# yhwu/rsicnv

Measured on AMD Instinct MI355X. Metric: bases/sec through RSI pipeline (bin+GC+NB+segment), higher is better.
Workload: dtype int32

## Files before the change

### include/rsi_hot.h

```cpp
#ifndef RSI_HOT_H
#define RSI_HOT_H
#include <stddef.h>
#include <stdint.h>
#ifdef __cplusplus
extern "C" {
#endif

typedef enum rsi_status {
  RSI_OK = 0,
  RSI_ERR_NO_DEVICE = -1,
  RSI_ERR_BAD_ARG = -2,
  RSI_ERR_HIP = -3,
  RSI_ERR_TOO_SMALL = -4,
  RSI_ERR_UNSUPPORTED = -5,
  RSI_ERR_INTERNAL = -6
} rsi_status;

typedef struct rsi_params {
  int32_t m;
  int32_t gcadjust;
  int32_t trans;
  int32_t merge;
  int32_t maxchkbp;
  int32_t debug;
// ... 182 lines not shown
int rsi_result_summary(const rsi_result* r, int chrom_id, double* out, int max_calls);
int rsi_summary_format_row(const double* block, int i, const char* chrom, char* buf, int cap);
int rsi_summary_format_rows(const double* block, const char* chrom, char* buf, int cap);
int rsi_result_log_line(const rsi_result* r, int i, char* buf, int cap);
int rsi_bam_references(const char* bam_path, char* names, int names_cap, int64_t* lengths, int max_refs);
int rsi_hot_run_bam(rsi_ctx* ctx, const rsi_params* p, const char* bam_path, const char* chrom, int minq, int min_baseq,
                    const uint8_t* fasta, int64_t n, rsi_result** out, rsi_bam_stats* stats);
int rsi_hot_run_device(rsi_ctx* ctx, const rsi_params* p, const void* d_depth, const void* d_fasta, int64_t n,
                       rsi_result** out);

typedef struct rsi_ref rsi_ref;
typedef struct rsi_ref_seq {
  int64_t length, offset;
  int32_t linebases, linewidth;
  char name[256];
} rsi_ref_seq;
typedef struct rsi_ref_stats {
  int64_t bytes_read;
  int64_t text_bytes;
  int64_t members;
  int32_t format;
  int32_t index_used;
  double t_kernel_ms;
  double t_wall_ms;
} rsi_ref_stats;
int rsi_ref_open(const char* fasta_path, const char* fai_path, const char* gzi_path, rsi_ref** out);
void rsi_ref_close(rsi_ref* ref);
const char* rsi_ref_last_error(const rsi_ref* ref);
int rsi_ref_count(const rsi_ref* ref);
int rsi_ref_sequence(const rsi_ref* ref, int i, rsi_ref_seq* out);
int rsi_ref_find(const rsi_ref* ref, const char* rname);
int rsi_ref_format(const rsi_ref* ref);
const char* rsi_ref_index_path(const rsi_ref* ref);
int rsi_ref_load_device(rsi_ref* ref, int device, int i, void* d_out, int64_t cap, void* stream, rsi_ref_stats* st);
int rsi_ref_load_host(rsi_ref* ref, int device, int i, uint8_t* out, int64_t cap);
int rsi_hot_run_text_dfasta(rsi_ctx* ctx, const rsi_params* p, const char* depth_path, const void* d_fasta, int64_t n,
                            rsi_result** out, rsi_text_stats* stats);
int rsi_hot_run_bam_dfasta(rsi_ctx* ctx, const rsi_params* p, const char* bam_path, const char* chrom, int minq, int min_baseq,
                           const void* d_fasta, int64_t n, rsi_result** out, rsi_bam_stats* stats);
void* rsi_ref_device_alloc(int device, int64_t bytes);
void rsi_ref_device_free(int device, void* p);
int rsi_ref_debug_fai_line(const char* line, rsi_ref_seq* out);
int rsi_ref_debug_set_chunks(rsi_ref* ref, int64_t text_chunk_bases, int64_t bgzf_span_bytes);
int rsi_ref_debug_ranges(const rsi_ref_seq* s, int64_t k0, int64_t k1, int64_t a_in, int64_t b_in, int at_eof, int64_t* out);
int64_t rsi_ref_debug_gzi(const uint8_t* image, int64_t len, int64_t* table, int64_t cap);
int rsi_ref_debug_cover(const int64_t* table, int64_t n, int64_t a, int64_t b, int64_t* out);

int rsi_hot_set_exclude(rsi_ctx* ctx, const int64_t* start, const int64_t* end, int count);
int rsi_exclude_read_bed(const char* path, const char* chrom, int64_t n, int64_t* start, int64_t* end, int cap);

typedef struct rsi_track_stats { int64_t n, lines, bytes, slices; double t_total_ms, t_kernel_ms, t_write_ms; } rsi_track_stats;
int rsi_hot_write_track(rsi_ctx* ctx, int which, const char* chrom, const char* path, int append, rsi_track_stats* stats);
int rsi_hot_write_track_device(rsi_ctx* ctx, const void* d_values, int64_t n, const char* chrom, const char* path, int append,
                               rsi_track_stats* stats);
int64_t rsi_hot_debug_track(rsi_ctx* ctx, const int32_t* values, int64_t n, const char* chrom, int64_t pos0, int64_t slice_bases,
                            char* out, int64_t cap, rsi_track_stats* stats);

int rsi_hot_write_bin_track(rsi_ctx* ctx, int which, const char* chrom, const char* path, int append, rsi_track_stats* stats);
int64_t rsi_hot_debug_bin_track(rsi_ctx* ctx, const int32_t* values, int64_t nb, int m, int64_t n, const int32_t* pairs, int npairs,
                                int64_t median2, int which, const char* chrom, int64_t slice_bins, char* out, int64_t cap,
                                rsi_track_stats* stats);

enum { RSI_TRACK_TEXT = 0, RSI_TRACK_BGZF = 1 };
int rsi_hot_set_track_format(rsi_ctx* ctx, int format);
typedef struct rsi_deflate_stats {
  int64_t members;
  int64_t stored_members;
  int64_t text_bytes;
  int64_t file_bytes;
  double t_kernel_ms;
} rsi_deflate_stats;
int rsi_hot_last_deflate_stats(const rsi_ctx* ctx, rsi_deflate_stats* out);
int rsi_bgzf_write_eof(const char* path);
int64_t rsi_hot_debug_deflate(rsi_ctx* ctx, const uint8_t* text, int64_t len, uint8_t* out, int64_t cap, rsi_deflate_stats* stats);

typedef struct rsi_track_index rsi_track_index;
rsi_track_index* rsi_track_index_create(void);
void rsi_track_index_free(rsi_track_index* ix);
int rsi_hot_set_track_index(rsi_ctx* ctx, rsi_track_index* ix);
int rsi_track_index_append(rsi_track_index* dst, const rsi_track_index* src, int64_t shift);
int rsi_track_index_write_tbi(rsi_track_index* ix, const char* path);
int rsi_track_index_counts(const rsi_track_index* ix, int64_t* nref, int64_t* nchunks, int64_t* nwindows);
int64_t rsi_track_index_debug_tbi(const rsi_track_index* ix, uint8_t* out, int64_t cap);

int rsi_hot_loaded_depth(rsi_ctx* ctx, const void** d_depth, int64_t* n);
typedef struct rsi_depth_summary {
  int64_t n, sum;
  int64_t over;
  int64_t negative;
  int32_t min, max;
} rsi_depth_summary;
int rsi_hot_depth_summary(rsi_ctx* ctx, const void* d_depth, int64_t n, rsi_depth_summary* out, int64_t* dist, int dist_cap);
typedef struct rsi_depth_region { int64_t n, sum; int32_t min, max; } rsi_depth_region;
int rsi_hot_depth_regions(rsi_ctx* ctx, const void* d_depth, int64_t n, int nreg, const int64_t* start, const int64_t* end, rsi_depth_region* out);
int rsi_hot_write_window_track(rsi_ctx* ctx, const void* d_depth, int64_t n, const char* chrom, int64_t W, const char* path, int append,
                               rsi_track_stats* stats);
int rsi_hot_write_region_track(rsi_ctx* ctx, const void* d_depth, int64_t n, const char* chrom, int nreg, const int64_t* start,
                               const int64_t* end, const char* path, int append, rsi_track_stats* stats);
typedef struct rsi_depth_stats {
  int64_t launches;
  int64_t workgroups;
  int64_t bytes;
  double ms;
  double kernel_ms;
} rsi_depth_stats;
int rsi_hot_last_depth_stats(const rsi_ctx* ctx, rsi_depth_stats* out);
int rsi_hot_debug_depth_summary(rsi_ctx* ctx, const int32_t* values, int64_t n, int64_t span, rsi_depth_summary* out, int64_t* dist, int dist_cap);
int rsi_hot_debug_depth_regions(rsi_ctx* ctx, const int32_t* values, int64_t n, int tile, int nreg, const int64_t* start, const int64_t* end,
                                rsi_depth_region* out);
int64_t rsi_hot_debug_region_track(rsi_ctx* ctx, const int32_t* values, int64_t n, const char* chrom, int64_t W, int nreg, const int64_t* start,
                                   const int64_t* end, int span, int tile, int64_t slice_lines, int64_t pos0, char* out, int64_t cap,
                                   rsi_track_stats* stats);

int rsi_result_ncalls(const rsi_result* r, int which);
const rsi_call* rsi_result_calls(const rsi_result* r, int which);
const rsi_chrom_stats* rsi_result_stats(const rsi_result* r);
int rsi_result_noncode(const rsi_result* r, int32_t* pairs, int cap);
int rsi_result_format_row(const rsi_result* r, int i, const char* chrom, char* buf, int cap);
void rsi_result_free(rsi_result* r);

int64_t rsi_hot_fetch_i32(rsi_ctx* ctx, const char* name, int32_t* out, int64_t cap);
int64_t rsi_hot_fetch_f32(rsi_ctx* ctx, const char* name, float* out, int64_t cap);
int64_t rsi_hot_fetch_i64(rsi_ctx* ctx, const char* name, int64_t* out, int64_t cap);

int rsi_hot_debug_level_sums(rsi_ctx* ctx, const float* T, const int32_t* status, int64_t nb, int Lmax, float* sums, int32_t* counts);
int rsi_hot_debug_scan(rsi_ctx* ctx, const float* T, const int32_t* medint, int64_t nb, double RDmedian, double tmedian, double tlamda,
                       int Lmax, int32_t* status, int32_t* info);
int rsi_hot_debug_segments(rsi_ctx* ctx, const float* T, const int32_t* status, int64_t nb, const int32_t* runs, int nruns, double tmedian,
                           double tlamda, int64_t pairs_per_item, int32_t* seg_start, int32_t* seg_end, int32_t* seg_type, double* seg_score,
                           int32_t* info);
int rsi_hot_debug_sharpen(rsi_ctx* ctx, const int32_t* depth, int64_t n, int storage, int32_t* start, int32_t* end, const int32_t* type,
                          int njobs, int32_t* info);
typedef struct rsi_cand_record {
  int32_t capacity, top, margin, cut, nleft, nright;
  int32_t road;
  int32_t flags, nref, nbody, nwin, left_reach, right_reach, body_min, body_max;
  int32_t type, status, geno;
  double body_q[3], body_s1, body_s2, ref_q[3], ref_s1, ref_s2;
  double p1, cnvmed, cnvsd, cnviqr, refmed, refsd, refiqr;
} rsi_cand_record;
int rsi_hot_debug_candidate_tests(rsi_ctx* ctx, const int32_t* depth, int64_t n, int storage, int64_t span_all, double RDmedian, int m,
                                  double minmlen, double chklen, double buffer, int maxchkbp, const int32_t* start, const int32_t* end,
                                  const int32_t* type, const int32_t* status, int ncand, const int32_t* index, int nindex, int form,
                                  rsi_cand_record* out, int32_t* info);
int rsi_hot_debug_range_sums(rsi_ctx* ctx, const int32_t* depth, int64_t n, int storage, const int32_t* lo, const int32_t* hi, int nranges,
                             int64_t* sums, int32_t* info);
int rsi_hot_debug_block_stage(rsi_ctx* ctx, const int32_t* binmedint, const int32_t* status, int64_t nb, int64_t ncompact, double RDmedian,
                              const rsi_params* P, rsi_call* segs, int nsegs, int use_tester, int sparse, int32_t* road, int32_t* info);
int rsi_hot_debug_merge(rsi_ctx* ctx, const int32_t* depth, int64_t n, int storage, double RDmedian, const rsi_params* P, const rsi_call* list,
                        int nlist, int use_tester, rsi_call* out, int32_t* nout, int32_t* info);
int rsi_hot_debug_calls(rsi_ctx* ctx, const int32_t* depth, int64_t n, int storage, double RDmedian, double RDsd, const rsi_params* P,
                        const rsi_call* segs, int nsegs, const int32_t* noncode_start, const int32_t* noncode_end, int nnoncode, int use_tester,
                        rsi_call* blocks, rsi_call* raw, rsi_call* kept, int32_t* counts, int32_t* info);
int rsi_hot_debug_nb_transform(rsi_ctx* ctx, const int64_t* binsum, int64_t nb, int m, int64_t ncompact, double RDmedian, double r,
                               float* raw, float* T, int32_t* info);
int rsi_hot_debug_filterstatus(rsi_ctx* ctx, const float* T, const int32_t* status, int64_t nb, int Lmax, double dev, int32_t* status_out,
                               int32_t* info);
int rsi_hot_debug_grid_median(rsi_ctx* ctx, const float* x, const int32_t* mask, int64_t nb, int mode, double center, double* out,
                              int32_t* info);
int rsi_hot_debug_grid_mad_i32(rsi_ctx* ctx, const int32_t* x, int64_t nb, double center, double* out, int32_t* info);
int rsi_hot_debug_nb_keyed(rsi_ctx* ctx, const int64_t* binsum, const int32_t* mask, int64_t nb, int m, int64_t K, double RDmedian, double r,
                           float* T, double* out, int32_t* info);

int rsi_hot_debug_classify(rsi_ctx* ctx, const uint8_t* fasta, int64_t n, const int64_t* start, const int64_t* end, int count,
                           uint64_t* gcbits, uint64_t* nbits);

int rsi_hot_debug_per_base(rsi_ctx* ctx, const rsi_params* p, const int32_t* depth, const uint8_t* fasta, int64_t n, const int64_t* start,
                           const int64_t* end, int count, rsi_chrom_stats* out);

int rsi_hot_kernel_times(const rsi_ctx* ctx, const char** names, float* ms, int cap);
int rsi_hot_phase_times(const rsi_ctx* ctx, const char** names, double* ms, int cap);
void rsi_hot_set_timing(rsi_ctx* ctx, int on);
void rsi_hot_set_timing_kernel(rsi_ctx* ctx, const char* name);

typedef struct rsi_pool rsi_pool;
#define RSI_MAX_TIMED 64
typedef struct rsi_batch_times {
  int32_t nkernels, nphases;
  const char* kernel_name[RSI_MAX_TIMED];
  double kernel_ms[RSI_MAX_TIMED];
  int64_t kernel_launches[RSI_MAX_TIMED];
  int64_t kernel_bases[RSI_MAX_TIMED];
  const char* phase_name[RSI_MAX_TIMED];
  double phase_ms[RSI_MAX_TIMED];
} rsi_batch_times;

rsi_pool* rsi_pool_create(int device, int nworkers, int* status);
void rsi_pool_destroy(rsi_pool* pool);
int rsi_pool_workers(const rsi_pool* pool);
int rsi_pool_hw_queues(const rsi_pool* pool);
rsi_ctx* rsi_pool_worker(rsi_pool* pool, int w);
void rsi_pool_set_timing(rsi_pool* pool, int on);
void rsi_pool_set_timing_kernel(rsi_pool* pool, const char* name);
void rsi_pool_set_schedule(rsi_pool* pool, int isolate, int streamers);
const char* rsi_pool_last_error(const rsi_pool* pool);
int rsi_pool_run(rsi_pool* pool, const rsi_params* p, int nchrom, const void* const* d_depth,
                 const void* const* d_fasta, const int64_t* n, rsi_result** out, int* status,
                 rsi_batch_times* times);

int rsi_plot_expand(const int32_t* rdc, int64_t ncompact, const int32_t* regions, int npairs, int32_t* out, int64_t n);
int rsi_plot_write_files(const rsi_call* c, const char* title, const int32_t* rd, int64_t n, double chrom_median, int m,
                         double minmlen, double chklen, const char* format, double gnuplot_version, const char* datfile,
                         const char* gpfile, const char* imgfile);

typedef struct rsi_plot_batch rsi_plot_batch;
rsi_plot_batch* rsi_plot_batch_new(int64_t n, int m, double minmlen, double chklen);
void rsi_plot_batch_free(rsi_plot_batch* b);
int rsi_plot_batch_add(rsi_plot_batch* b, const rsi_call* c);
int rsi_plot_batch_add_span(rsi_plot_batch* b, int start, int end, int type);
int rsi_plot_batch_size(const rsi_plot_batch* b);
int rsi_plot_batch_refusal(const rsi_plot_batch* b, int i);
const char* rsi_plot_refusal_text(int refusal);
int64_t rsi_plot_batch_queries(const rsi_plot_batch* b);
int rsi_plot_batch_fill_host(rsi_plot_batch* b, const int32_t* rd, int64_t n);
double rsi_plot_batch_chrom_median(const rsi_plot_batch* b);
int rsi_plot_batch_compare(const rsi_plot_batch* a, const rsi_plot_batch* b);
int rsi_plot_batch_write(const rsi_plot_batch* b, int i, const char* title, const char* format, double gnuplot_version, const char* datfile,
                         const char* gpfile, const char* imgfile);
typedef struct rsi_plot_stats {
  int64_t launches, batches, tiles;
  int64_t calls, queries;
  int64_t bytes_up, bytes_down;
  int64_t bytes;
  double ms, expand_ms;
} rsi_plot_stats;
int rsi_hot_plot_depth(rsi_ctx* ctx, const void* d_depth, int64_t n, rsi_plot_batch* b);
int rsi_hot_plot_run(rsi_ctx* ctx, const rsi_result* res, rsi_plot_batch* b);
int rsi_hot_last_plot_stats(const rsi_ctx* ctx, rsi_plot_stats* out);
int rsi_hot_debug_plot(rsi_ctx* ctx, const int32_t* depth, int64_t n, int tile, int64_t workspace_bytes, rsi_plot_batch* b);
int rsi_hot_debug_plot_expand(rsi_ctx* ctx, const int32_t* rdc, int64_t ncompact, int storage, const int32_t* regions, int npairs, int32_t* out, int64_t n);

int rsi_pool_run_host(rsi_pool* pool, const rsi_params* p, int nchrom, const int32_t* const* depth,
                      const uint8_t* const* fasta, const int64_t* n, rsi_result** out, int* status,
                      rsi_batch_times* times);

uint64_t rsi_pool_submit(rsi_pool* pool, const rsi_params* p, int nchrom, const void* const* d_depth,
                         const void* const* d_fasta, const int64_t* n, rsi_result** out, int* status,
                         rsi_batch_times* times);
int rsi_pool_wait(rsi_pool* pool, uint64_t ticket);

#ifdef __cplusplus
}
#endif
#endif
```

### rsicnv_amd/api.py

```python
import contextlib
import ctypes as C
import os

import numpy as np

POOL_HW_QUEUES, MIN_HW_QUEUES = 32, 4


def _queue_count(s):
    return int(s) if s is not None and 1 <= len(s) <= 9 and all(c in "0123456789" for c in s) else -1


def _process_setup(env=os.environ):
    user = env.get("RSI_HOT_HW_QUEUES")
    if user != "keep":
        want = _queue_count(user)
        if want >= 0:
            env["GPU_MAX_HW_QUEUES"] = str(min(POOL_HW_QUEUES, max(MIN_HW_QUEUES, want)))
        elif _queue_count(env.get("GPU_MAX_HW_QUEUES")) < POOL_HW_QUEUES:
            env["GPU_MAX_HW_QUEUES"] = str(POOL_HW_QUEUES)
    return max(0, _queue_count(env.get("GPU_MAX_HW_QUEUES")))


HW_QUEUES = _process_setup()

_HERE = os.path.dirname(os.path.abspath(__file__))
LIB_PATH = os.environ.get("RSI_HOT_LIB") or os.path.join(_HERE, "librsi_hot.so")

RSI_OK = 0
STATUS_NAMES = {0: "RSI_OK", -1: "RSI_ERR_NO_DEVICE", -2: "RSI_ERR_BAD_ARG", -3: "RSI_ERR_HIP",
                -4: "RSI_ERR_TOO_SMALL", -5: "RSI_ERR_UNSUPPORTED", -6: "RSI_ERR_INTERNAL"}

CAND_RECORD = np.dtype([(k, np.int32) for k in ("capacity", "top", "margin", "cut", "nleft", "nright", "road", "flags", "nref", "nbody", "nwin",
                                                "left_reach", "right_reach", "body_min", "body_max", "type", "status", "geno")] +
                       [("body_q", np.float64, 3), ("body_s1", np.float64), ("body_s2", np.float64), ("ref_q", np.float64, 3),
                        ("ref_s1", np.float64), ("ref_s2", np.float64)] +
                       [(k, np.float64) for k in ("p1", "cnvmed", "cnvsd", "cnviqr", "refmed", "refsd", "refiqr")])
assert CAND_RECORD.itemsize == 18 * 4 + 17 * 8

CALL_RECORD = np.dtype([(k, np.int32) for k in ("start", "end", "type", "geno", "status", "length", "qscore", "pad")] +
                       [(k, np.float64) for k in ("score", "p1", "cnvmed", "cnvsd", "cnviqr", "refmed", "refsd", "refiqr")])
assert CALL_RECORD.itemsize == 8 * 4 + 8 * 8
LIST_INFO = ("spec_hits", "single_tests", "host_fallbacks", "block_batch_hits", "waits", "sum_launches", "sum_reused", "sum_redone", "tests")

GENO_RECORD = np.dtype([(k, np.int32) for k in ("n_body", "n_flank", "body_min", "body_max")] +
                       [("body_sum", np.int64), ("flank_sum", np.int64), ("body_q", np.float64, 3), ("flank_q", np.float64, 3),
                        ("chrom_median", np.float64)])
assert GENO_RECORD.itemsize == 4 * 4 + 2 * 8 + 7 * 8

DEPTH_SUMMARY = np.dtype([(k, np.int64) for k in ("n", "sum", "over", "negative")] + [("min", np.int32), ("max", np.int32)])
DEPTH_REGION = np.dtype([("n", np.int64), ("sum", np.int64), ("min", np.int32), ("max", np.int32)])
assert DEPTH_SUMMARY.itemsize == 40 and DEPTH_REGION.itemsize == 24
DEPTH_BINS = 65536

EXPORTS = ["rsi_default_params", "rsi_hot_create", "rsi_hot_destroy", "rsi_hot_last_error", "rsi_hot_run",
           "rsi_hot_run_device", "rsi_hot_load_depth_text", "rsi_hot_run_text", "rsi_hot_load_depth_bam", "rsi_hot_run_bam", "rsi_bam_references", "rsi_result_annotate_bam", "rsi_result_summary", "rsi_summary_format_row", "rsi_summary_format_rows", "rsi_result_pairs", "rsi_result_ncalls", "rsi_result_calls", "rsi_result_stats", "rsi_result_noncode",
           "rsi_result_format_row", "rsi_result_free", "rsi_hot_fetch_i32", "rsi_hot_fetch_f32", "rsi_hot_fetch_i64",
           "rsi_hot_kernel_times", "rsi_hot_phase_times", "rsi_hot_set_timing", "rsi_hot_process_setup", "rsi_pool_create", "rsi_pool_destroy", "rsi_pool_workers", "rsi_pool_hw_queues", "rsi_pool_worker",
           "rsi_pool_set_timing", "rsi_pool_set_timing_kernel", "rsi_hot_set_timing_kernel", "rsi_pool_set_schedule", "rsi_pool_last_error", "rsi_pool_run", "rsi_pool_run_host", "rsi_pool_submit", "rsi_pool_wait", "rsi_plot_expand", "rsi_plot_write_files", "rsi_result_log_line", "rsi_hot_debug_level_sums", "rsi_hot_debug_scan", "rsi_hot_debug_segments", "rsi_hot_debug_sharpen", "rsi_hot_debug_candidate_tests", "rsi_hot_debug_range_sums", "rsi_hot_debug_block_stage", "rsi_hot_debug_merge", "rsi_hot_debug_calls", "rsi_hot_debug_nb_transform", "rsi_hot_debug_nb_keyed", "rsi_hot_debug_filterstatus", "rsi_hot_debug_grid_median", "rsi_hot_debug_grid_mad_i32", "rsi_synth_generate_host", "rsi_synth_generate_device", "rsi_synth_write_depth_text", "rsi_synth_write_fasta", "rsi_synth_append_genome_text",
           "rsi_genome_text_open", "rsi_genome_text_next", "rsi_genome_text_release", "rsi_genome_text_copy_depth",
           "rsi_genome_text_kernel_ms", "rsi_genome_text_close", "rsi_genome_text_last_error", "rsi_hot_run_depth_device",
           "rsi_hot_last_inflate_stats", "rsi_hot_inflate_bgzf", "rsi_genome_text_inflate_stats",
           "rsi_synth_append_genome_bgzf", "rsi_genome_text_open_samples", "rsi_genome_text_samples", "rsi_genome_text_max_resident",
           "rsi_genome_text_sample_depth", "rsi_genome_text_copy_sample_depth", "rsi_synth_append_genome_samples",
           "rsi_genome_bedgraph_open", "rsi_synth_append_genome_bedgraph", "rsi_genome_bedgraph_open_indexed", "rsi_genome_text_index_range",
           "rsi_hot_set_exclude", "rsi_exclude_read_bed", "rsi_hot_debug_classify", "rsi_hot_debug_per_base",
           "rsi_hot_write_track", "rsi_hot_write_track_device", "rsi_hot_debug_track",
           "rsi_hot_write_bin_track", "rsi_hot_debug_bin_track",
           "rsi_hot_set_track_format", "rsi_hot_last_deflate_stats", "rsi_bgzf_write_eof", "rsi_hot_debug_deflate",
           "rsi_track_index_create", "rsi_track_index_free", "rsi_hot_set_track_index", "rsi_track_index_append",
           "rsi_track_index_write_tbi", "rsi_track_index_counts", "rsi_track_index_debug_tbi",
           "rsi_ref_open", "rsi_ref_close", "rsi_ref_last_error", "rsi_ref_count", "rsi_ref_sequence", "rsi_ref_find", "rsi_ref_format",
           "rsi_ref_index_path", "rsi_ref_load_device", "rsi_ref_load_host", "rsi_ref_device_alloc", "rsi_ref_device_free",
           "rsi_hot_run_text_dfasta", "rsi_hot_run_bam_dfasta",
           "rsi_hot_set_bam_read", "rsi_hot_last_bam_read_stats",
           "rsi_hot_set_bam_pairs", "rsi_result_annotate_device", "rsi_hot_last_pairs_stats", "rsi_hot_debug_pair_sample",
           "rsi_hot_debug_pair_annotate",
           "rsi_hot_set_bam_pin", "rsi_hot_stat_calls", "rsi_hot_pin_sample", "rsi_hot_pin_calls", "rsi_hot_last_pin_stats",
           "rsi_hot_debug_pin_sample", "rsi_hot_debug_pin_calls",
           "rsi_hot_geno_calls", "rsi_hot_last_geno_stats", "rsi_hot_debug_geno",
           "rsi_hot_loaded_depth", "rsi_hot_depth_summary", "rsi_hot_depth_regions", "rsi_hot_write_window_track", "rsi_hot_write_region_track",
           "rsi_hot_last_depth_stats", "rsi_hot_debug_depth_summary", "rsi_hot_debug_depth_regions", "rsi_hot_debug_region_track",
           "rsi_plot_batch_new", "rsi_plot_batch_free", "rsi_plot_batch_add", "rsi_plot_batch_add_span", "rsi_plot_batch_size",
           "rsi_plot_batch_refusal", "rsi_plot_refusal_text", "rsi_plot_batch_queries", "rsi_plot_batch_fill_host",
           "rsi_plot_batch_chrom_median", "rsi_plot_batch_compare", "rsi_plot_batch_write", "rsi_hot_plot_depth", "rsi_hot_plot_run", "rsi_hot_last_plot_stats",
           "rsi_hot_debug_plot", "rsi_hot_debug_plot_expand",
           "rsi_ref_debug_set_chunks", "rsi_ref_debug_fai_line", "rsi_ref_debug_ranges", "rsi_ref_debug_gzi", "rsi_ref_debug_cover"]


class RsiParams(C.Structure):
    _fields_ = [("m", C.c_int32), ("gcadjust", C.c_int32), ("trans", C.c_int32), ("merge", C.c_int32),
                ("maxchkbp", C.c_int32), ("debug", C.c_int32), ("cap", C.c_double), ("epsilon", C.c_double),
                ("threshold", C.c_double), ("chklen", C.c_double), ("minmlen", C.c_double),
                ("buffer", C.c_double), ("p", C.c_double)]


class RsiCall(C.Structure):
    _fields_ = [("start", C.c_int32), ("end", C.c_int32), ("type", C.c_int32), ("geno", C.c_int32),
                ("status", C.c_int32), ("length", C.c_int32), ("qscore", C.c_int32), ("pad", C.c_int32),
                ("score", C.c_double), ("p1", C.c_double), ("cnvmed", C.c_double), ("cnvsd", C.c_double),
                ("cnviqr", C.c_double), ("refmed", C.c_double), ("refsd", C.c_double), ("refiqr", C.c_double)]


class RsiChromStats(C.Structure):
    _fields_ = [("n", C.c_int64), ("n_compact", C.c_int64), ("nbins", C.c_int64), ("n_noncode", C.c_int32),
                ("Lmax", C.c_int32), ("gc_rdmean", C.c_double), ("cap_median", C.c_double), ("RDmedian", C.c_double),
                ("RDsd", C.c_double), ("nb_mad", C.c_double), ("nb_r", C.c_double), ("nb_tmin", C.c_double),
                ("tmedian1", C.c_double), ("tsigma1", C.c_double), ("tlamda1", C.c_double), ("tmedian2", C.c_double),
                ("tsigma2", C.c_double), ("tlamda2", C.c_double), ("trim_escapes", C.c_int32),
                ("inexact_sums", C.c_int32), ("t_device_ms", C.c_double), ("t_kernels_ms", C.c_double),
                ("byte_escapes", C.c_int64), ("scan_tiles", C.c_int32), ("scan_tiles_listed", C.c_int32)]


RSI_MAX_TIMED = 64
SUMMARY_HEAD, SUMMARY_CALL = 8, 8


class RsiTextStats(C.Structure):
    _fields_ = [("bytes", C.c_int64), ("lines", C.c_int64), ("stored", C.c_int64), ("beyond", C.c_int64),
                ("fallback", C.c_int32), ("pad", C.c_int32), ("t_total_ms", C.c_double), ("t_parse_kernel_ms", C.c_double)]


class RsiInflateStats(C.Structure):
    _fields_ = [("format", C.c_int32), ("eof_block", C.c_int32), ("input_error", C.c_int32), ("pad", C.c_int32), ("compressed_bytes", C.c_int64), ("text_bytes", C.c_int64),
                ("blocks", C.c_int64), ("t_inflate_kernel_ms", C.c_double), ("t_host_inflate_ms", C.c_double)]


class RsiTrackStats(C.Structure):
    _fields_ = [("n", C.c_int64), ("lines", C.c_int64), ("bytes", C.c_int64), ("slices", C.c_int64),
                ("t_total_ms", C.c_double), ("t_kernel_ms", C.c_double), ("t_write_ms", C.c_double)]


class RsiDeflateStats(C.Structure):
    _fields_ = [("members", C.c_int64), ("stored_members", C.c_int64), ("text_bytes", C.c_int64), ("file_bytes", C.c_int64),
                ("t_kernel_ms", C.c_double)]


INFLATE_FORMATS = {0: "text", 1: "bgzf", 2: "gzip"}
TRACK_FORMATS = {"text": 0, "bgzf": 1}


class RsiRefSeq(C.Structure):
    _fields_ = [("length", C.c_int64), ("offset", C.c_int64), ("linebases", C.c_int32), ("linewidth", C.c_int32), ("name", C.c_char * 256)]


class RsiRefStats(C.Structure):
    _fields_ = [("bytes_read", C.c_int64), ("text_bytes", C.c_int64), ("members", C.c_int64), ("format", C.c_int32),
                ("index_used", C.c_int32), ("t_kernel_ms", C.c_double), ("t_wall_ms", C.c_double)]


def _inflate_dict(st):
    d = {f[0]: getattr(st, f[0]) for f in RsiInflateStats._fields_ if f[0] != "pad"}
    d["format"] = INFLATE_FORMATS.get(st.format, str(st.format))
    return d


class RsiGenomeChrom(C.Structure):
    _fields_ = [("slot", C.c_int32), ("pad", C.c_int32), ("n", C.c_int64), ("d_depth", C.c_void_p), ("stats", RsiTextStats),
                ("name", C.c_char * 256)]


class RsiBamStats(C.Structure):
    _fields_ = [("n", C.c_int64), ("bytes_compressed", C.c_int64), ("bytes_inflated", C.c_int64), ("records", C.c_int64), ("on_chrom", C.c_int64),
                ("used", C.c_int64), ("runs", C.c_int64), ("tid", C.c_int32), ("indexed", C.c_int32),
                ("t_total_ms", C.c_double), ("t_inflate_ms", C.c_double), ("t_walk_ms", C.c_double), ("t_wait_ms", C.c_double),
                ("malformed", C.c_int64)]


class RsiBamReadStats(C.Structure):
    _fields_ = [("mode", C.c_int32), ("pad", C.c_int32), ("chunks", C.c_int64), ("members", C.c_int64), ("segments", C.c_int64),
                ("guessed", C.c_int64), ("rewalked", C.c_int64), ("passed", C.c_int64),
                ("t_upload_ms", C.c_double), ("t_inflate_ms", C.c_double), ("t_find_ms", C.c_double)]


class RsiPairsStats(C.Structure):
    _fields_ = [("records", C.c_int64), ("table_bytes", C.c_int64), ("maxspan", C.c_int64), ("sample_count", C.c_int64),
                ("sample_abs", C.c_int64), ("sample_sq", C.c_int64), ("sample_stop", C.c_int64), ("isize", C.c_int32),
                ("isize_sd", C.c_int32), ("calls", C.c_int64), ("examined", C.c_int64),
                ("t_table_ms", C.c_double), ("t_sample_ms", C.c_double), ("t_annotate_ms", C.c_double)]


class RsiPinStats(C.Structure):
    _fields_ = [("records", C.c_int64), ("table_bytes", C.c_int64), ("pool_words", C.c_int64), ("sample_reads", C.c_int64),
                ("pos_start", C.c_int32), ("pos_end", C.c_int32), ("l_qseq", C.c_int32), ("r_len", C.c_int32),
                ("rd", C.c_double), ("rd_sd", C.c_double), ("drd", C.c_double), ("drd_sd", C.c_double), ("breakpoints", C.c_int64),
                ("t_table_ms", C.c_double), ("t_sample_ms", C.c_double), ("t_windows_ms", C.c_double)]


class RsiGenoStats(C.Structure):
    _fields_ = [("launches", C.c_int64), ("jobs", C.c_int64), ("tiles", C.c_int64), ("passes", C.c_int64), ("bytes", C.c_int64),
                ("ms", C.c_double)]


class RsiPlotStats(C.Structure):
    _fields_ = [(k, C.c_int64) for k in ("launches", "batches", "tiles", "calls", "queries", "bytes_up", "bytes_down", "bytes")] + \
               [("ms", C.c_double), ("expand_ms", C.c_double)]


class RsiDepthStats(C.Structure):
    _fields_ = [("launches", C.c_int64), ("workgroups", C.c_int64), ("bytes", C.c_int64), ("ms", C.c_double), ("kernel_ms", C.c_double)]


BAM_READ_MODES = {"host": 0, "device": 1}
BAM_SEGMENT = 16384


class RsiBatchTimes(C.Structure):
    _fields_ = [("nkernels", C.c_int32), ("nphases", C.c_int32), ("kernel_name", C.c_char_p * RSI_MAX_TIMED),
                ("kernel_ms", C.c_double * RSI_MAX_TIMED), ("kernel_launches", C.c_int64 * RSI_MAX_TIMED),
                ("kernel_bases", C.c_int64 * RSI_MAX_TIMED), ("phase_name", C.c_char_p * RSI_MAX_TIMED),
                ("phase_ms", C.c_double * RSI_MAX_TIMED)]

# ... 438 lines not shown
        return [r.replace("%CHROM%", chrom) for r in self.rows]


class RsiHot:

    def __init__(self, device=0):
        self.lib = load_library()
        st = C.c_int(0)
        self.ctx = self.lib.rsi_hot_create(device, C.byref(st))
        if not self.ctx:
            raise RsiError(st.value, self.lib.rsi_hot_last_error(None).decode())

    def close(self):
        if getattr(self, "ctx", None):
            self.lib.rsi_hot_destroy(self.ctx)
            self.ctx = None

    def __del__(self):
        try:
            self.close()
        except Exception:
            pass

    def _check(self, rc):
        if rc != RSI_OK:
            raise RsiError(rc, self.lib.rsi_hot_last_error(self.ctx).decode())

    def set_timing(self, on=True):
        self.lib.rsi_hot_set_timing(self.ctx, int(on))

    def debug_level_sums(self, T, status, Lmax):
        t = np.ascontiguousarray(T, dtype=np.float32)
        s = np.ascontiguousarray(status, dtype=np.int32)
        assert t.size == s.size
        sums = np.zeros(2 * Lmax + 1, dtype=np.float32)
        counts = np.zeros(2 * Lmax + 1, dtype=np.int32)
        self.lib.rsi_hot_debug_level_sums.argtypes = [C.c_void_p, C.c_void_p, C.c_void_p, C.c_int64, C.c_int, C.c_void_p, C.c_void_p]
        self._check(self.lib.rsi_hot_debug_level_sums(self.ctx, t.ctypes.data, s.ctypes.data, t.size, int(Lmax), sums.ctypes.data, counts.ctypes.data))
        return sums, counts

    def debug_scan(self, T, medint, RDmedian, tmedian, tlamda, Lmax):
        t = np.ascontiguousarray(T, dtype=np.float32)
        mi = np.ascontiguousarray(medint, dtype=np.int32)
        assert t.size == mi.size
        st = np.zeros(t.size, dtype=np.int32)
        info = np.zeros(4, dtype=np.int32)
        self.lib.rsi_hot_debug_scan.argtypes = [C.c_void_p, C.c_void_p, C.c_void_p, C.c_int64, C.c_double, C.c_double, C.c_double, C.c_int,
                                                C.c_void_p, C.c_void_p]
        self._check(self.lib.rsi_hot_debug_scan(self.ctx, t.ctypes.data, mi.ctypes.data, t.size, float(RDmedian), float(tmedian), float(tlamda),
                                                int(Lmax), st.ctypes.data, info.ctypes.data))
        return st, info

    def debug_segments(self, T, status, runs, tmedian, tlamda=0.0, pairs_per_item=0):
        t = np.ascontiguousarray(T, dtype=np.float32)
        st = np.ascontiguousarray(status, dtype=np.int32)
        assert st.size == t.size
        rl = np.ascontiguousarray(runs, dtype=np.int32).reshape(-1, 2)
        k = rl.shape[0]
        s, e, ty = (np.zeros(max(k, 1), dtype=np.int32) for _ in range(3))
        sc = np.zeros(max(k, 1), dtype=np.float64)
        info = np.zeros(8, dtype=np.int32)
        self.lib.rsi_hot_debug_segments.argtypes = [C.c_void_p, C.c_void_p, C.c_void_p, C.c_int64, C.c_void_p, C.c_int, C.c_double, C.c_double,
                                                    C.c_int64, C.c_void_p, C.c_void_p, C.c_void_p, C.c_void_p, C.c_void_p]
        self._check(self.lib.rsi_hot_debug_segments(self.ctx, t.ctypes.data, st.ctypes.data, t.size, rl.ctypes.data, k, float(tmedian), float(tlamda),
                                                    int(pairs_per_item), s.ctypes.data, e.ctypes.data, ty.ctypes.data, sc.ctypes.data, info.ctypes.data))
        n = int(info[5])
        return s[:n], e[:n], ty[:n], sc[:n], info

    def debug_sharpen(self, depth, storage, start, end, type_):
        d = np.ascontiguousarray(depth, dtype=np.int32)
        s = np.array(start, dtype=np.int32).reshape(-1)
        e = np.array(end, dtype=np.int32).reshape(-1)
        ty = np.ascontiguousarray(type_, dtype=np.int32).reshape(-1)
        assert s.size == e.size == ty.size
        info = np.zeros(4, dtype=np.int32)
        self.lib.rsi_hot_debug_sharpen.argtypes = [C.c_void_p, C.c_void_p, C.c_int64, C.c_int, C.c_void_p, C.c_void_p, C.c_void_p, C.c_int, C.c_void_p]
        self._check(self.lib.rsi_hot_debug_sharpen(self.ctx, d.ctypes.data, d.size, int(storage), s.ctypes.data, e.ctypes.data, ty.ctypes.data, s.size,
                                                   info.ctypes.data))
        return s, e, info

    def debug_candidate_tests(self, depth, storage, span_all, RDmedian, cands, index, form, m=101, minmlen=3.01, chklen=2.5, buffer=0.05,
                              maxchkbp=100000):
        d = np.ascontiguousarray(depth, dtype=np.int32)
        c = np.ascontiguousarray(cands, dtype=np.int32).reshape(-1, 4)
        cols = [np.ascontiguousarray(c[:, j]) for j in range(4)]
        ix = np.ascontiguousarray(index, dtype=np.int32).reshape(-1)
        out = np.zeros(max(ix.size, 1), dtype=CAND_RECORD)
        info = np.zeros(8, dtype=np.int32)
        self.lib.rsi_hot_debug_candidate_tests.argtypes = [C.c_void_p, C.c_void_p, C.c_int64, C.c_int, C.c_int64, C.c_double, C.c_int, C.c_double,
                                                           C.c_double, C.c_double, C.c_int, C.c_void_p, C.c_void_p, C.c_void_p, C.c_void_p, C.c_int,
                                                           C.c_void_p, C.c_int, C.c_int, C.c_void_p, C.c_void_p]
        self._check(self.lib.rsi_hot_debug_candidate_tests(self.ctx, d.ctypes.data, d.size, int(storage), int(span_all), float(RDmedian), int(m),
                                                           float(minmlen), float(chklen), float(buffer), int(maxchkbp), cols[0].ctypes.data,
                                                           cols[1].ctypes.data, cols[2].ctypes.data, cols[3].ctypes.data, c.shape[0],
                                                           ix.ctypes.data, ix.size, int(form), out.ctypes.data, info.ctypes.data))
        return out[:ix.size], info

    def debug_range_sums(self, depth, storage, lo, hi):
        d = np.ascontiguousarray(depth, dtype=np.int32)
        a = np.ascontiguousarray(lo, dtype=np.int32).reshape(-1)
        b = np.ascontiguousarray(hi, dtype=np.int32).reshape(-1)
        assert a.size == b.size
        sums = np.zeros(max(a.size, 1), dtype=np.int64)
        info = np.zeros(2, dtype=np.int32)
        self.lib.rsi_hot_debug_range_sums.argtypes = [C.c_void_p, C.c_void_p, C.c_int64, C.c_int, C.c_void_p, C.c_void_p, C.c_int, C.c_void_p, C.c_void_p]
        self._check(self.lib.rsi_hot_debug_range_sums(self.ctx, d.ctypes.data, d.size, int(storage), a.ctypes.data, b.ctypes.data, a.size,
                                                      sums.ctypes.data, info.ctypes.data))
        return sums[:a.size], info

    def debug_block_stage(self, binmedint, status, segs, ncompact, RDmedian, tester=True, sparse=False, **params):
        b = np.ascontiguousarray(binmedint, dtype=np.int32)
        st = np.ascontiguousarray(status, dtype=np.int32)
        assert b.size == st.size
        L = np.array(segs, dtype=CALL_RECORD).reshape(-1)
        road = np.full(max(L.size, 1), -1, dtype=np.int32)
        info = np.zeros(10, dtype=np.int32)
        P = make_params(**params)
        self.lib.rsi_hot_debug_block_stage.argtypes = [C.c_void_p, C.c_void_p, C.c_void_p, C.c_int64, C.c_int64, C.c_double, C.c_void_p, C.c_void_p,
                                                       C.c_int, C.c_int, C.c_int, C.c_void_p, C.c_void_p]
        self._check(self.lib.rsi_hot_debug_block_stage(self.ctx, b.ctypes.data, st.ctypes.data, b.size, int(ncompact), float(RDmedian), C.addressof(P),
                                                       L.ctypes.data, L.size, int(bool(tester)), int(bool(sparse)), road.ctypes.data, info.ctypes.data))
        return L, road[:L.size], dict(zip(LIST_INFO, (int(v) for v in info)))

    def debug_merge(self, depth, storage, cands, RDmedian, tester=True, **params):
        d = np.ascontiguousarray(depth, dtype=np.int32)
        L = np.ascontiguousarray(np.array(cands, dtype=CALL_RECORD).reshape(-1))
        out = np.zeros(max(L.size, 1), dtype=CALL_RECORD)
        nout = np.zeros(1, dtype=np.int32)
        info = np.zeros(10, dtype=np.int32)
        P = make_params(**params)
        self.lib.rsi_hot_debug_merge.argtypes = [C.c_void_p, C.c_void_p, C.c_int64, C.c_int, C.c_double, C.c_void_p, C.c_void_p, C.c_int, C.c_int,
                                                 C.c_void_p, C.c_void_p, C.c_void_p]
        self._check(self.lib.rsi_hot_debug_merge(self.ctx, d.ctypes.data, d.size, int(storage), float(RDmedian), C.addressof(P), L.ctypes.data, L.size,
                                                 int(bool(tester)), out.ctypes.data, nout.ctypes.data, info.ctypes.data))
        return out[:int(nout[0])], dict(zip(LIST_INFO, (int(v) for v in info)))

    def debug_calls(self, depth, storage, segs, noncode, RDmedian, RDsd, tester=True, **params):
        d = np.ascontiguousarray(depth, dtype=np.int32)
        L = np.ascontiguousarray(np.array(segs, dtype=CALL_RECORD).reshape(-1))
        nc = np.asarray(noncode, dtype=np.int32).reshape(-1, 2)
        a, b = np.ascontiguousarray(nc[:, 0]), np.ascontiguousarray(nc[:, 1])
        outs = [np.zeros(max(L.size, 1), dtype=CALL_RECORD) for _ in range(3)]
        counts = np.zeros(3, dtype=np.int32)
        info = np.zeros(10, dtype=np.int32)
        P = make_params(**params)
        self.lib.rsi_hot_debug_calls.argtypes = [C.c_void_p, C.c_void_p, C.c_int64, C.c_int, C.c_double, C.c_double, C.c_void_p, C.c_void_p, C.c_int,
                                                 C.c_void_p, C.c_void_p, C.c_int, C.c_int, C.c_void_p, C.c_void_p, C.c_void_p, C.c_void_p, C.c_void_p]
        self._check(self.lib.rsi_hot_debug_calls(self.ctx, d.ctypes.data, d.size, int(storage), float(RDmedian), float(RDsd), C.addressof(P),
                                                 L.ctypes.data, L.size, a.ctypes.data if a.size else None, b.ctypes.data if b.size else None, a.size,
                                                 int(bool(tester)), outs[0].ctypes.data, outs[1].ctypes.data, outs[2].ctypes.data, counts.ctypes.data,
                                                 info.ctypes.data))
        return outs[0][:counts[0]], outs[1][:counts[1]], outs[2][:counts[2]], dict(zip(LIST_INFO, (int(v) for v in info)))

    def debug_nb_transform(self, binsum, m, ncompact, RDmedian, r):
        b = np.ascontiguousarray(binsum, dtype=np.int64)
        raw = np.zeros(b.size, dtype=np.float32)
        T = np.zeros(b.size, dtype=np.float32)
        info = np.zeros(8, dtype=np.int32)
        self.lib.rsi_hot_debug_nb_transform.argtypes = [C.c_void_p, C.c_void_p, C.c_int64, C.c_int, C.c_int64, C.c_double, C.c_double, C.c_void_p,
                                                        C.c_void_p, C.c_void_p]
        self._check(self.lib.rsi_hot_debug_nb_transform(self.ctx, b.ctypes.data, b.size, int(m), int(ncompact), float(RDmedian), float(r),
                                                        raw.ctypes.data, T.ctypes.data, info.ctypes.data))
        return raw, T, info

    def debug_nb_keyed(self, binsum, m, K, RDmedian, r, mask=None):
        b = np.ascontiguousarray(binsum, dtype=np.int64)
        mk = None if mask is None else np.ascontiguousarray(mask, dtype=np.int32)
        assert mk is None or mk.size == b.size
        T = np.zeros(b.size, dtype=np.float32)
        out = np.zeros(4, dtype=np.float64)
        info = np.zeros(8, dtype=np.int32)
        self.lib.rsi_hot_debug_nb_keyed.argtypes = [C.c_void_p, C.c_void_p, C.c_void_p, C.c_int64, C.c_int, C.c_int64, C.c_double, C.c_double,
                                                    C.c_void_p, C.c_void_p, C.c_void_p]
        self._check(self.lib.rsi_hot_debug_nb_keyed(self.ctx, b.ctypes.data, None if mk is None else mk.ctypes.data, b.size, int(m), int(K),
                                                    float(RDmedian), float(r), T.ctypes.data, out.ctypes.data, info.ctypes.data))
        return T, out, info

    def debug_filterstatus(self, T, status, Lmax, dev):
        t = np.ascontiguousarray(T, dtype=np.float32)
        st = np.ascontiguousarray(status, dtype=np.int32)
        assert st.size == t.size
        out = np.zeros(t.size, dtype=np.int32)
        info = np.zeros(10, dtype=np.int32)
        self.lib.rsi_hot_debug_filterstatus.argtypes = [C.c_void_p, C.c_void_p, C.c_void_p, C.c_int64, C.c_int, C.c_double, C.c_void_p, C.c_void_p]
        self._check(self.lib.rsi_hot_debug_filterstatus(self.ctx, t.ctypes.data, st.ctypes.data, t.size, int(Lmax), float(dev), out.ctypes.data,
                                                        info.ctypes.data))
        return out, info

    GRID_MODES = {"pair": 0, "mad": 1, "host": 2}

    def debug_grid_median(self, x, mask=None, mode="pair", center=0.0):
        out = np.zeros(4, dtype=np.float64)
        info = np.zeros(8, dtype=np.int32)
        if mode == "med":
            assert mask is None
            xi = np.ascontiguousarray(x, dtype=np.int32)
            self.lib.rsi_hot_debug_grid_mad_i32.argtypes = [C.c_void_p, C.c_void_p, C.c_int64, C.c_double, C.c_void_p, C.c_void_p]
            self._check(self.lib.rsi_hot_debug_grid_mad_i32(self.ctx, xi.ctypes.data, xi.size, float(center), out.ctypes.data, info.ctypes.data))
            return out, info
        xf = np.ascontiguousarray(x, dtype=np.float32)
        mk = None if mask is None else np.ascontiguousarray(mask, dtype=np.int32)
        assert mk is None or mk.size == xf.size
        self.lib.rsi_hot_debug_grid_median.argtypes = [C.c_void_p, C.c_void_p, C.c_void_p, C.c_int64, C.c_int, C.c_double, C.c_void_p, C.c_void_p]
        self._check(self.lib.rsi_hot_debug_grid_median(self.ctx, xf.ctypes.data, None if mk is None else mk.ctypes.data, xf.size,
                                                       self.GRID_MODES[mode], float(center), out.ctypes.data, info.ctypes.data))
        return out, info

    def set_exclude(self, exclude):
        if exclude is None or len(exclude) == 0:
            self._check(self.lib.rsi_hot_set_exclude(self.ctx, None, None, 0))
            return
        s, e = _interval_arrays(exclude)
        self._check(self.lib.rsi_hot_set_exclude(self.ctx, s.ctypes.data, e.ctypes.data, s.size))

    def debug_classify(self, fasta, exclude=None):
        f = np.ascontiguousarray(fasta, dtype=np.uint8)
        gc = np.zeros(f.size // 64 + 1, dtype=np.uint64)
        nb = np.zeros(f.size // 64 + 1, dtype=np.uint64)
        if exclude is None or len(exclude) == 0:
            rc = self.lib.rsi_hot_debug_classify(self.ctx, f.ctypes.data, f.size, None, None, 0, gc.ctypes.data, nb.ctypes.data)
        else:
            s, e = _interval_arrays(exclude)
            rc = self.lib.rsi_hot_debug_classify(self.ctx, f.ctypes.data, f.size, s.ctypes.data, e.ctypes.data, s.size, gc.ctypes.data, nb.ctypes.data)
        self._check(rc)
        return gc, nb

    def debug_per_base(self, params, depth, fasta, exclude=None):
        d = np.ascontiguousarray(depth, dtype=np.int32)
        f = np.ascontiguousarray(fasta, dtype=np.uint8)
        if d.shape != f.shape or d.ndim != 1:
            raise ValueError("depth and fasta must be 1-D arrays of the same length")
        st = RsiChromStats()
        if exclude is None or len(exclude) == 0:
            rc = self.lib.rsi_hot_debug_per_base(self.ctx, C.byref(params), d.ctypes.data, f.ctypes.data, d.size, None, None, 0, C.byref(st))
        else:
            s, e = _interval_arrays(exclude)
            rc = self.lib.rsi_hot_debug_per_base(self.ctx, C.byref(params), d.ctypes.data, f.ctypes.data, d.size, s.ctypes.data, e.ctypes.data,
                                                 s.size, C.byref(st))
        self.last_stats = {k[0]: getattr(st, k[0]) for k in RsiChromStats._fields_}
        self._check(rc)
        return self.last_stats

    def run(self, params, depth, fasta, exclude=None):
        d = np.ascontiguousarray(depth, dtype=np.int32)
        f = np.ascontiguousarray(fasta, dtype=np.uint8)
        if d.shape != f.shape or d.ndim != 1:
            raise ValueError("depth and fasta must be 1-D arrays of the same length")
        out = C.c_void_p()
        if exclude is not None:
            self.set_exclude(exclude)
        self._check(self.lib.rsi_hot_run(self.ctx, C.byref(params), d.ctypes.data, f.ctypes.data, d.size, C.byref(out)))
        return Result(self.lib, out)

    def load_depth_text(self, path, n):
        st = RsiTextStats()
        self._check(self.lib.rsi_hot_load_depth_text(self.ctx, os.fsencode(path), int(n), C.byref(st)))
        return {f[0]: getattr(st, f[0]) for f in RsiTextStats._fields_ if f[0] != "pad"}

    def inflate_bgzf(self, data):
        data = bytes(data)
        st = RsiInflateStats()
        src = np.frombuffer(data, dtype=np.uint8) if data else np.zeros(1, dtype=np.uint8)
        size = self._bgzf_text_size(data)
        out = np.zeros(max(size, 1), dtype=np.uint8)
        k = self.lib.rsi_hot_inflate_bgzf(self.ctx, src.ctypes.data, len(data), out.ctypes.data, size, C.byref(st))
        self._check(int(k) if k < 0 else 0)
        return out[:k].tobytes()

    @staticmethod
    def _bgzf_text_size(data):
        p, total = 0, 0
        while p + 18 <= len(data):
            xlen = data[p + 10] | (data[p + 11] << 8)
            bsize = None
            k = p + 12
            while k + 4 <= p + 12 + xlen and k + 4 <= len(data):
                slen = data[k + 2] | (data[k + 3] << 8)
                if data[k] == 66 and data[k + 1] == 67 and slen == 2 and k + 6 <= len(data):
                    bsize = (data[k + 4] | (data[k + 5] << 8)) + 1
                k += 4 + slen
            if bsize is None or p + bsize > len(data):
                break
            total += int.from_bytes(data[p + bsize - 4:p + bsize], "little")
            p += bsize
        return total

    def inflate_stats(self):
        st = RsiInflateStats()
        self._check(self.lib.rsi_hot_last_inflate_stats(self.ctx, C.byref(st)))
        return _inflate_dict(st)

    def run_text(self, params, path, fasta, exclude=None):
        f = np.ascontiguousarray(fasta, dtype=np.uint8)
        if exclude is not None:
            self.set_exclude(exclude)
        out = C.c_void_p()
        st = RsiTextStats()
        self._check(self.lib.rsi_hot_run_text(self.ctx, C.byref(params), os.fsencode(path), f.ctypes.data, f.size, C.byref(out), C.byref(st)))
        res = Result(self.lib, out)
        res.text_stats = {f_[0]: getattr(st, f_[0]) for f_ in RsiTextStats._fields_ if f_[0] != "pad"}
        return res

    def load_depth_bam(self, bam, chrom, minq=0, min_baseq=13):
        st = RsiBamStats()
        self._check(self.lib.rsi_hot_load_depth_bam(self.ctx, os.fsencode(bam), chrom.encode(), int(minq), int(min_baseq), C.byref(st)))
        return {f[0]: getattr(st, f[0]) for f in RsiBamStats._fields_}
# ... 682 lines not shown
```

### rsicnv_amd/csrc/host_calls.cpp

```cpp
#include "host_calls.h"
#include <immintrin.h>
#include <math.h>
#include <stdio.h>
#include <stdlib.h>
#include <string.h>
#include <algorithm>
#include <chrono>
#include "hostmath.h"

namespace rsih {

static inline double tick_ms() { return std::chrono::duration<double, std::milli>(std::chrono::steady_clock::now().time_since_epoch()).count(); }

namespace {
inline void bucket_indices_body(const float* x, size_t n, double lo, double dy, uint32_t* idx) {
  for (size_t i = 0; i < n; ++i) idx[i] = (uint32_t)(int64_t)(((double)x[i] - lo) / dy + 0.5);
}
__attribute__((target("avx2"))) void bucket_indices_avx2(const float* x, size_t n, double lo, double dy, uint32_t* idx) {
  bucket_indices_body(x, n, lo, dy, idx);
}
void bucket_indices_sse2(const float* x, size_t n, double lo, double dy, uint32_t* idx) { bucket_indices_body(x, n, lo, dy, idx); }
}

void bucket_indices_f32(const float* x, size_t n, double lo, double dy, uint32_t* idx) {
// ... 524 lines not shown
  auto mean_of = [&](int slot, int lo, int hi) -> double {
    if (slot >= 0 && ranges[slot].first == lo && ranges[slot].second == hi) {
      if (in.prof) in.prof->sum_reused++;
      return (double)sums[slot] / double(hi - lo + 1);
    }
    if (in.tester) {
      std::vector<std::pair<int, int>> one(1, {lo, hi});
      std::vector<int64_t> s1;
      if (in.prof) { in.prof->sum_launches++; in.prof->sum_redone++; }
      if (in.tester->range_sums(one, s1)) return (double)s1[0] / double(hi - lo + 1);
    }
    return range_mean(A, lo, hi);
  };
  auto depth_rule = [&](int i, int slot) {
    const int w1 = L[i].end - L[i].start, w2 = L[i + 1].end - L[i + 1].start;
    const double m1 = mean_of(slot, L[i].start, L[i].end), m2 = mean_of(slot < 0 ? -1 : slot + 1, L[i + 1].start, L[i + 1].end);
    const double both = (m1 * w1 + m2 * w2) / (w1 + w2);
    const double across = mean_of(slot < 0 ? -1 : slot + 2, L[i].start, L[i + 1].end);
    if (L[i].type == kDel && across > both + 1.5 * L[i + 1].refsd + 1.5 * L[i].refsd) return false;
    if (L[i].type == kDup && across < both - 1.5 * L[i + 1].refsd - 1.5 * L[i].refsd) return false;
    return true;
  };
  auto joined_list = [&](int i) {
    Candidate joined = L[i];
    joined.end = L[i + 1].end;
    T = L; T[i] = joined; T[i + 1] = joined; T[i + 1].status = -9;
  };
  Speculation spec;
  std::vector<int> spec_slot((size_t)npairs, -1);
  if (in.tester) {
    for (int i = 0; i < npairs; ++i) {
      if (sum_slot[i] < 0 || !depth_rule(i, sum_slot[i])) continue;
      joined_list(i);
      int cut = 0;
      spec_slot[i] = (int)spec.plans.size();
      spec.plans.push_back(plan_test(in, A.size(), T, i, &cut));
    }
    spec.run(in);
  }
  for (int i = 0; i + 1 < (int)L.size(); ++i) {
    if (!near_pair(i)) continue;
    if (!depth_rule(i, in.tester ? sum_slot[i] : -1)) continue;
    joined_list(i);
    test_bases(in, A, T, i, &spec, spec_slot[i]);
    if (T[i].geno == 0) continue;
    L[i] = T[i]; L[i + 1] = T[i]; L[i].status = -9;
  }
  drop_deleted(L);
}

int to_reference(const std::vector<Region>& noncode, int p) {
  int removed = 0;
  for (const Region& r : noncode) {
    const int grown = removed + (r.end - r.start + 1);
    if (p < r.end + 1 - grown) break;
    removed = grown;
  }
  return p + removed;
}

}

void debug_merge_neighbours(const CallerInput& in, DepthPager& depth, std::vector<Candidate>& list) {
  merge_neighbours(in, PagedView{&depth}, list);
}

int debug_neighbour_tests(const CallerInput& in, DepthPager& depth, const std::vector<Candidate>& list, const std::vector<int>& idx,
                          std::vector<DebugTest>& out) {
  const PagedView A{&depth};
  std::vector<TestPlan> plans;
  int cut = 0;
  for (int ci : idx) {
    plans.push_back(plan_test(in, A.size(), list, ci, &cut));
    if (plans.back().capacity <= 0) return 2;
  }
  std::vector<TestStats> stats;
  std::vector<int> reach;
  std::vector<char> ok;
  if (!in.tester || !in.tester->test(plans, stats, reach, ok)) return 1;
  out.clear();
  std::vector<Candidate> L;
  for (size_t k = 0; k < idx.size(); ++k) {
    L = list;
    if (ok[k]) finish_judgement(in, stats[k], L[(size_t)idx[k]]);
    else test_candidate(in, A, L, idx[k]);
    out.push_back(DebugTest{plans[k], L[(size_t)idx[k]], ok[k] ? 0 : 1});
  }
  return 0;
}

void test_block_segments(const CallerInput& in, IntSpan status, std::vector<Candidate>& segs) {
  const VecView bins{in.binmedint};
  std::vector<Candidate> T = segs;
  constexpr int kBlockBatchMin = 24;
  std::vector<TestPlan> plans;
  std::vector<TestStats> stats;
  std::vector<int> reach;
  std::vector<char> ok;
  bool sorted = true;
  for (size_t i = 1; i < T.size(); ++i) sorted = sorted && T[i - 1].end < T[i].start;
  for (const Candidate& c : T) sorted = sorted && c.status != -9;
  if (in.block_tester && sorted && (int)T.size() >= kBlockBatchMin) {
    int cut = 0;
    for (int i = 0; i < (int)T.size(); ++i) plans.push_back(plan_test(in, bins.size(), T, i, &cut));
    if (!in.block_tester->test(plans, stats, reach, ok)) plans.clear();
  }
  int rejected_end = -1;
  if (in.block_roads) in.block_roads->clear();
  for (int i = 0; i < (int)T.size(); ++i) {
    if (!plans.empty() && ok[(size_t)i] && !(plans[(size_t)i].cut & 1) && rejected_end < reach[(size_t)i]) {
      finish_judgement(in, stats[(size_t)i], T[i]);
      if (in.prof) in.prof->block_batch_hits++;
      if (in.block_roads) in.block_roads->push_back(0);
    } else {
      if (in.block_roads) in.block_roads->push_back(plans.empty() ? 1 : !ok[(size_t)i] ? 4 : (plans[(size_t)i].cut & 1) ? 3 : 2);
      test_candidate(in, bins, T, i);
    }
    if (T[i].status == -9 && T[i].end > rejected_end) rejected_end = T[i].end;
  }
  for (int i = 0; i < (int)T.size(); ++i) {
    if (T[i].status != -9) continue;
    if (T[i].type == kDel && T[i].cnvmed < 0.7 * T[i].refmed) { T[i].geno = 1; T[i].p1 = in.P.p; continue; }
    if (T[i].type == kDup && T[i].cnvmed > 1.3 * T[i].refmed) { T[i].geno = 1; T[i].p1 = in.P.p; continue; }
    const Candidate original = T[i];
    Candidate chosen = T[i];
    std::vector<Candidate> levels;
    nested_levels(chosen, status, levels);
    for (int j = (int)levels.size() - 1; j >= 0; --j) {
      levels[j].type = chosen.type;
      T[i] = levels[j];
      test_candidate(in, bins, T, i);
      levels[j] = T[i];
    }
    for (int j = (int)levels.size() - 1; j >= 0; --j) {
      if (levels[j].geno == 0) continue;
      if (chosen.geno == 0) chosen = levels[j];
      if (levels[j].length > chosen.length) chosen = levels[j];
    }
    if (chosen.geno == 0) chosen = original;
    T[i] = chosen;
  }
  segs.swap(T);
}

void call_from_segments(const CallerInput& in, std::vector<Candidate> segs, DepthPager& depth,
                        std::vector<Candidate>& blocks, std::vector<Candidate>& raw, std::vector<Candidate>& kept) {
  const rsi_params& P = in.P;
  const PagedView bases{&depth};
  const int m = P.m, np = (int)in.ncompact;
  order_by_start(segs);
  blocks = segs;
  std::vector<Candidate> L;
  for (Candidate c : segs) {
    if (c.geno == 0 || c.start == c.end) continue;
    c.start = c.start * m + m / 2;
    c.end = c.end * m + m / 2;
    if (c.start < 0) c.start = 0;
    if (c.end > np - 1) c.end = np - 1;
    c.length = c.end - c.start + 1;
    L.push_back(c);
  }
  const double ts0 = tick_ms();
  if (!(in.tester && in.tester->sharpen(L)))
    for (int pass = 0; pass < 2; ++pass) for (Candidate& c : L) sharpen_edges(bases, c);
  order_by_start(L);
  const double ts1 = tick_ms();
  merge_neighbours(in, bases, L);
  const double ts2 = tick_ms();
  order_by_start(L);
  Speculation spec;
  if (in.tester) {
    int cut = 0;
    for (int i = 0; i < (int)L.size(); ++i) spec.plans.push_back(plan_test(in, bases.size(), L, i, &cut));
    spec.run(in);
  }
  raw.clear();
  for (int i = 0; i < (int)L.size(); ++i) {
    const double nbins = double(L[i].end - L[i].start + 1) / double(m);
    test_bases(in, bases, L, i, &spec, i);
    L[i].score = (L[i].cnvmed - in.RDmedian) * sqrt(nbins);
    const int r1 = to_reference(*in.noncode, L[i].start), r2 = to_reference(*in.noncode, L[i].end);
    for (const Region& g : *in.noncode) if (std::max(r1, g.start) <= std::min(r2, g.end)) L[i].status = -9;
    if (L[i].status != -9) raw.push_back(L[i]);
  }
  if (in.prof) { in.prof->sharpen += ts1 - ts0; in.prof->merge += ts2 - ts1; in.prof->final_tests += tick_ms() - ts2; }
  for (Candidate& c : raw) { c.start = to_reference(*in.noncode, c.start); c.end = to_reference(*in.noncode, c.end); }

  kept.clear();
  const int minlen = std::max(m * 2, 500);
  const double sd = in.RDsd / 1.2;
  for (const Candidate& c : raw) {
    const int span = abs(c.end - c.start);
    bool keep = !(span < 1000);
    if (c.type == kDel) {
      if (c.p1 > 0.2 || c.refsd > 0.6 * sd || c.cnvsd > 1.3 * sd) keep = false;
      if (c.cnvsd * in.RDmedian > 2.5 * c.cnvmed * sd) keep = false;
      if (c.cnvmed < 0.66 * std::min(in.RDmedian, c.refmed) && c.cnvsd < sd && span > 800) keep = true;
    }
    if (c.type == kDup) {
      if (c.p1 > 0.05 || c.refsd > 0.6 * sd) keep = false;
      if (c.cnvsd * in.RDmedian > 2.0 * c.cnvmed * sd) keep = false;
    }
    if (span < minlen) keep = false;
    if (keep) kept.push_back(c);
  }
}

}
```

### rsicnv_amd/csrc/host_calls.h

```cpp
#pragma once
#include <hip/hip_runtime.h>
#include <stdint.h>
#include <functional>
#include <memory>
#include <utility>
#include <vector>
#include "../../include/rsi_hot.h"

namespace rsih {

enum { kDel = 0, kDup = 1, kUnknown = 2 };

struct Candidate {
  int type = kUnknown, geno = 0, status = 0, start = 0, end = 0, length = 0;
  double score = 0, p1 = 1.0, cnvmed = 0, cnvsd = 0, cnviqr = 0, refmed = 0, refsd = 0, refiqr = 0;
};

struct Region { int start, end; };

class DepthPager {
 public:
  DepthPager(const int32_t* d_ptr, int64_t n, hipStream_t stream, std::function<int32_t*()> mirror, void* staging = nullptr,
             size_t staging_bytes = 0, hipEvent_t sync_event = nullptr);
  DepthPager(const int32_t* host_ptr, int64_t n);
  DepthPager(const DepthPager&) = delete;
  DepthPager& operator=(const DepthPager&) = delete;
  int64_t size() const { return n_; }
  int operator[](int64_t i) {
    if (!have_[(size_t)(i >> kBits)]) fetch(i >> kBits, i >> kBits);
    return failed_ ? 0 : mirror_[i];
  }
  bool failed() const { return failed_; }
  void prefetch(int64_t lo, int64_t hi);
  const int32_t* raw() const { return mirror_; }
  int64_t bytes_fetched() const { return fetched_; }
  double fetch_ms() const { return fetch_ms_; }
 private:
  static constexpr int kBits = 14;
  void fetch(int64_t p0, int64_t p1);
  const int32_t* d_;
  int64_t n_;
  hipStream_t stream_;
  std::function<int32_t*()> mirror_source_;
  int32_t* mirror_ = nullptr;
  std::vector<unsigned char> have_;
  int32_t* staging_ = nullptr;
  int64_t staging_elems_ = 0;
  hipEvent_t sync_ev_ = nullptr;
  void wait();
  int64_t fetched_ = 0;
  double fetch_ms_ = 0;
  bool failed_ = false;
};

struct CallProfile {
  double fetch = 0, gather = 0, winmean = 0, quantiles = 0, variance = 0, sharpen = 0, merge = 0, final_tests = 0, device_ms = 0;
  int tests = 0, spec_hits = 0, single_tests = 0, host_fallbacks = 0, block_batch_hits = 0;
  int sum_launches = 0, sum_reused = 0, sum_redone = 0;
};

struct TestStats { double cnv_lqt, cnv_med, cnv_uqt, cnv_var, ref_lqt, ref_med, ref_uqt, ref_var; };

struct TestPlan {
  int start, end, kind, margin, capacity, top, budget, cut;
  double right_cap;
  std::vector<std::pair<int, int>> left_chain, right_chain;
};

class NeighbourTester {
 public:
  virtual ~NeighbourTester() {}
  virtual bool sharpen(std::vector<Candidate>& L) = 0;
  virtual bool test(const std::vector<TestPlan>& plans, std::vector<TestStats>& stats, std::vector<int>& left_reach,
                    std::vector<char>& ok) = 0;
  virtual bool range_sums(const std::vector<std::pair<int, int>>& ranges, std::vector<int64_t>& sums) = 0;
};

struct IntSpan {
  const int* p = nullptr;
  int64_t n = 0;
  struct Range { int64_t first, last, at; };
  const std::vector<Range>* ranges = nullptr;
  IntSpan() {}
  IntSpan(const int* p_, int64_t n_) : p(p_), n(n_) {}
  IntSpan(const std::vector<int>& v) : p(v.data()), n((int64_t)v.size()) {}
  IntSpan(const int* values, int64_t n_, const std::vector<Range>* r) : p(values), n(n_), ranges(r) {}
  const int* at(int64_t i) const {
    if (!ranges) return p + i;
    size_t lo = 0, hi = ranges->size();
    while (lo + 1 < hi) { const size_t mid = (lo + hi) / 2; if ((*ranges)[mid].first <= i) lo = mid; else hi = mid; }
    const Range& r = (*ranges)[lo];
    if (i < r.first || i > r.last) { static const int zero = 0; return &zero; }
    return p + r.at + (i - r.first);
  }
  int operator[](int64_t i) const { return ranges ? *at(i) : p[i]; }
  int64_t size() const { return n; }
};

struct CallerInput {
  rsi_params P;
  CallProfile* prof = nullptr;
  NeighbourTester* tester = nullptr;
  NeighbourTester* block_tester = nullptr;
  double RDmedian, RDsd;
  int64_t ncompact;
  const std::vector<Region>* noncode;
  IntSpan binmedint;
  int* short_neighbourhoods = nullptr;
  std::vector<int>* block_roads = nullptr;
};

void test_block_segments(const CallerInput& in, IntSpan status, std::vector<Candidate>& segs);

void call_from_segments(const CallerInput& in, std::vector<Candidate> segs, DepthPager& depth,
                        std::vector<Candidate>& blocks, std::vector<Candidate>& raw, std::vector<Candidate>& kept);

struct DebugTest { TestPlan plan; Candidate judged; int road; };
int debug_neighbour_tests(const CallerInput& in, DepthPager& depth, const std::vector<Candidate>& list, const std::vector<int>& idx,
                          std::vector<DebugTest>& out);

void debug_merge_neighbours(const CallerInput& in, DepthPager& depth, std::vector<Candidate>& list);

int64_t narrow_depth_u8(const int32_t* src, int64_t n, uint8_t* dst, int32_t* esc_pos, int32_t* esc_val, int64_t cap);

}
```

### rsicnv_amd/csrc/hostmath.h

```cpp
#pragma once
#include <math.h>
#include <stddef.h>
#include <stdint.h>
#include <algorithm>
#include <vector>

namespace rsih {

struct Quantiles { double lqt, med, uqt; };

template <class T>
inline double grid_step(const T*) { return 0.01; }
template <>
inline double grid_step<int>(const int*) { return 1.0; }

void bucket_indices_f32(const float* x, size_t n, double lo, double dy, uint32_t* idx);

template <class T>
Quantiles grid_quantiles(const T* x, size_t n) {
  const double dy = grid_step(x);
  double lo = x[0], hi = x[0], acc = 0;
  for (size_t i = 0; i < n; ++i) {
    acc += x[i];
    if (x[i] < lo) lo = x[i];
    if (x[i] > hi) hi = x[i];
  }
  Quantiles q{lo, acc / (double)n, hi};
  if ((hi - lo) < dy) return q;
  const size_t buckets = (size_t)((hi - lo) / dy + 2);
  std::vector<uint32_t> cnt(buckets + 1, 0);
  for (size_t i = 0; i < n; ++i) cnt[(size_t)((x[i] - lo) / dy + 0.5)]++;
  const size_t r1 = n / 4, r2 = n / 2, r3 = n * 3 / 4;
  size_t seen = 0;
  for (size_t b = 0; b < buckets; ++b) {
    const size_t upto = seen + cnt[b];
    if (seen < r1 && upto >= r1) q.lqt = lo + b * dy;
    if (seen < r2 && upto >= r2) q.med = lo + b * dy;
    if (seen < r3 && upto >= r3) q.uqt = lo + b * dy;
    seen = upto;
  }
  return q;
}

template <>
inline Quantiles grid_quantiles<int>(const int* x, size_t n) {
  int lo = x[0], hi = x[0];
  double acc = 0;
  long long isum = 0;
  for (size_t i = 0; i < n; ++i) { isum += x[i]; lo = x[i] < lo ? x[i] : lo; hi = x[i] > hi ? x[i] : hi; }
  acc = (double)isum;
  Quantiles q{(double)lo, acc / (double)n, (double)hi};
  if (((double)hi - (double)lo) < 1.0) return q;
  const size_t buckets = (size_t)(((double)hi - (double)lo) / 1.0 + 2);
  std::vector<uint32_t> cnt(buckets + 1, 0);
  for (size_t i = 0; i < n; ++i) cnt[(size_t)((long long)x[i] - lo)]++;
  const size_t r1 = n / 4, r2 = n / 2, r3 = n * 3 / 4;
  size_t seen = 0;
  for (size_t b = 0; b < buckets; ++b) {
    const size_t upto = seen + cnt[b];
    if (seen < r1 && upto >= r1) q.lqt = (double)lo + b * 1.0;
    if (seen < r2 && upto >= r2) q.med = (double)lo + b * 1.0;
    if (seen < r3 && upto >= r3) q.uqt = (double)lo + b * 1.0;
    seen = upto;
  }
  return q;
}
inline Quantiles grid_quantiles_f32_known(const float* x, size_t n, float flo, float fhi, double sum) {
  const double dy = 0.01;
  const double lo = flo, hi = fhi;
  Quantiles q{lo, sum / (double)n, hi};
  if (n == 0 || (hi - lo) < dy) return q;
  const size_t buckets = (size_t)((hi - lo) / dy + 2);
  std::vector<uint32_t> cnt(buckets + 1, 0), idx(n);
  bucket_indices_f32(x, n, lo, dy, idx.data());
  for (size_t i = 0; i < n; ++i) cnt[idx[i]]++;
  const size_t r1 = n / 4, r2 = n / 2, r3 = n * 3 / 4;
  size_t seen = 0;
  for (size_t b = 0; b < buckets; ++b) {
    const size_t upto = seen + cnt[b];
    if (seen < r1 && upto >= r1) q.lqt = lo + b * dy;
    if (seen < r2 && upto >= r2) q.med = lo + b * dy;
    if (seen < r3 && upto >= r3) q.uqt = lo + b * dy;
    seen = upto;
  }
  return q;
}
template <>
inline Quantiles grid_quantiles<float>(const float* x, size_t n) {
  float flo = x[0], fhi = x[0];
  double acc = 0;
  for (size_t i = 0; i < n; ++i) { acc += x[i]; flo = x[i] < flo ? x[i] : flo; fhi = x[i] > fhi ? x[i] : fhi; }
  return grid_quantiles_f32_known(x, n, flo, fhi, acc);
}

inline bool hist_quantiles_int(const uint64_t* hist, size_t nvals, uint64_t total, Quantiles& q) {
  if (total == 0) return false;
  size_t lo = 0, hi = nvals - 1;
  while (lo < nvals && hist[lo] == 0) ++lo;
  while (hi > lo && hist[hi] == 0) --hi;
  if (lo >= nvals) return false;
  q = Quantiles{(double)lo, (double)lo, (double)hi};
  if ((double)hi - (double)lo < 1.0) return true;
  const uint64_t r1 = total / 4, r2 = total / 2, r3 = total * 3 / 4;
  uint64_t seen = 0;
  for (size_t v = lo; v <= hi; ++v) {
    const uint64_t upto = seen + hist[v];
    if (seen < r1 && upto >= r1) q.lqt = (double)lo + (double)(v - lo) * 1.0;
    if (seen < r2 && upto >= r2) q.med = (double)lo + (double)(v - lo) * 1.0;
    if (seen < r3 && upto >= r3) q.uqt = (double)lo + (double)(v - lo) * 1.0;
    seen = upto;
  }
  return true;
}

inline double hist_median_grid(const uint32_t* hist, size_t np, uint64_t total, double ymin) {
  const uint64_t r2 = total / 2;
  uint64_t seen = 0;
  double med = ymin;
  for (size_t b = 0; b < np; ++b) {
    const uint64_t upto = seen + hist[b];
    if (seen < r2 && upto >= r2) med = ymin + b * 0.01;
    seen = upto;
  }
  return med;
}

template <class T>
double variance_pop(const T* y, size_t n) {
  double s1 = 0.0, s2 = 0.0;
  for (size_t i = 0; i < n; ++i) { s1 += (double)y[i]; s2 += (double)y[i] * (double)y[i]; }
  const double mu = s1 / double(n);
  return s2 / double(n) - mu * mu;
}

double normal_cdf(double x);

template <class Pred>
double last_true(Pred pred) {
  if (!pred(0.0)) return -1.0;
  union { double d; uint64_t u; } lo, hi, mid;
  lo.d = 0.0; hi.d = INFINITY;
  if (pred(hi.d)) return INFINITY;
  while (hi.u - lo.u > 1) {
    mid.u = lo.u + (hi.u - lo.u) / 2;
    if (pred(mid.d)) lo = mid; else hi = mid;
  }
  return lo.d;
}
template <class Pred>
double first_true(Pred pred) {
  if (pred(0.0)) return 0.0;
  union { double d; uint64_t u; } lo, hi, mid;
  lo.d = 0.0; hi.d = INFINITY;
  if (!pred(hi.d)) return INFINITY;
  while (hi.u - lo.u > 1) {
    mid.u = lo.u + (hi.u - lo.u) / 2;
    if (pred(mid.d)) hi = mid; else lo = mid;
  }
  return hi.d;
}

}
```

### rsicnv_amd/csrc/pipeline.hip

```cpp
#include <new>
#include "pipeline_internal.h"
#include "geno_host.h"
#include "pipeline_steps.h"

using namespace rsik;
using namespace rsip;
using rsih::Candidate;
using rsih::Region;

namespace {

struct ScanOut {
  double tmedian1 = 0, tsigma1 = 0, tlamda1 = 0, tmedian2 = 0, tsigma2 = 0, tlamda2 = 0;
  int Lmax = 0;
  rsih::IntSpan status2;
  std::vector<int> run_status;
  std::vector<rsih::IntSpan::Range> run_ranges;
  std::vector<Candidate> segs;
  uint32_t escapes = 0, inexact = 0;
  uint32_t tiles_listed = 0;
  std::vector<uint32_t> level_log[4];
  uint32_t stop_levels[4] = {0, 0, 0, 0};
  std::vector<std::string> fs_lines;
};

int selection_mean(rsi_ctx* ctx, const float* d_x, const int32_t* d_mask, int64_t nb, int use_abs, double center, double* mean,
                   uint64_t* count) {
  HIPCHK(ctx->h_T.ensure((size_t)nb * 4));
  HIPCHK(hipMemcpyAsync(ctx->h_T.p, d_x, (size_t)nb * 4, hipMemcpyDeviceToHost, ctx->stream));
  if (d_mask) {
    HIPCHK(ctx->h_status.ensure((size_t)nb * 4));
    HIPCHK(hipMemcpyAsync(ctx->h_status.p, d_mask, (size_t)nb * 4, hipMemcpyDeviceToHost, ctx->stream));
  }
  HIPCHK(CTX_SYNC());
  const float* x = ctx->h_T.as<float>();
  const int* mk = d_mask ? ctx->h_status.as<int>() : nullptr;
  double acc = 0.0;
  uint64_t k = 0;
  for (int64_t i = 0; i < nb; ++i) {
    if (mk && mk[i] != 0) continue;
    const float v = use_abs ? (float)fabs((double)x[i] - center) : x[i];
    acc += v;
    ++k;
  }
  *count = k;
  *mean = k ? acc / (double)k : 0.0;
  return RSI_OK;
}

int grid_median(rsi_ctx* ctx, const float* d_x, const int32_t* d_mask, int64_t nb, int use_abs, double center,
                double* med, uint64_t* count) {
  uint8_t* small = ctx->small.as<uint8_t>();
  { Timer t(ctx, "minmax_f32"); launch_minmax_f32(d_x, d_mask, nb, use_abs, center, reinterpret_cast<MinMaxF*>(small + kOffMinMax), ctx->stream); }
  MinMaxF mm;
  HIPCHK(copy_d2h(ctx, &mm, small + kOffMinMax, sizeof(mm)));
  HIPCHK(hipMemsetAsync(small + kOffMinMax, 0, sizeof(MinMaxF), ctx->stream));
  HIPCHK(CTX_SYNC());
  if (mm.min_inv == 0u) { *count = 0; *med = 0; return RSI_OK; }
  if (mm.nonfinite) return fail(ctx, RSI_ERR_UNSUPPORTED, "non-finite value in the transformed bins");
  const double ymin = rsih::unkey_f32(~mm.min_inv), ymax = rsih::unkey_f32(mm.max_bits);
  if ((ymax - ymin) < 0.01) return selection_mean(ctx, d_x, d_mask, nb, use_abs, center, med, count);
  const size_t np = (size_t)((ymax - ymin) / 0.01 + 2);
  if (np > (64u << 20)) return fail(ctx, RSI_ERR_UNSUPPORTED, "transformed bin range too wide for the 0.01 grid");
  HIPCHK(ctx->hist_f.ensure(np * 4));
  HIPCHK(hipMemsetAsync(ctx->hist_f.p, 0, np * 4, ctx->stream));
  { Timer t(ctx, "hist_f32"); launch_hist_f32(d_x, d_mask, nb, use_abs, center, ymin, ctx->hist_f.as<uint32_t>(), (uint32_t)np, ctx->stream); }
  std::vector<uint32_t> h(np);
  HIPCHK(copy_d2h(ctx, h.data(), ctx->hist_f.p, np * 4));
  HIPCHK(CTX_SYNC());
  uint64_t total = 0;
  for (uint32_t c : h) total += c;
  *count = total;
  *med = rsih::hist_median_grid(h.data(), np, total, ymin);
  return RSI_OK;
}

constexpr uint32_t kGridCap = 1u << 20;
constexpr int32_t kFsListCap = 1 << 20;
struct ChainOut { GridMedian g[2]; uint32_t rawmin_inv; uint32_t pad[15]; };
GridChain grid_chain(rsi_ctx* ctx) {
  uint8_t* small = ctx->small.as<uint8_t>();
  return GridChain{reinterpret_cast<MinMaxF*>(small + kOffMinMax), ctx->hist_f.as<uint32_t>(), kGridCap,
                   reinterpret_cast<unsigned int*>(small + kOffDone) + kDoneBinSlot};
}
int nb_transform(rsi_ctx* ctx, const int64_t* d_binsum, int64_t nb, int m, int64_t ncompact, double RDmedian, double r, rsih::NbLevels& lev,
                 float* raw_out) {
  uint8_t* small = ctx->small.as<uint8_t>();
  hipStream_t st = ctx->stream;
  HIPCHK(ctx->tnb.ensure((size_t)nb * 4));
  HIPCHK(ctx->hist_f.ensure((size_t)kGridCap * 4));
  uint32_t* d_rawmin = reinterpret_cast<uint32_t*>(small + kOffRawMin);
  GridMedian* d_g = reinterpret_cast<GridMedian*>(small + kOffGrid);
  { Timer t(ctx, "nb_raw"); launch_nb_raw(d_binsum, nb, m, ncompact, r, ctx->tnb.as<float>(), d_rawmin, st); }
  if (raw_out) HIPCHK(hipMemcpyAsync(raw_out, ctx->tnb.p, (size_t)nb * 4, hipMemcpyDeviceToHost, st));
  lev = rsih::nb_reference_levels(RDmedian, m, r);
  { Timer t(ctx, "nb_scale"); launch_nb_scale_minmax(ctx->tnb.as<float>(), nb, d_rawmin, lev.med_raw, lev.del_raw, lev.dup_raw, RDmedian, grid_chain(ctx), d_g, st); }
  return RSI_OK;
}
void scan_fill_list(rsi_ctx* ctx, int pass, int64_t nb, FillList& fl) {
  uint8_t* small = ctx->small.as<uint8_t>();
  uint32_t* d_first_del = ctx->first_del.as<uint32_t>();
  const int64_t nbpad = (nb + 3) & ~int64_t(3);
  fill_add(fl, d_first_del, (size_t)(nbpad + nb) * 4, 0xffffffffu);
  fill_add(fl, small + kOffScanPass + (size_t)pass * kScanPassBytes, kScanPassBytes, 0u);
  fill_add(fl, small + kOffCounters, 32, 0u);
  if (pass == 0 && ctx->fs_ws.p) fill_add(fl, ctx->fs_ws.p, level_sums_head_bytes(kMaxL), 0u);
}
int grid_pair_issue(rsi_ctx* ctx, const float* d_x, const int32_t* d_mask, int64_t nb, bool with_median, double center, bool planned,
                    int fill_pass, ChainOut** out) {
  uint8_t* small = ctx->small.as<uint8_t>();
  GridMedian* d_g = reinterpret_cast<GridMedian*>(small + kOffGrid);
  const GridChain gc = grid_chain(ctx);
  ChainOut* slot = static_cast<ChainOut*>(mb_alloc(ctx, sizeof(ChainOut)));
  if (!slot) return fail(ctx, RSI_ERR_INTERNAL, "out of pinned mailbox memory");
  memset(slot, 0, sizeof(*slot));
  GateShared gs(ctx);
  if (with_median) {
    if (!planned) { Timer t(ctx, "minmax_plan"); launch_minmax_plan(d_x, d_mask, nb, 0, 0.0, nullptr, gc, d_g, ctx->stream); }
    { Timer t(ctx, "hist_walk"); launch_hist_walk(d_x, d_mask, nb, 0, 0.0, nullptr, gc, d_g, nullptr, nullptr, ctx->stream); }
    planned = false;
  }
  const double* d_center = with_median ? &d_g->med : nullptr;
  if (!planned) { Timer t(ctx, "minmax_plan"); launch_minmax_plan(d_x, d_mask, nb, 1, center, d_center, gc, d_g + 1, ctx->stream); }
  GridExport ex{};
  ex.src[0] = d_g; ex.dst[0] = slot->g; ex.bytes[0] = 2 * sizeof(GridMedian);
  ex.src[1] = small + kOffRawMin; ex.dst[1] = &slot->rawmin_inv; ex.bytes[1] = 4;
  FillList fl{};
  if (fill_pass >= 0) scan_fill_list(ctx, fill_pass, nb, fl);
  { Timer t(ctx, "hist_walk"); launch_hist_walk(d_x, d_mask, nb, 1, center, d_center, gc, d_g + 1, &ex, &fl, ctx->stream); }
  *out = slot;
  return RSI_OK;
}
static_assert(rsih::kNbKeyLimit == kNbKeyMax, "the route's limit is the kernels' table size");
struct NbKeyed { int64_t K = 0; const int64_t* d_binsum = nullptr; int m = 0; int64_t ncompact = 0; double r = 0, RDmedian = 0; rsih::NbLevels lev{0, 0, 0}; };
int nb_keyed_issue(rsi_ctx* ctx, const NbKeyed& kd, const int32_t* d_mask, int64_t nb, int fill_pass, ChainOut** out) {
  uint8_t* small = ctx->small.as<uint8_t>();
  GridMedian* d_g = reinterpret_cast<GridMedian*>(small + kOffGrid);
  hipStream_t st = ctx->stream;
  HIPCHK(ctx->tnb.ensure((size_t)nb * 4));
  HIPCHK(ctx->hist_f.ensure((size_t)kGridCap * 4));
  const bool fresh = ctx->nb_keys.p == nullptr;
  HIPCHK(ctx->nb_keys.ensure(nb_keys_workspace_bytes()));
  if (fresh) HIPCHK(hipMemsetAsync(ctx->nb_keys.p, 0, nb_keys_workspace_bytes(), st));
  ChainOut* slot = static_cast<ChainOut*>(mb_alloc(ctx, sizeof(ChainOut)));
  if (!slot) return fail(ctx, RSI_ERR_INTERNAL, "out of pinned mailbox memory");
  memset(slot, 0, sizeof(*slot));
  GridExport ex{};
  ex.src[0] = d_g; ex.dst[0] = slot->g; ex.bytes[0] = 2 * sizeof(GridMedian);
  ex.src[1] = small + kOffRawMin; ex.dst[1] = &slot->rawmin_inv; ex.bytes[1] = 4;
  FillList fl{};
  if (fill_pass >= 0) scan_fill_list(ctx, fill_pass, nb, fl);
  uint32_t* d_rawmin = reinterpret_cast<uint32_t*>(small + kOffRawMin);
  GateShared gs(ctx);
  if (!d_mask) {
    { Timer t(ctx, "nb_keys"); launch_nb_keys(kd.d_binsum, nullptr, nb, kd.m, kd.K, kd.r, kd.lev.med_raw, kd.lev.del_raw, kd.lev.dup_raw, kd.RDmedian, ctx->nb_keys.p, d_rawmin, grid_chain(ctx), d_g, &ex, nullptr, st); }
    { Timer t(ctx, "nb_apply"); launch_nb_apply(kd.d_binsum, nb, kd.K, ctx->nb_keys.p, ctx->tnb.as<float>(), &fl, st); }
  } else {
    Timer t(ctx, "nb_keys_masked");
    launch_nb_keys(kd.d_binsum, d_mask, nb, kd.m, kd.K, kd.r, kd.lev.med_raw, kd.lev.del_raw, kd.lev.dup_raw, kd.RDmedian, ctx->nb_keys.p, d_rawmin, grid_chain(ctx), d_g, &ex, &fl, st);
  }
  *out = slot;
  return RSI_OK;
}

struct Selection { const float* d_x; const int32_t* d_mask; int64_t nb; int use_abs; double center; };
int grid_result(rsi_ctx* ctx, const GridMedian& g, const Selection& sel, double* med, uint64_t* count) {
  if (g.flags & kGridEmpty) { *count = 0; *med = 0; return RSI_OK; }
  if (g.flags & kGridNonFinite) return fail(ctx, RSI_ERR_UNSUPPORTED, "non-finite value in the transformed bins");
  if (g.flags & kGridDegenerate) return selection_mean(ctx, sel.d_x, sel.d_mask, sel.nb, sel.use_abs, sel.center, med, count);
  *med = g.med; *count = g.count;
  return RSI_OK;
}

void scan_thresholds(double tmedian, double tlamda, int Lmax, std::vector<double>& del, std::vector<double>& dup) {
  del.assign((size_t)Lmax + 1 + kScanPad, -INFINITY);
  dup.assign((size_t)Lmax + 1 + kScanPad, INFINITY);
  del[0] = -1.0;
  for (int L = 1; L <= Lmax; ++L) {
    const double dL = (double)L, sq = sqrt(dL);
    auto score = [&](double sum) { const float meanf = (float)(sum / dL); return ((double)meanf - tmedian) * sq; };
    del[L] = rsih::last_true([&](double s) { return !(score(s) > -tlamda); });
    dup[L] = rsih::first_true([&](double s) { return !(score(s) < tlamda); });
  }
}

constexpr uint32_t kEagerBounds = 1024;
int runs_from_export(rsi_ctx* ctx, const uint32_t* slot, const uint64_t* d_list, std::vector<Region>& runs) {
  const uint32_t cnt = slot[0];
  runs.clear();
  if (cnt == 0) return RSI_OK;
  if (cnt > kMaxRunEntries) return fail(ctx, RSI_ERR_UNSUPPORTED, "boundary list overflow");
  std::vector<uint64_t> raw(cnt);
  memcpy(raw.data(), slot + 2, (size_t)std::min(cnt, kEagerBounds) * 8);
  if (cnt > kEagerBounds) {
    HIPCHK(copy_d2h(ctx, raw.data() + kEagerBounds, d_list + kEagerBounds, (size_t)(cnt - kEagerBounds) * 8));
    HIPCHK(CTX_SYNC());
  }
  if (!rsih::boundary_pairs(raw.data(), raw.size(), false, runs)) return fail(ctx, RSI_ERR_INTERNAL, "unbalanced run boundaries");
  runs.pop_back();
  return RSI_OK;
}

struct RunArgs { RunsInline inl; bool use_inl = false; int32_t* d_start = nullptr; int32_t* d_end = nullptr; };
int prepare_runs(rsi_ctx* ctx, const std::vector<Region>& runs, RunArgs& ra) {
  const size_t k = runs.size();
  if (k <= (size_t)kRunsInline) {
    memset(&ra.inl, 0, sizeof(ra.inl));
    for (size_t i = 0; i < k; ++i) { ra.inl.se[2 * i] = runs[i].start; ra.inl.se[2 * i + 1] = runs[i].end; }
    ra.use_inl = true;
    return RSI_OK;
  }
  HIPCHK(ctx->run_se.ensure(k * 8 + 64));
  std::vector<int32_t> se(2 * k);
  for (size_t i = 0; i < k; ++i) { se[i] = runs[i].start; se[k + i] = runs[i].end; }
  HIPCHK(copy_h2d(ctx, ctx->run_se.p, se.data(), k * 8));
  ra.use_inl = false;
  ra.d_start = ctx->run_se.as<int32_t>();
  ra.d_end = ctx->run_se.as<int32_t>() + k;
  return RSI_OK;
}

constexpr size_t kCandScratchBytes = size_t(512) << 20;
class DeviceTester : public rsih::NeighbourTester {
 public:
  DeviceTester(rsi_ctx* c, DepthRef rdc, int64_t n, double RDmedian) : ctx(c), d_rdc(rdc), N(n), median(RDmedian) {}
  double kernel_wait_ms = 0;
  int launches = 0;
  int force_split = -1, force_bytes = -1;
  std::vector<CandOut>* sink = nullptr;
  int mailbox_lists = 0, copied_lists = 0;

  bool sharpen(std::vector<Candidate>& L) override {
    if (L.empty()) return true;
    const int nj = (int)L.size();
    EdgeJob* slot = static_cast<EdgeJob*>(mb_alloc(ctx, (size_t)nj * sizeof(EdgeJob)));
    std::vector<EdgeJob> spill;
    EdgeJob* jobs = slot;
    if (!slot) { spill.resize((size_t)nj); jobs = spill.data(); }
    for (int i = 0; i < nj; ++i) jobs[i] = {L[(size_t)i].start, L[(size_t)i].end, L[(size_t)i].type, 0};
    {
      Phase ph(ctx, "cand.ensure");
      if (nj > ctx->sharpen_ws_jobs) {
        const int cap = std::max(256, 2 * nj);
        if (!ok(ctx->sharpen_ws.ensure(sharpen_workspace_bytes(cap)))) return false;
        if (!ok(hipMemsetAsync(ctx->sharpen_ws.p, 0, sharpen_workspace_zero_bytes(cap), ctx->stream))) return false;
        ctx->sharpen_ws_jobs = cap;
      }
      if (!slot && !ok(ctx->cand_jobs.ensure((size_t)nj * sizeof(EdgeJob)))) return false;
    }
    GateShared gs(ctx);
    Phase ph(ctx, "cand.sharpen");
    EdgeJob* d_jobs = slot ? slot : ctx->cand_jobs.as<EdgeJob>();
    if (!slot && !ok(copy_h2d(ctx, ctx->cand_jobs.p, jobs, (size_t)nj * sizeof(EdgeJob)))) return false;
    for (int pass = 0; pass < 2; ++pass) {
      Timer t(ctx, "sharpen_edges");
      launch_sharpen_edges(d_rdc, N, d_jobs, nj, ctx->sharpen_ws.p, ctx->sharpen_ws_jobs, ctx->stream);
    }
    if (!slot && !ok(copy_d2h(ctx, jobs, ctx->cand_jobs.p, (size_t)nj * sizeof(EdgeJob)))) return false;
    if (!wait()) return false;
    gs.release();
    for (int i = 0; i < nj; ++i) { L[(size_t)i].start = jobs[i].start; L[(size_t)i].end = jobs[i].end; }
    return true;
  }

  bool test(const std::vector<rsih::TestPlan>& plans, std::vector<rsih::TestStats>& stats, std::vector<int>& left_reach,
            std::vector<char>& okv) override {
    const size_t n = plans.size();
    stats.assign(n, rsih::TestStats{});
    left_reach.assign(n, 0);
    okv.assign(n, 0);
    const bool split = force_split >= 0 ? force_split != 0 : env_int("RSI_HOT_CAND_SPLIT", 1) != 0;
    if (sink) { CandOut none{}; none.flags = -1; sink->assign(n, none); }
    const int value_bytes = d_rdc.bytes == 1 && (force_bytes >= 0 ? force_bytes != 0 : env_int("RSI_HOT_CAND_BYTES", 1) != 0) ? 1 : 4;
    size_t first = 0;
    while (first < n) {
      std::vector<CandJob> jobs;
      std::vector<int32_t> chains;
      size_t ibytes = 0, lwords = 0, last = first;
      for (; last < n; ++last) {
        const rsih::TestPlan& T = plans[last];
        if (T.capacity <= 0 || T.end < T.start || T.start < 0 || T.end >= N) break;
        auto up4 = [](size_t x) { return (x + 3) & ~(size_t)3; };
        const size_t ib = cand_scratch_bytes(T.top, T.capacity, T.budget, value_bytes, split);
        const size_t lw = split ? 0 : up4((size_t)T.capacity + 1);
        if (!jobs.empty() && ibytes + ib + (lwords + lw) * 8 > kCandScratchBytes) break;
        CandJob J{};
        J.start = T.start; J.end = T.end; J.kind = T.kind; J.margin = T.margin; J.capacity = T.capacity; J.top = T.top;
        J.nleft = (int)T.left_chain.size(); J.nright = (int)T.right_chain.size();
        J.left_off = (int)(chains.size() / 2);
        for (const auto& iv : T.left_chain) { chains.push_back(iv.first); chains.push_back(iv.second); }
        J.right_off = (int)(chains.size() / 2);
        for (const auto& iv : T.right_chain) { chains.push_back(iv.first); chains.push_back(iv.second); }
        J.budget = T.budget; J.cut = T.cut; J.right_cap = T.right_cap;
        J.iscratch_off = (int64_t)(ibytes / 4); J.lscratch_off = (int64_t)lwords;
        ibytes += ib; lwords += lw;
        jobs.push_back(J);
      }
      if (jobs.empty()) { ++first; continue; }
      chains.push_back(0); chains.push_back(0);
      std::vector<CandOut> outs(jobs.size());
      {
        Phase ph(ctx, "cand.ensure");
        if (!ok(ctx->cand_jobs.ensure(jobs.size() * sizeof(CandJob))) || !ok(ctx->cand_chains.ensure(chains.size() * 4)) ||
            !ok(ctx->cand_outs.ensure(outs.size() * sizeof(CandOut))) || !ok(ctx->cand_i32.ensure(ibytes)) ||
            (!split && !ok(ctx->cand_i64.ensure(lwords * 8))))
          return false;
        if (split) {
          const size_t m0 = ctx->cand_mid.cap, h0 = ctx->cand_hist.cap;
          if (!ok(ctx->cand_mid.ensure(jobs.size() * sizeof(CandMid))) || !ok(ctx->cand_hist.ensure(jobs.size() * (size_t)kCandHistBins * 4))) return false;
          if (ctx->cand_mid.cap != m0 && !ok(hipMemsetAsync(ctx->cand_mid.p, 0, ctx->cand_mid.cap, ctx->stream))) return false;
          if (ctx->cand_hist.cap != h0 && !ok(hipMemsetAsync(ctx->cand_hist.p, 0, ctx->cand_hist.cap, ctx->stream))) return false;
        }
      }
      GateShared gs(ctx);
      Phase ph(ctx, "cand.test");
      const size_t jb = (jobs.size() * sizeof(CandJob) + 63) & ~size_t(63), cb = (chains.size() * 4 + 63) & ~size_t(63);
      const size_t ob = outs.size() * sizeof(CandOut);
      unsigned char* slot = jb + cb + ob <= kMailboxMaxCopy ? static_cast<unsigned char*>(mb_alloc(ctx, jb + cb + ob)) : nullptr;
      const CandJob* d_jobs = ctx->cand_jobs.as<CandJob>();
      const void* d_chains = ctx->cand_chains.p;
      CandOut* d_outs = ctx->cand_outs.as<CandOut>();
      ++(slot ? mailbox_lists : copied_lists);
      if (slot) {
        memcpy(slot, jobs.data(), jobs.size() * sizeof(CandJob));
        memcpy(slot + jb, chains.data(), chains.size() * 4);
        d_jobs = reinterpret_cast<const CandJob*>(slot); d_chains = slot + jb; d_outs = reinterpret_cast<CandOut*>(slot + jb + cb);
      } else {
        if (!ok(copy_h2d(ctx, ctx->cand_jobs.p, jobs.data(), jobs.size() * sizeof(CandJob)))) return false;
        if (!ok(copy_h2d(ctx, ctx->cand_chains.p, chains.data(), chains.size() * 4))) return false;
      }
      {
        const bool wide = d_rdc.bytes == 1 && value_bytes == 4;
        Timer t(ctx, split ? (wide ? "candidate_test_i32" : "candidate_test") : (wide ? "candidate_test_one_wg_i32" : "candidate_test_one_wg"));
        if (split)
          launch_candidate_test_split(d_rdc, N, d_jobs, (int)jobs.size(), d_chains, ctx->cand_i32.as<int32_t>(),
                                      median, ctx->cand_mid.as<CandMid>(), ctx->cand_hist.as<uint32_t>(),
                                      d_outs, value_bytes, ctx->stream);
        else
          launch_candidate_test(d_rdc, N, d_jobs, (int)jobs.size(), d_chains, ctx->cand_i32.as<int32_t>(),
                                ctx->cand_i64.as<long long>(), median, d_outs, value_bytes, ctx->stream);
      }
      if (!slot && !ok(copy_d2h(ctx, outs.data(), ctx->cand_outs.p, outs.size() * sizeof(CandOut)))) return false;
      if (!wait()) return false;
      if (slot) memcpy(outs.data(), d_outs, ob);
      gs.release();
      ph.stop();
      static const bool cand_dbg = env_int("RSI_HOT_CAND_DBG", 0) != 0;
      for (size_t k = 0; k < jobs.size(); ++k) {
        const CandOut& O = outs[k];
        if (cand_dbg)
          fprintf(stderr, "[cand] [%d,%d] kind %d margin %d cap %d top %d chains %d/%d cut %d -> flags %d nref %d nbody %d nwin %d reach %d/%d ref q %.6f %.6f %.6f s1 %.6f s2 %.6f\n",
                  jobs[k].start, jobs[k].end, jobs[k].kind, jobs[k].margin, jobs[k].capacity, jobs[k].top, jobs[k].nleft, jobs[k].nright, jobs[k].cut,
                  O.flags, O.nref, O.nbody, O.nwin, O.left_reach, O.right_reach, O.ref_q[0], O.ref_q[1], O.ref_q[2], O.ref_s1, O.ref_s2);
        if (sink) (*sink)[first + k] = O;
        if (O.flags != 0) continue;
        rsih::TestStats& S = stats[first + k];
        const double nb = (double)O.nbody, nw = (double)O.nwin;
        S.cnv_lqt = O.body_q[0]; S.cnv_med = O.body_q[1]; S.cnv_uqt = O.body_q[2];
        { const double mu = O.body_s1 / nb; S.cnv_var = O.body_s2 / nb - mu * mu; }
        S.ref_lqt = O.ref_q[0]; S.ref_med = O.ref_q[1]; S.ref_uqt = O.ref_q[2];
        { const double mu = O.ref_s1 / nw; S.ref_var = O.ref_s2 / nw - mu * mu; }
        left_reach[first + k] = O.left_reach;
        okv[first + k] = 1;
      }
      first += jobs.size();
    }
    return true;
  }

  bool range_sums(const std::vector<std::pair<int, int>>& ranges, std::vector<int64_t>& sums) override {
    sums.assign(ranges.size(), 0);
    if (ranges.empty()) return true;
    std::vector<int32_t> flat;
    for (const auto& r : ranges) {
      if (r.first < 0 || r.second >= N || r.second < r.first) return false;
      flat.push_back(r.first); flat.push_back(r.second);
    }
    static_assert(sizeof(long long) == sizeof(int64_t), "int64");
    const size_t fb = (flat.size() * 4 + 63) & ~size_t(63);
    unsigned char* slot = static_cast<unsigned char*>(mb_alloc(ctx, fb + ranges.size() * 8));
    GateShared gs(ctx);
    if (slot) {
      memcpy(slot, flat.data(), flat.size() * 4);
      long long* d_sums = reinterpret_cast<long long*>(slot + fb);
      { Timer t(ctx, "range_sums"); launch_range_sums(d_rdc, slot, (int)ranges.size(), d_sums, ctx->stream); }
      if (!wait()) return false;
      memcpy(sums.data(), d_sums, ranges.size() * 8);
      return true;
    }
    if (!ok(ctx->cand_chains.ensure(flat.size() * 4)) || !ok(ctx->cand_outs.ensure(ranges.size() * 8))) return false;
    if (!ok(copy_h2d(ctx, ctx->cand_chains.p, flat.data(), flat.size() * 4))) return false;
    { Timer t(ctx, "range_sums"); launch_range_sums(d_rdc, ctx->cand_chains.p, (int)ranges.size(), ctx->cand_outs.as<long long>(), ctx->stream); }
    if (!ok(copy_d2h(ctx, sums.data(), ctx->cand_outs.p, ranges.size() * 8))) return false;
    return wait();
  }

 private:
  rsi_ctx* ctx;
  DepthRef d_rdc;
  int64_t N;
  double median;
  bool ok(hipError_t e) {
    if (e == hipSuccess) return true;
    ctx->err = std::string("candidate stage: ") + hipGetErrorString(e);
    set_global_error(ctx->err);
    failed = true;
    return false;
  }
  bool wait() {
    const double t0 = now_ms();
    const bool r = ok(ctx_sync(ctx));
    kernel_wait_ms += now_ms() - t0;
    ++launches;
    return r;
  }
 public:
  bool failed = false;
};

int scan_pass(rsi_ctx* ctx, int pass, const float* d_T, const int32_t* d_medint, int64_t nb, double RDmedian, double tmedian,
              double tlamda, int Lmax, int32_t* d_status, int32_t* d_copy, const uint32_t** work_slot, const uint32_t** runs_slot,
              std::vector<uint32_t>* spill) {
  uint8_t* small = ctx->small.as<uint8_t>();
  std::vector<double> del, dup;
  scan_thresholds(tmedian, tlamda, Lmax, del, dup);
  const size_t nthr = (size_t)Lmax + 1 + kScanPad;
  ScanThr inl;
  const bool use_inl = nthr <= (size_t)kThrInline;
  double* d_del = nullptr;
  double* d_dup = nullptr;
  if (use_inl) {
    for (size_t k = 0; k < (size_t)kThrInline; ++k) { inl.del[k] = k < nthr ? del[k] : -INFINITY; inl.dup[k] = k < nthr ? dup[k] : INFINITY; }
  } else {
    HIPCHK(ctx->thr.ensure(nthr * 16));
    d_del = ctx->thr.as<double>();
    d_dup = d_del + nthr;
    del.insert(del.end(), dup.begin(), dup.end());
    HIPCHK(copy_h2d(ctx, d_del, del.data(), 2 * nthr * 8));
  }
  uint32_t* work = reinterpret_cast<uint32_t*>(small + kOffScanPass + (size_t)pass * kScanPassBytes);
  if (Lmax > kMaxL) {
    const size_t dev_bytes = (64 + 2 * (size_t)scan_level_stride(Lmax) * 4 + 255) & ~size_t(255);
    HIPCHK(ctx->scan_work_big.ensure(2 * dev_bytes));
    work = reinterpret_cast<uint32_t*>(ctx->scan_work_big.as<uint8_t>() + (size_t)pass * dev_bytes);
    HIPCHK(hipMemsetAsync(work, 0, dev_bytes, ctx->stream));
    if (pass == 0) ctx->phases.push_back({"scan.long (Lmax > 10400)", 1.0});
  }
  uint32_t* d_first_del = ctx->first_del.as<uint32_t>();
  uint32_t* d_first_dup = d_first_del + ((nb + 3) & ~int64_t(3));
  unsigned int* d_done = reinterpret_cast<unsigned int*>(small + kOffDone) + kDoneBinSlot;
  uint32_t* d_count = reinterpret_cast<uint32_t*>(small + kOffCounters) + 4;
  const size_t work_bytes = 64 + ((size_t)scan_level_stride(Lmax) + (size_t)Lmax + 1) * 4;
  if (scan_tile_workspace_bytes(Lmax)) HIPCHK(ctx->scan_ws.ensure(scan_tile_workspace_bytes(Lmax)));
  uint32_t* rslot = static_cast<uint32_t*>(mb_alloc(ctx, 8 + (size_t)kEagerBounds * 8));
  uint32_t* wslot = static_cast<uint32_t*>(work_bytes <= kMailboxBytes / 8 ? mb_alloc(ctx, work_bytes) : nullptr);
  const bool spilled = !wslot && Lmax > kMaxL && spill;
  if (spilled) spill->assign((work_bytes + 3) / 4, 0u);
  if ((!wslot && !spilled) || !rslot) return fail(ctx, RSI_ERR_INTERNAL, "out of pinned mailbox memory");
  ScanParams sp;
  sp.nb = nb; sp.Lmax = Lmax; sp.pad = 0; sp.tmedian = tmedian;
  sp.lim_del = RDmedian * 0.75; sp.lim_dup = RDmedian * 1.25;
  { Timer t(ctx, "rsi_scan"); launch_rsi_scan(d_T, d_medint, sp, d_del, d_dup, use_inl ? &inl : nullptr, d_first_del, d_first_dup, work, ctx->scan_tiles.as<uint32_t>(), ctx->scan_ws.p, ctx->stream); }
  { Timer t(ctx, "level_stop"); launch_level_stop(d_first_del, d_first_dup, nb, Lmax, work, ctx->runs.p, d_done + 2, wslot, wslot ? work_bytes : 0, ctx->stream); }
  if (spilled) { HIPCHK(hipMemcpyAsync(spill->data(), work, work_bytes, hipMemcpyDeviceToHost, ctx->stream)); wslot = spill->data(); }
  { Timer t(ctx, "resolve_runs"); launch_resolve_runs(d_first_del, d_first_dup, work + 2, nb, d_status, d_copy, ctx->runs.as<uint64_t>(), d_count, kMaxRunEntries, d_done + 3, rslot, kEagerBounds, ctx->stream); }
  *work_slot = wslot; *runs_slot = rslot;
  return RSI_OK;
}

struct SegForm { int runs = 0, items = 0, inl = 0, mailbox_status = 0, unstaged = 0; int64_t pairs_per_item = 0; };
int rsi_segments(rsi_ctx* ctx, const float* d_T, const int32_t* d_st2, int64_t nb, const std::vector<Region>& runs, double tmedian,
                 double tlamda, int64_t pairs_per_item, ScanOut& out, SegForm* form) {
  int rc;
  out.status2 = rsih::IntSpan();
  out.segs.clear();
  if (runs.empty()) return RSI_OK;
  std::vector<int64_t> poff;
  std::vector<SegItem> items;
  if (pairs_per_item <= 0) pairs_per_item = rsih::segment_pairs_per_item(runs, !ctx->gate || ctx->gate->lonely());
  rsih::segment_items(runs, pairs_per_item, poff, items);
  HIPCHK(ctx->scratch.ensure((size_t)poff.back() * 8 + (runs.size() + 1) * 8));
  double* d_scratch = ctx->scratch.as<double>();
  const bool inl = runs.size() <= (size_t)kRunsInline && items.size() <= (size_t)kItemsInline && poff.back() < (int64_t)1 << 31;
  std::vector<BestSeg> best(items.size());
  if (inl) {
    RunArgs ra;
    if ((rc = prepare_runs(ctx, runs, ra)) != RSI_OK) return rc;
    ItemsInline ii;
    memset(&ii, 0, sizeof(ii));
    for (size_t r = 0; r < runs.size(); ++r) { ra.inl.off[r] = (int32_t)poff[r]; ii.off[r] = (int32_t)poff[r]; }
    for (size_t i = 0; i < items.size(); ++i) ii.it[i] = items[i];
    BestSeg* slot = static_cast<BestSeg*>(mb_alloc(ctx, items.size() * sizeof(BestSeg)));
    if (!slot) return fail(ctx, RSI_ERR_INTERNAL, "out of pinned mailbox memory");
    const size_t run_bins = (size_t)(poff.back() - (int64_t)runs.size());
    int32_t* sslot = run_bins * 4 <= kMailboxMaxCopy ? static_cast<int32_t*>(mb_alloc(ctx, std::max<size_t>(run_bins, 1) * 4)) : nullptr;
    if (!sslot) {
      HIPCHK(ctx->h_status2.ensure((size_t)nb * 4));
      HIPCHK(hipMemcpyAsync(ctx->h_status2.p, d_st2, (size_t)nb * 4, hipMemcpyDeviceToHost, ctx->stream));
    }
    { Timer t(ctx, "run_prefix"); launch_run_prefix(d_T, nullptr, nullptr, &ra.inl, (int)runs.size(), nullptr, d_scratch, d_st2, sslot, ctx->stream); }
    { Timer t(ctx, "best_subsegment"); launch_best_items(nullptr, &ii, (int)items.size(), nullptr, d_scratch, tmedian, slot, ctx->stream); }
    HIPCHK(CTX_SYNC());
    memcpy(best.data(), slot, items.size() * sizeof(BestSeg));
    if (sslot) {
      out.run_status.assign(sslot, sslot + run_bins);
      out.run_ranges.clear();
      for (size_t r = 0; r < runs.size(); ++r) out.run_ranges.push_back({runs[r].start, runs[r].end, poff[r] - (int64_t)r});
      out.status2 = rsih::IntSpan(out.run_status.data(), nb, &out.run_ranges);
    } else {
      out.status2 = rsih::IntSpan(ctx->h_status2.as<int>(), nb);
    }
  } else {
    RunArgs ra;
    const size_t kr = runs.size();
    HIPCHK(ctx->run_se.ensure(kr * 8 + 64));
    std::vector<int32_t> se(2 * kr);
    for (size_t i = 0; i < kr; ++i) { se[i] = runs[i].start; se[kr + i] = runs[i].end; }
    HIPCHK(copy_h2d(ctx, ctx->run_se.p, se.data(), kr * 8));
    int64_t* d_poff = reinterpret_cast<int64_t*>(d_scratch + poff.back());
    HIPCHK(ctx->items.ensure(items.size() * sizeof(SegItem)));
    HIPCHK(ctx->best.ensure(items.size() * sizeof(BestSeg)));
    HIPCHK(copy_h2d(ctx, d_poff, poff.data(), poff.size() * 8));
    HIPCHK(copy_h2d(ctx, ctx->items.p, items.data(), items.size() * sizeof(SegItem)));
    HIPCHK(ctx->h_status2.ensure((size_t)nb * 4));
    HIPCHK(hipMemcpyAsync(ctx->h_status2.p, d_st2, (size_t)nb * 4, hipMemcpyDeviceToHost, ctx->stream));
    out.status2 = rsih::IntSpan(ctx->h_status2.as<int>(), nb);
    { Timer t(ctx, "run_prefix"); launch_run_prefix(d_T, ctx->run_se.as<int32_t>(), ctx->run_se.as<int32_t>() + kr, nullptr, (int)kr, d_poff, d_scratch, nullptr, nullptr, ctx->stream); }
    { Timer t(ctx, "best_subsegment"); launch_best_items(ctx->items.p, nullptr, (int)items.size(), d_poff, d_scratch, tmedian, ctx->best.as<BestSeg>(), ctx->stream); }
    HIPCHK(copy_d2h(ctx, best.data(), ctx->best.p, items.size() * sizeof(BestSeg)));
    HIPCHK(CTX_SYNC());
  }
  if (form) {
    form->runs = (int)runs.size(); form->items = (int)items.size(); form->inl = inl ? 1 : 0;
    form->mailbox_status = out.status2.ranges ? 1 : 0;
    form->pairs_per_item = pairs_per_item;
    for (const Region& r : runs) if (r.end - r.start + 2 > kBestLds) ++form->unstaged;
  }
  rsih::segments_from_best(runs, items, best.data(), out.status2, tlamda, out.segs);
  return RSI_OK;
}

struct FsForm { int runs = -1, inl = -1, copied = -1, route = 0, has_level0 = 0, trim = 0, leveldel = 0, leveladd = 0; float m0 = 0.0f; };
template <class Synced>
int rsi_filterstatus(rsi_ctx* ctx, const float* d_T, const int32_t* d_st1, int32_t* d_st1f, int64_t nb, int Lmax, double dev,
                     const uint32_t* rslot, Synced&& synced, std::vector<std::string>* fs_lines, FsForm* form) {
  int rc;
  const bool long_scan = Lmax > kMaxL;
  const int nlev = 2 * Lmax + 1;
  uint32_t* fs_slot = long_scan ? nullptr : static_cast<uint32_t*>(mb_alloc(ctx, (size_t)nlev * 8));
  if (!fs_slot && !long_scan) return fail(ctx, RSI_ERR_INTERNAL, "out of pinned mailbox memory");
  if (!long_scan) {
    GateShared gs(ctx);
    Timer t(ctx, "level_sums");
    launch_level_sums(d_T, d_st1, nb, Lmax, ctx->fs_ws.p, kMaxL, kFsListCap, ctx->fs_out.as<float>(),
                      reinterpret_cast<unsigned int*>(ctx->small.as<uint8_t>() + kOffDone) + kDoneBinSlot + 4, fs_slot, ctx->stream);
  }
  { Phase phc(ctx, "fs.wait"); HIPCHK(CTX_SYNC()); }
  if ((rc = synced()) != RSI_OK) return rc;
  {
    Phase phs(ctx, "fs.sums");
    std::vector<float> wsum((size_t)nlev, 0.0f);
    std::vector<int> wcnt((size_t)nlev, 0);
    if (fs_slot) {
      memcpy(wsum.data(), fs_slot, (size_t)nlev * 4);
      memcpy(wcnt.data(), fs_slot + nlev, (size_t)nlev * 4);
    }
    if (form) form->route = long_scan ? 2 : (wcnt[(size_t)Lmax] < 0 ? 1 : 0);
    if (long_scan || wcnt[(size_t)Lmax] < 0) {
      Phase phc(ctx, "fs.copy");
      HIPCHK(ctx->h_T.ensure((size_t)nb * 4));
      HIPCHK(ctx->h_status.ensure((size_t)nb * 4));
      HIPCHK(hipMemcpyAsync(ctx->h_T.p, d_T, (size_t)nb * 4, hipMemcpyDeviceToHost, ctx->stream));
      HIPCHK(hipMemcpyAsync(ctx->h_status.p, d_st1, (size_t)nb * 4, hipMemcpyDeviceToHost, ctx->stream));
      HIPCHK(CTX_SYNC());
      rsih::level_sums_host(ctx->h_T.as<float>(), ctx->h_status.as<int>(), nb, Lmax, wsum, wcnt);
    }
    rsih::LevelChoice lc = rsih::choose_levels(wsum, wcnt, Lmax, dev);
    phs.stop();
// ... 473 lines not shown
  K4Regions inl;
  memset(&inl, 0, sizeof(inl));
  if ((int)noncode.size() <= kRegInline) {
    for (size_t k = 0; k < ct.cbreak.size(); ++k) inl.brk[k] = ct.cbreak[k];
    for (size_t k = 0; k < ct.cum.size(); ++k) inl.cum[k] = ct.cum[k];
  } else {
    std::vector<int64_t> both((size_t)4100 + ct.cum.size(), 0);
    std::copy(ct.cbreak.begin(), ct.cbreak.end(), both.begin());
    std::copy(ct.cum.begin(), ct.cum.end(), both.begin() + 4100);
    HIPCHK(copy_h2d(ctx, d_cbreak, both.data(), both.size() * 8));
  }
  HIPCHK(ctx->rdc.ensure((size_t)(ncompact + 4) * 4));
  HIPCHK(ctx->binmed.ensure((size_t)nb * 4));
  HIPCHK(ctx->binsum.ensure((size_t)nb * 8));
  const size_t res_vals = want_cap && capval < kHistValues - 1 ? (size_t)std::max(capval, 0) + 1 : (size_t)kHistValues;
  size_t exp_bytes = kResHead + res_vals * kResClasses * 4;
  const K4Plan plan = k4_plan(P.gcadjust, want_cap, capval, P.m, ncompact, (int)noncode.size(), deep, joint_ok, sw);
  PhaseParams hpp;
  memcpy(&hpp, head + kOffPhase, sizeof(hpp));
  bool spec_done = false;
  if (spec_slot) {
    const bool ran = spec_slot[3] != kSpecMagic;
    spec_done = ran && (!P.gcadjust || (joint_ok && !deep && !jinfo.esc_pending)) && hpp.regions_ok == 1 && hpp.capval == capval &&
                hpp.nreg == (int32_t)noncode.size() && hpp.ncompact == ncompact && plan.bytes_fit && plan.shape == spec_plan.shape &&
                (int)noncode.size() <= kMaxRegions;
    if (ran && !spec_done) HIPCHK(hipMemsetAsync(ctx->hist_res.p, 0, kResHead + (size_t)256 * kResClasses * 4, st));
    ctx->phases.push_back({spec_done ? "spec.k4j accepted" : "spec.k4j rejected", 1.0});
  }
  uint32_t* exp_slot = spec_done ? spec_slot : (exp_bytes <= kMailboxMaxCopy ? static_cast<uint32_t*>(mb_alloc(ctx, exp_bytes)) : nullptr);
  if (spec_done) {
    ctx->rdc_is_bytes = true;
    for (const char* mark : spec_plan.marks)
      if (mark) ctx->phases.push_back({mark, 1.0});
  } else {
    int vbase = 0;
    if (plan.route == K4Route::wide16 || plan.route == K4Route::int32) {
      if (P.gcadjust) {
        const int rcm = materialize_rd_gc(ctx);
        if (rcm != RSI_OK) return rcm;
        d_src = ctx->rd_gc.as<int32_t>();
      }
      vbase = want_cap ? hist_window_base(S.cap_median, kK4Window) : (P.gcadjust ? hist_window_base(S.gc_rdmean, kK4Window) : 0);
      if (plan.route == K4Route::wide16 || !cap_compact_overwrites(P.m, capval, ncompact, vbase)) HIPCHK(hipMemsetAsync(d_res, 0, res_vals * kResClasses * 4, st));
      HIPCHK(ctx->slabs.ensure(plan.route == K4Route::wide16 ? cap_compact16_slab_bytes(P.m, ncompact) : cap_compact_slab_bytes(P.m, capval, ncompact, vbase)));
    } else {
      HIPCHK(ctx->slabs.ensure(cap_compact8_slab_bytes(P.m, capval, ncompact)));
      HIPCHK(ctx->rdc8.ensure((size_t)ncompact + 64));
      if (plan.route == K4Route::stream) {
        HIPCHK(ctx->slabs.ensure(rescale_compact_split_slab_bytes(capval, ncompact)));
        HIPCHK(ctx->rdc8.ensure(rescale_compact_split_rdc_bytes(ncompact)));
      }
      ctx->rdc_is_bytes = true;
    }
    for (const char* mark : plan.marks)
      if (mark) ctx->phases.push_back({mark, 1.0});
    K4Args a = k4_args(inl, (int)noncode.size(), ncompact, capval, exp_slot, exp_slot ? exp_bytes : 0);
    a.vbase = vbase;
    issue_k4(ctx, plan, a);
  }
  BinAccum bacc;
  std::vector<uint32_t> hres_all(kResHead / 4 + res_vals * kResClasses);
  if (!exp_slot) HIPCHK(copy_d2h(ctx, hres_all.data(), ctx->hist_res.p, hres_all.size() * 4));
  if (!spec_done) HIPCHK(CTX_SYNC());
  if ((joint_ok || nogc_bytes) && plan.bytes_fit) { ctx->spec_capval = capval; ctx->spec_m = P.m; ctx->spec_cap = (double)P.cap; ctx->spec_gc = P.gcadjust != 0; }
  if (exp_slot) memcpy(hres_all.data(), exp_slot, exp_bytes);
  memcpy(&bacc, hres_all.data(), sizeof(bacc));
  const uint32_t* hres = hres_all.data() + kResHead / 4;
  if (bacc.big) {
    Phase ph_h(ctx, "a6.statistics on the host (depth > 65535)");
    if (ctx->rdc_is_bytes) return fail(ctx, RSI_ERR_INTERNAL, "values beyond the histogram on the byte path");
    std::vector<int32_t> rd;
    const int rcf = fetch_i32(ctx, ctx->rdc.as<int32_t>(), ncompact, rd);
    if (rcf != RSI_OK) return rcf;
    rsih::ChromStats cs;
    rsih::array_chrom_stats(rd, cs, pb.mads);
    const double RDmed = cs.median;
    S.RDsd = cs.sd;
    S.RDmedian = RDmed;
    pb.host_stats = true;
    pb.capval = capval; pb.capped = want_cap;
    pb.ncompact = ncompact; pb.nb = nb; pb.res_vals = 0; pb.RDmedian = RDmed;
    return RSI_OK;
  }
  rsih::ChromStats cs;
  if (!rsih::hist_chrom_stats(hres, res_vals, ncompact, cs)) return fail(ctx, RSI_ERR_INTERNAL, "empty depth histogram");
  const double RDmedian = cs.median;
  S.RDsd = cs.sd;
  S.RDmedian = RDmedian;
  pb.capval = capval; pb.capped = want_cap;
  pb.ncompact = ncompact; pb.nb = nb; pb.res_vals = res_vals; pb.RDmedian = RDmedian;
  pb.hres_all = std::move(hres_all);
  return RSI_OK;
}

int bin_level_stages(rsi_ctx* ctx, const rsi_params& P, int64_t n, rsi_result* res, const PerBase& pb,
                     std::vector<Candidate>& blocks, std::vector<Candidate>& raw, std::vector<Candidate>& kept,
                     std::vector<Candidate>& segs_all) {
  rsi_chrom_stats& S = res->stats;
  uint8_t* small = ctx->small.as<uint8_t>();
  hipStream_t st = ctx->stream;
  const std::vector<Region>& noncode = pb.noncode;
  const int64_t ncompact = pb.ncompact, nb = pb.nb;
  const size_t res_vals = pb.res_vals;
  const uint32_t* hres = pb.hres_all.data() + kResHead / 4;
  const double RDmedian = pb.RDmedian;
  int rc = RSI_OK;

  if (!(RDmedian < 5)) {
    Phase ph_nb(ctx, "a9-10.mad+nb");
    GateShared gs_nb(ctx);
    double mads[31];
    const uint64_t sublen = (uint64_t)(ncompact / 31);
    if (sublen == 0) return fail(ctx, RSI_ERR_TOO_SMALL, "fewer than 31 bases");
    if (pb.host_stats) std::copy(pb.mads, pb.mads + 31, mads);
    else if (!rsih::hist_subsample_mads(hres, res_vals, RDmedian, sublen, mads)) return fail(ctx, RSI_ERR_INTERNAL, "empty MAD histogram");
    const double mad = rsih::grid_quantiles(mads, (size_t)31).med;
    const double r = RDmedian / mad;
    S.nb_mad = mad; S.nb_r = r;
    const double factor = sqrt(2.0 * (1.0 + P.epsilon) * log(3.1E9));
    const int LmaxBase = std::max(20, 10000 / P.m);

    HIPCHK(ctx->first_del.ensure((size_t)(2 * nb + 8) * 4));
    HIPCHK(ctx->status1.ensure((size_t)nb * 4));
    HIPCHK(ctx->status1f.ensure((size_t)nb * 4));
    HIPCHK(ctx->status2.ensure((size_t)nb * 4));
    HIPCHK(ctx->runs.ensure((size_t)kMaxRunEntries * 8));
    HIPCHK(ctx->scan_tiles.ensure((size_t)(nb / 256 + 2) * 4));
    HIPCHK(ctx->fs_ws.ensure(level_sums_workspace_bytes(nb, kFsListCap, kMaxL)));
    HIPCHK(ctx->fs_out.ensure((size_t)(2 * kMaxL + 1) * 8 + 64));

    GridMedian* d_g = reinterpret_cast<GridMedian*>(small + kOffGrid);
    rsih::NbLevels lev;
    NbKeyed keyed;
    const int64_t nkeys = pb.capped ? rsih::nb_key_count(P.m, pb.capval) : 0;
    if (!env_off("RSI_HOT_NB_KEYED") && rsih::nb_keyed_applies(P.trans == 0, pb.capped && pb.capval >= 0, nkeys, nb, LmaxBase > kMaxL)) {
      keyed.K = nkeys; keyed.d_binsum = ctx->binsum.as<int64_t>(); keyed.m = P.m; keyed.ncompact = ncompact; keyed.r = r; keyed.RDmedian = RDmedian;
      keyed.lev = lev = rsih::nb_reference_levels(RDmedian, P.m, r);
      ctx->phases.push_back({"nb.keyed", 1.0});
    } else {
      if ((rc = nb_transform(ctx, ctx->binsum.as<int64_t>(), nb, P.m, ncompact, RDmedian, r, lev, nullptr)) != RSI_OK) return rc;
      ctx->have_nb = true;
    }
    const double med_raw = lev.med_raw, del_raw = lev.del_raw, dup_raw = lev.dup_raw;
    bool nb_planned = true;

    ph_nb.stop();
    gs_nb.release();
    rsih::CallerInput in;
    int short_neighbourhoods = 0;
    in.short_neighbourhoods = &short_neighbourhoods;
    in.P = P; in.RDmedian = RDmedian; in.RDsd = S.RDsd; in.ncompact = ncompact; in.noncode = &noncode;
    HIPCHK(ctx->h_medint.ensure((size_t)nb * 4));
    struct CopyJoin { rsi_ctx* c; ~CopyJoin() { (void)join_copy(c); } } copy_join{ctx};
    HIPCHK(hipMemcpyAsync(ctx->h_medint.p, ctx->binmed.p, (size_t)nb * 4, hipMemcpyDeviceToHost, ctx->copy_stream));
    ctx->copy_pending = true;
    HIPCHK(hipEventRecord(ctx->copy_ev, ctx->copy_stream));
    ctx->copy_recorded = true;
    in.binmedint = rsih::IntSpan(ctx->h_medint.as<int>(), nb);

    auto do_scan = [&](bool use_med, std::vector<Candidate>& segs) -> int {
      ScanOut so;
      const float* d_T;
      ChainOut* first = nullptr;
      int rc2;
      if (use_med) {
        HIPCHK(ctx->tmed.ensure((size_t)nb * 4));
        { Timer t(ctx, "i32_to_f32"); launch_i32_to_f32_minmax(ctx->binmed.as<int32_t>(), ctx->tmed.as<float>(), nb, RDmedian, grid_chain(ctx), d_g + 1, st); }
        d_T = ctx->tmed.as<float>();
        ctx->have_med = true;
        nb_planned = false;
        if ((rc2 = grid_pair_issue(ctx, d_T, nullptr, nb, false, RDmedian, true, 0, &first)) != RSI_OK) return rc2;
      } else {
        if (keyed.K) {
          if ((rc2 = nb_keyed_issue(ctx, keyed, nullptr, nb, 0, &first)) != RSI_OK) return rc2;
          ctx->have_nb = true;
        }
        d_T = ctx->tnb.as<float>();
        if (!keyed.K && (rc2 = grid_pair_issue(ctx, d_T, nullptr, nb, true, 0.0, nb_planned, 0, &first)) != RSI_OK) return rc2;
        nb_planned = false;
      }
      rc2 = run_scan(ctx, P, use_med, d_T, nb, RDmedian, factor, LmaxBase, first, med_raw, del_raw, dup_raw, use_med ? nullptr : &keyed, so);
      if (rc2 != RSI_OK) return rc2;
      S.nb_tmin = rsih::unkey_f32(~first->rawmin_inv);
      ctx->last_scan_med = use_med;
      S.tmedian1 = so.tmedian1; S.tsigma1 = so.tsigma1; S.tlamda1 = so.tlamda1;
      S.tmedian2 = so.tmedian2; S.tsigma2 = so.tsigma2; S.tlamda2 = so.tlamda2;
      S.Lmax = so.Lmax; S.trim_escapes += (int)so.escapes; S.inexact_sums = (int)so.inexact;
      S.scan_tiles = (int32_t)((nb + 255) / 256); S.scan_tiles_listed = (int32_t)so.tiles_listed;
      for (int w = 0; w < 4; ++w) { res->level_log[w] = so.level_log[w]; res->stop_levels[w] = so.stop_levels[w]; }
      res->fs_lines = so.fs_lines;
      res->log_nb = !use_med;
      for (const Candidate& c : so.segs) segs_all.push_back(c);
      segs = so.segs;
      {
        Phase ph(ctx, "a15.blocks");
        HIPCHK(join_copy(ctx));
        DeviceTester block_tester(ctx, DepthRef{ctx->binmed.p, 4}, nb, RDmedian);
        rsih::CallProfile bprof;
        in.block_tester = env_off("RSI_HOT_BLOCK_BATCH") ? nullptr : &block_tester;
        in.prof = &bprof;
        rsih::test_block_segments(in, so.status2, segs);
        in.block_tester = nullptr;
        in.prof = nullptr;
        if (block_tester.failed) return RSI_ERR_HIP;
        if (bprof.block_batch_hits) ctx->phases.push_back({"a15.block batch hits", (double)bprof.block_batch_hits});
      }
      return RSI_OK;
    };
    std::vector<Candidate> tested;
    if (P.trans != 0) { if ((rc = do_scan(true, tested)) != RSI_OK) return rc; }
    if (P.trans == 0) { if ((rc = do_scan(false, tested)) != RSI_OK) return rc; }
    if (P.trans == 2) {
      std::vector<Candidate> more;
      if ((rc = do_scan(false, more)) != RSI_OK) return rc;
      tested.insert(tested.end(), more.begin(), more.end());
    }
    auto mirror_source = [ctx, ncompact]() -> int32_t* {
      if (materialize_rdc(ctx) != RSI_OK) return nullptr;
      if (ctx->mirror_cap < (size_t)ncompact) {
        if (ctx->mirror) (void)hipHostFree(ctx->mirror);
        ctx->mirror = nullptr;
        ctx->mirror_cap = (size_t)ncompact + (size_t)ncompact / 8 + 1024;
        if (hipHostMalloc(reinterpret_cast<void**>(&ctx->mirror), ctx->mirror_cap * sizeof(int32_t), hipHostMallocDefault) != hipSuccess) {
          ctx->mirror = nullptr; ctx->mirror_cap = 0;
        }
      }
      return ctx->mirror;
    };
    rsih::DepthPager pager(ctx->rdc.as<int32_t>(), ncompact, st, mirror_source, nullptr, 0, ctx->sync_ev);
    rsih::CallProfile prof;
    in.prof = &prof;
    const DepthRef depth_ref = ctx->rdc_is_bytes ? DepthRef{ctx->rdc8.p, 1} : DepthRef{ctx->rdc.p, 4};
    DeviceTester tester(ctx, depth_ref, ncompact, RDmedian);
    const bool host_tests = env_int("RSI_HOT_HOST_CANDIDATES", 0) != 0;
    in.tester = host_tests ? nullptr : &tester;
    { Phase ph(ctx, "a16-19.calls"); rsih::call_from_segments(in, tested, pager, blocks, raw, kept); }
    if (tester.failed) return RSI_ERR_HIP;
    if (short_neighbourhoods) return fail(ctx, RSI_ERR_UNSUPPORTED, "a candidate longer than the neighbourhood left around it (the reference aborts in isitcnv, rsi.cpp:107)");
    if (pager.failed()) return fail(ctx, RSI_ERR_INTERNAL, "no pinned host memory for the candidate stages' depth mirror");
    ctx->phases.push_back({"calls.device(wait)", tester.kernel_wait_ms});
    ctx->phases.push_back({"calls.device_ms", prof.device_ms});
    ctx->phases.push_back({"calls.final", prof.final_tests});
    ctx->phases.push_back({"calls.launches", (double)tester.launches});
    ctx->phases.push_back({"calls.spec_hits", (double)prof.spec_hits});
    ctx->phases.push_back({"calls.single_tests", (double)prof.single_tests});
    ctx->phases.push_back({"calls.host_fallbacks", (double)prof.host_fallbacks});
    ctx->phases.push_back({"calls.fetch", pager.fetch_ms()});
    ctx->phases.push_back({"calls.gather(incl fetch)", prof.gather});
    ctx->phases.push_back({"calls.winmean", prof.winmean});
    ctx->phases.push_back({"calls.quantiles", prof.quantiles});
    ctx->phases.push_back({"calls.variance", prof.variance});
    ctx->phases.push_back({"calls.sharpen", prof.sharpen});
    ctx->phases.push_back({"calls.merge(incl tests)", prof.merge});
    ctx->phases.push_back({"calls.ntests", (double)prof.tests});
  }
  return RSI_OK;
}

int run_enter(rsi_ctx* ctx, const rsi_params& P, const int32_t* d_depth, const uint8_t* d_fasta, int64_t n) {
  ctx->run_m = 0; ctx->run_rdmedian = 0.0;
  if (n <= 0 || n >= (1ll << 31) - 4096) return fail(ctx, RSI_ERR_BAD_ARG, "chromosome length must be in (0, 2^31)");
  if (P.m < 1 || (P.m % 2) != 1) return fail(ctx, RSI_ERR_BAD_ARG, "m must be odd (the reference forces it, rsi.cpp:2061-2064)");
  if (P.m > 3000) return fail(ctx, RSI_ERR_UNSUPPORTED, "bin size above 3000 is not supported by the bin kernel");
  if (((uintptr_t)d_depth & 15) || ((uintptr_t)d_fasta & 15)) return fail(ctx, RSI_ERR_BAD_ARG, "device inputs must be 16-byte aligned");
  if (P.gcadjust && n / 20 <= 201)
    return fail(ctx, RSI_ERR_TOO_SMALL, "size of RDA should be much larger than bin size (gccontent.cpp:66-71)");
  HIPCHK(hipSetDevice(ctx->device));
  ctx->ktimes.clear();
  ctx->event_next = 0;
  ctx->phases.clear();
  { const int64_t reserve = ctx->reserve_n.load(); tl_grow = reserve > n ? (double)reserve / (double)n : 1.0; }
  tl_grow_ms = 0.0;
  if (!ctx_enter(ctx)) return RSI_ERR_HIP;
  mailbox_reset(ctx);
  return RSI_OK;
}

int run_device_impl(rsi_ctx* ctx, const rsi_params* Pp, const int32_t* d_depth, const uint8_t* d_fasta, int64_t n,
                    rsi_result* res) {
  const rsi_params& P = *Pp;
  const double t_begin = now_ms();
  int rc = run_enter(ctx, P, d_depth, d_fasta, n);
  if (rc != RSI_OK) return rc;
  PerBase pb;
  rc = per_base_phase(ctx, P, d_depth, d_fasta, n, res, pb);
  if (rc != RSI_OK) return rc;
  rsi_chrom_stats& S = res->stats;
  std::vector<Candidate> blocks, raw, kept, segs_all;
  if ((rc = bin_level_stages(ctx, P, n, res, pb, blocks, raw, kept, segs_all)) != RSI_OK) return rc;
  Phase ph_fin(ctx, "z.finish");
  const std::vector<Candidate>* lists[4] = {&kept, &raw, &segs_all, &blocks};
  for (int w = 0; w < 4; ++w) {
    res->lists[w].resize(lists[w]->size());
    for (size_t i = 0; i < lists[w]->size(); ++i) to_call((*lists[w])[i], &res->lists[w][i]);
  }
  HIPCHK(CTX_SYNC());
  ph_fin.stop();
  ctx->phases.push_back({"mem.grow", tl_grow_ms});
  S.t_device_ms = now_ms() - t_begin;
  ctx->phases.push_back({"z.total", S.t_device_ms});
  if (ctx->timing) {
    double tot = 0;
    for (const KernelTime& k : ctx->ktimes) tot += elapsed_ms(k.a, k.b);
    S.t_kernels_ms = tot;
  }
  ctx->run_m = P.m; ctx->run_rdmedian = S.RDmedian;
  return RSI_OK;
}

int grid_debug_enter(rsi_ctx* ctx, int64_t nb, double* out, int32_t* info) {
  if (!ctx || !out || !info || nb <= 0 || nb >= (1ll << 31) - 4096) return fail(ctx, RSI_ERR_BAD_ARG, "bad argument");
  HIPCHK(hipSetDevice(ctx->device));
  if (!ctx_enter(ctx)) return RSI_ERR_HIP;
  mailbox_reset(ctx);
  const bool fresh = ctx->small.p == nullptr;
  HIPCHK(ctx->small.ensure(kSmallBytes));
  if (fresh) HIPCHK(hipMemsetAsync(ctx->small.p, 0, kHeaderBytes, ctx->stream));
  HIPCHK(ctx->hist_f.ensure((size_t)kGridCap * 4));
  for (int k = 0; k < 4; ++k) out[k] = 0.0;
  for (int k = 0; k < 8; ++k) info[k] = 0;
  info[0] = info[2] = info[4] = -1;
  return RSI_OK;
}
void grid_debug_record(const GridMedian& g, int32_t* info) { info[0] = (int32_t)g.flags; info[1] = (int32_t)g.np; }
int grid_debug_mad(rsi_ctx* ctx, const float* d_x, const int32_t* d_mask, int64_t nb, double center, bool planned, double* out,
                   int32_t* info) {
  ChainOut* co = nullptr;
  int rc;
  if ((rc = grid_pair_issue(ctx, d_x, d_mask, nb, false, center, planned, -1, &co)) != RSI_OK) return rc;
  HIPCHK(CTX_SYNC());
  const GridMedian g = co->g[1];
  grid_debug_record(g, info + 2);
  info[4] = hist_walk_pack16(nb) ? 1 : 0;
  double mad = 0;
  uint64_t cnt = 0;
  if (g.flags & kGridTooWide) { ++info[5]; rc = grid_median(ctx, d_x, d_mask, nb, 1, center, &mad, &cnt); }
  else rc = grid_result(ctx, g, Selection{d_x, d_mask, nb, 1, center}, &mad, &cnt);
  if (rc != RSI_OK) return rc;
  out[0] = center; out[1] = 0; out[2] = mad; out[3] = (double)cnt;
  return RSI_OK;
}
}

namespace rsip { int ensure_rd_gc(rsi_ctx* ctx) { return materialize_rd_gc(ctx); } }

extern "C" {

void rsi_default_params(rsi_params* p) {
  p->m = 101; p->gcadjust = 1; p->trans = 0; p->merge = 1; p->maxchkbp = 100000; p->debug = 0;
  p->cap = 4.0; p->epsilon = 1.5; p->threshold = -1.0; p->chklen = 2.5; p->minmlen = 3.01; p->buffer = 0.05; p->p = 0.05;
}

static hipStream_t shared_copy_stream(int device) {
  static std::mutex mu;
  static hipStream_t streams[64] = {};
  if (device < 0 || device >= 64) return nullptr;
  std::lock_guard<std::mutex> lk(mu);
  if (!streams[device] && hipStreamCreateWithFlags(&streams[device], hipStreamNonBlocking) != hipSuccess) streams[device] = nullptr;
  return streams[device];
}

rsi_ctx* rsi_hot_create(int device, int* status) {
  int count = 0;
  hipError_t e = hipGetDeviceCount(&count);
  if (e != hipSuccess || count <= 0 || device < 0 || device >= count) {
    set_global_error("no usable HIP device (librsi_hot has no CPU fallback)");
    if (status) *status = RSI_ERR_NO_DEVICE;
    return nullptr;
  }
  rsi_ctx* ctx = new rsi_ctx();
  ctx->device = device;
  if (hipSetDevice(device) != hipSuccess || hipStreamCreateWithFlags(&ctx->stream, hipStreamNonBlocking) != hipSuccess ||
      hipEventCreateWithFlags(&ctx->sync_ev, hipEventDisableTiming) != hipSuccess ||
      (ctx->copy_stream = shared_copy_stream(device)) == nullptr ||
      hipEventCreateWithFlags(&ctx->copy_ev, hipEventDisableTiming) != hipSuccess) {
    set_global_error("hipSetDevice / hipStreamCreate failed");
    if (status) *status = RSI_ERR_HIP;
    delete ctx;
    return nullptr;
  }
  if (status) *status = RSI_OK;
  return ctx;
}

void rsi_hot_destroy(rsi_ctx* ctx) {
  if (!ctx) return;
  (void)hipSetDevice(ctx->device);
  for (hipEvent_t e : ctx->event_pool) (void)hipEventDestroy(e);
  if (ctx->mirror) (void)hipHostFree(ctx->mirror);
  if (ctx->mailbox) (void)hipHostFree(ctx->mailbox);
  for (int b = 0; b < 2; ++b) if (ctx->text_pin[b]) (void)hipHostFree(ctx->text_pin[b]);
  track_free(ctx);
  depth_free(ctx);
  plot_free(ctx);
  for (int b = 0; b < 2; ++b) {
    for (hipEvent_t e : ctx->bamdev.ev[b]) if (e) (void)hipEventDestroy(e);
    if (ctx->bamdev.find[b]) (void)hipEventDestroy(ctx->bamdev.find[b]);
// ... 536 lines not shown
    rsi_cand_record& R = out[k];
    memset(&R, 0, sizeof(R));
    R.capacity = T.plan.capacity; R.top = T.plan.top; R.margin = T.plan.margin; R.cut = T.plan.cut;
    R.nleft = (int32_t)T.plan.left_chain.size(); R.nright = (int32_t)T.plan.right_chain.size();
    R.road = T.road;
    R.flags = O.flags; R.nref = O.nref; R.nbody = O.nbody; R.nwin = O.nwin; R.left_reach = O.left_reach; R.right_reach = O.right_reach;
    R.body_min = O.body_min; R.body_max = O.body_max;
    for (int q = 0; q < 3; ++q) { R.body_q[q] = O.body_q[q]; R.ref_q[q] = O.ref_q[q]; }
    R.body_s1 = O.body_s1; R.body_s2 = O.body_s2; R.ref_s1 = O.ref_s1; R.ref_s2 = O.ref_s2;
    const Candidate& c = T.judged;
    R.type = c.type; R.status = c.status; R.geno = c.geno;
    R.p1 = c.p1; R.cnvmed = c.cnvmed; R.cnvsd = c.cnvsd; R.cnviqr = c.cnviqr; R.refmed = c.refmed; R.refsd = c.refsd; R.refiqr = c.refiqr;
  }
  if (info) {
    info[0] = tester.launches; info[1] = tester.mailbox_lists; info[2] = tester.copied_lists;
    info[3] = (int32_t)mid0; info[4] = (int32_t)ctx->cand_mid.cap; info[5] = (int32_t)hist0; info[6] = (int32_t)ctx->cand_hist.cap; info[7] = 0;
  }
  return RSI_OK;
}

int rsi_hot_debug_range_sums(rsi_ctx* ctx, const int32_t* depth, int64_t n, int storage, const int32_t* lo, const int32_t* hi, int nranges,
                             int64_t* sums, int32_t* info) {
  if (!lo || !hi || !sums || nranges < 1) return fail(ctx, RSI_ERR_BAD_ARG, "bad argument");
  DepthRef ref;
  int rc;
  if ((rc = debug_depth_upload(ctx, depth, n, storage, &ref)) != RSI_OK) return rc;
  std::vector<std::pair<int, int>> ranges((size_t)nranges);
  for (int k = 0; k < nranges; ++k) ranges[(size_t)k] = {lo[k], hi[k]};
  const size_t mb_before = ctx->mb_used;
  DeviceTester tester(ctx, ref, n, 0.0);
  std::vector<int64_t> got;
  if (!tester.range_sums(ranges, got)) return tester.failed ? RSI_ERR_HIP : fail(ctx, RSI_ERR_BAD_ARG, "a range outside the array, or hi < lo");
  memcpy(sums, got.data(), (size_t)nranges * 8);
  if (info) { info[0] = tester.launches; info[1] = ctx->mb_used > mb_before ? 1 : 0; }
  return RSI_OK;
}

static Candidate list_in(const rsi_call& c) {
  Candidate k;
  k.type = c.type; k.geno = c.geno; k.status = c.status; k.start = c.start; k.end = c.end; k.length = c.length;
  k.score = c.score; k.p1 = c.p1; k.cnvmed = c.cnvmed; k.cnvsd = c.cnvsd; k.cnviqr = c.cnviqr; k.refmed = c.refmed; k.refsd = c.refsd;
  k.refiqr = c.refiqr;
  return k;
}
static void list_out(const std::vector<Candidate>& L, rsi_call* out, int32_t* count) {
  for (size_t i = 0; i < L.size(); ++i) {
    const Candidate& k = L[i];
    rsi_call& c = out[i];
    memset(&c, 0, sizeof(c));
    c.type = k.type; c.geno = k.geno; c.status = k.status; c.start = k.start; c.end = k.end; c.length = k.length;
    c.score = k.score; c.p1 = k.p1; c.cnvmed = k.cnvmed; c.cnvsd = k.cnvsd; c.cnviqr = k.cnviqr; c.refmed = k.refmed; c.refsd = k.refsd;
    c.refiqr = k.refiqr;
  }
  *count = (int32_t)L.size();
}
static bool list_params_ok(const rsi_params* P, double RDmedian, int64_t longest) {
  if (!P || P->m < 1 || P->maxchkbp < 1 || P->maxchkbp > ((1 << 30) / 10) || !(P->minmlen > 0 && P->minmlen < 1e6) ||
      !(P->chklen > 0 && P->chklen < 1e6) || !(P->buffer >= 0 && P->buffer < 1e6) || !(P->p == P->p) || !(RDmedian == RDmedian))
    return false;
  const double d = std::max({(double)longest, (double)P->m * P->minmlen, P->minmlen + 1});
  return P->chklen * d * 2 < 1073741824.0;
}
static void list_info(const rsih::CallProfile& prof, int launches, int32_t* info) {
  if (!info) return;
  info[0] = prof.spec_hits; info[1] = prof.single_tests; info[2] = prof.host_fallbacks; info[3] = prof.block_batch_hits;
  info[4] = launches; info[5] = prof.sum_launches; info[6] = prof.sum_reused; info[7] = prof.sum_redone; info[8] = prof.tests; info[9] = 0;
}
int rsi_hot_debug_block_stage(rsi_ctx* ctx, const int32_t* binmedint, const int32_t* status, int64_t nb, int64_t ncompact, double RDmedian,
                              const rsi_params* P, rsi_call* segs, int nsegs, int use_tester, int sparse, int32_t* road, int32_t* info) {
  if (!ctx || !binmedint || !status || !segs || nsegs < 1 || nb < 1 || ncompact < 1 || ncompact >= (1ll << 31) || !list_params_ok(P, RDmedian, nb))
    return fail(ctx, RSI_ERR_BAD_ARG, "bad argument");
  for (int64_t i = 0; i < nb; ++i) if (binmedint[i] < 0) return fail(ctx, RSI_ERR_BAD_ARG, "a negative bin median");
  std::vector<Candidate> L((size_t)nsegs);
  for (int i = 0; i < nsegs; ++i) {
    if (segs[i].start < 0 || segs[i].end < segs[i].start || segs[i].end >= nb) return fail(ctx, RSI_ERR_BAD_ARG, "a segment must lie inside the bins, start <= end");
    if (segs[i].type != rsih::kDel && segs[i].type != rsih::kDup) return fail(ctx, RSI_ERR_BAD_ARG, "a segment's type must be DEL or DUP");
    L[(size_t)i] = list_in(segs[i]);
  }
  std::vector<int> run_status;
  std::vector<rsih::IntSpan::Range> run_ranges;
  if (sparse) {
    for (int64_t i = 0; i < nb;) {
      if (status[i] == 0) { ++i; continue; }
      int64_t j = i;
      while (j + 1 < nb && status[j + 1] != 0) ++j;
      run_ranges.push_back({i, j, (int64_t)run_status.size()});
      run_status.insert(run_status.end(), status + i, status + j + 1);
      i = j + 1;
    }
    if (run_ranges.empty()) return fail(ctx, RSI_ERR_BAD_ARG, "the sparse form needs a marked run");
  }
  DepthRef ref;
  int rc;
  if ((rc = debug_depth_upload(ctx, binmedint, nb, 4, &ref)) != RSI_OK) return rc;
  rsih::CallerInput in{};
  in.P = *P;
  in.RDmedian = RDmedian; in.RDsd = 0; in.ncompact = ncompact; in.noncode = nullptr;
  in.binmedint = rsih::IntSpan(binmedint, nb);
  rsih::CallProfile prof;
  int short_neighbourhoods = 0;
  std::vector<int> roads;
  in.prof = &prof; in.short_neighbourhoods = &short_neighbourhoods; in.block_roads = &roads;
  DeviceTester tester(ctx, ref, nb, RDmedian);
  tester.force_split = 1; tester.force_bytes = 1;
  in.block_tester = use_tester ? &tester : nullptr;
  const rsih::IntSpan st = sparse ? rsih::IntSpan(run_status.data(), nb, &run_ranges) : rsih::IntSpan(status, nb);
  rsih::test_block_segments(in, st, L);
  if (tester.failed) return RSI_ERR_HIP;
  if (short_neighbourhoods) return fail(ctx, RSI_ERR_UNSUPPORTED, "a segment longer than the neighbourhood left around it");
  int32_t count = 0;
  list_out(L, segs, &count);
  if (road) for (int i = 0; i < nsegs; ++i) road[i] = roads[(size_t)i];
  list_info(prof, tester.launches, info);
  return RSI_OK;
}

static int base_list(rsi_ctx* ctx, const rsi_call* list, int nlist, int64_t n, std::vector<Candidate>& L) {
  L.resize((size_t)nlist);
  for (int i = 0; i < nlist; ++i) {
    if (list[i].start < 0 || list[i].end < list[i].start || list[i].end >= n) return fail(ctx, RSI_ERR_BAD_ARG, "a candidate must lie inside the array, start <= end");
    if (list[i].type != rsih::kDel && list[i].type != rsih::kDup) return fail(ctx, RSI_ERR_BAD_ARG, "a candidate's type must be DEL or DUP");
    L[(size_t)i] = list_in(list[i]);
  }
  return RSI_OK;
}

int rsi_hot_debug_merge(rsi_ctx* ctx, const int32_t* depth, int64_t n, int storage, double RDmedian, const rsi_params* P, const rsi_call* list,
                        int nlist, int use_tester, rsi_call* out, int32_t* nout, int32_t* info) {
  if (!ctx || !depth || !list || !out || !nout || nlist < 1 || n < 1 || !list_params_ok(P, RDmedian, n)) return fail(ctx, RSI_ERR_BAD_ARG, "bad argument");
  for (int64_t i = 0; i < n; ++i) if (depth[i] < 0) return fail(ctx, RSI_ERR_BAD_ARG, "a negative depth");
  std::vector<Candidate> L;
  int rc;
  if ((rc = base_list(ctx, list, nlist, n, L)) != RSI_OK) return rc;
  DepthRef ref;
  if ((rc = debug_depth_upload(ctx, depth, n, storage, &ref)) != RSI_OK) return rc;
  rsih::CallerInput in{};
  in.P = *P;
  in.RDmedian = RDmedian; in.RDsd = 0; in.ncompact = n; in.noncode = nullptr;
  rsih::CallProfile prof;
  int short_neighbourhoods = 0;
  in.prof = &prof; in.short_neighbourhoods = &short_neighbourhoods;
  DeviceTester tester(ctx, ref, n, RDmedian);
  tester.force_split = 1; tester.force_bytes = 1;
  in.tester = use_tester ? &tester : nullptr;
  rsih::DepthPager pager(depth, n);
  rsih::debug_merge_neighbours(in, pager, L);
  if (tester.failed) return RSI_ERR_HIP;
  if (short_neighbourhoods) return fail(ctx, RSI_ERR_UNSUPPORTED, "a candidate longer than the neighbourhood left around it");
  list_out(L, out, nout);
  list_info(prof, tester.launches, info);
  return RSI_OK;
}

int rsi_hot_debug_calls(rsi_ctx* ctx, const int32_t* depth, int64_t n, int storage, double RDmedian, double RDsd, const rsi_params* P,
                        const rsi_call* segs, int nsegs, const int32_t* noncode_start, const int32_t* noncode_end, int nnoncode, int use_tester,
                        rsi_call* blocks, rsi_call* raw, rsi_call* kept, int32_t* counts, int32_t* info) {
  if (!ctx || !depth || !segs || !blocks || !raw || !kept || !counts || nsegs < 1 || n < 1 || nnoncode < 0 || (nnoncode > 0 && (!noncode_start || !noncode_end)) ||
      !(RDsd == RDsd) || !list_params_ok(P, RDmedian, n))
    return fail(ctx, RSI_ERR_BAD_ARG, "bad argument");
  for (int64_t i = 0; i < n; ++i) if (depth[i] < 0) return fail(ctx, RSI_ERR_BAD_ARG, "a negative depth");
  std::vector<Candidate> S((size_t)nsegs);
  for (int i = 0; i < nsegs; ++i) {
    if (segs[i].start < 0 || segs[i].end < segs[i].start || (int64_t)segs[i].start * P->m + P->m / 2 > n - 1 || (int64_t)segs[i].end * P->m + P->m / 2 >= (1ll << 31))
      return fail(ctx, RSI_ERR_BAD_ARG, "a segment must start inside the array, start <= end");
    if (segs[i].type != rsih::kDel && segs[i].type != rsih::kDup) return fail(ctx, RSI_ERR_BAD_ARG, "a segment's type must be DEL or DUP");
    S[(size_t)i] = list_in(segs[i]);
  }
  std::vector<Region> noncode((size_t)nnoncode);
  for (int i = 0; i < nnoncode; ++i) {
    if (noncode_start[i] < 0 || noncode_end[i] <= noncode_start[i] || (i > 0 && noncode_start[i] <= noncode_end[i - 1]))
      return fail(ctx, RSI_ERR_BAD_ARG, "the regions must be sorted, disjoint and longer than one base");
    noncode[(size_t)i] = Region{noncode_start[i], noncode_end[i]};
  }
  DepthRef ref;
  int rc;
  if ((rc = debug_depth_upload(ctx, depth, n, storage, &ref)) != RSI_OK) return rc;
  rsih::CallerInput in{};
  in.P = *P;
  in.RDmedian = RDmedian; in.RDsd = RDsd; in.ncompact = n; in.noncode = &noncode;
  rsih::CallProfile prof;
  int short_neighbourhoods = 0;
  in.prof = &prof; in.short_neighbourhoods = &short_neighbourhoods;
  DeviceTester tester(ctx, ref, n, RDmedian);
  tester.force_split = 1; tester.force_bytes = 1;
  in.tester = use_tester ? &tester : nullptr;
  rsih::DepthPager pager(depth, n);
  std::vector<Candidate> B, R, K;
  rsih::call_from_segments(in, S, pager, B, R, K);
  if (tester.failed) return RSI_ERR_HIP;
  if (short_neighbourhoods) return fail(ctx, RSI_ERR_UNSUPPORTED, "a candidate longer than the neighbourhood left around it");
  list_out(B, blocks, &counts[0]);
  list_out(R, raw, &counts[1]);
  list_out(K, kept, &counts[2]);
  list_info(prof, tester.launches, info);
  return RSI_OK;
}

}
int rsip::geno_run(rsi_ctx* ctx, const void* d_depth, int storage, int64_t ncompact, const std::vector<rsigeno::Ranges>& lines, int tile,
                    double chrom_median, rsi_geno_record* out) {
  rsi_ctx::Geno& G = ctx->geno;
  const int64_t bytes_held = G.stats.bytes;
  G.stats = rsi_geno_stats{};
  G.stats.bytes = bytes_held;
  if (lines.empty()) return RSI_OK;
  if (lines.size() > (size_t)(1 << 29)) return fail(ctx, RSI_ERR_UNSUPPORTED, "geno: more than 2^29 lines in one batch");
  const double t0 = now_ms();
  std::vector<rsigeno::Tile> tiles;
  if (!rsigeno::build_tiles(lines, ncompact, tile > 0 ? tile : rsigeno::kDefaultTile, tiles)) return fail(ctx, RSI_ERR_BAD_ARG, "geno: a range outside the array, or hi < lo");
  if (tiles.size() >= (size_t)0x7fffffff) return fail(ctx, RSI_ERR_UNSUPPORTED, "geno: more than 2^31 tiles in one batch");
  static_assert(sizeof(rsigeno::Tile) == sizeof(GenoTile), "one tile layout for the host table and the kernels");
  const int njobs = (int)(2 * lines.size()), ntiles = (int)tiles.size();
  const size_t hist_bytes = geno_hist_bytes(storage, njobs);
  HIPCHK(G.tiles.ensure(std::max<size_t>(tiles.size(), 1) * sizeof(GenoTile)));
  HIPCHK(G.hist.ensure(hist_bytes));
  HIPCHK(G.out.ensure((size_t)njobs * sizeof(GenoOut)));
  if (storage != 1) HIPCHK(G.state.ensure((size_t)njobs * sizeof(GenoState) + 256));
  G.stats.bytes = (int64_t)(G.tiles.cap + G.hist.cap + G.out.cap + G.state.cap);
  hipStream_t st = ctx->stream;
  if (ntiles) HIPCHK(copy_h2d(ctx, G.tiles.p, tiles.data(), tiles.size() * sizeof(GenoTile)));
  HIPCHK(hipMemsetAsync(G.hist.p, 0, hist_bytes, st));
  const GenoTile* d_tiles = G.tiles.as<GenoTile>();
  unsigned int* d_hist = G.hist.as<unsigned int>();
  GenoOut* d_out = G.out.as<GenoOut>();
  int launches = 0, passes = 0;
  if (storage == 1) {
    { Timer t(ctx, "geno_hist"); launch_geno_hist8(static_cast<const uint8_t*>(d_depth), d_tiles, ntiles, d_hist, st); }
    { Timer t(ctx, "geno_scan"); launch_geno_scan8(d_hist, njobs, d_out, st); }
    launches = (ntiles ? 1 : 0) + 1; passes = 1;
  } else {
    GenoState* d_st = G.state.as<GenoState>();
    unsigned int* d_bits = reinterpret_cast<unsigned int*>(G.state.as<uint8_t>() + (size_t)njobs * sizeof(GenoState));
    const int32_t* d32 = static_cast<const int32_t*>(d_depth);
    { Timer t(ctx, "geno_minmax"); launch_geno_init32(d_st, njobs, d_bits, st); launch_geno_minmax32(d32, d_tiles, ntiles, d_st, st); launch_geno_plan32(d_st, njobs, d_out, d_bits, st); }
    launches = 2 + (ntiles ? 1 : 0);
    unsigned int maxbits = 0;
    HIPCHK(copy_d2h(ctx, &maxbits, d_bits, 4));
    HIPCHK(CTX_SYNC());
    passes = (int)((maxbits + kGenoBits - 1) / kGenoBits);
    for (int p = 0; p < passes; ++p) {
      { Timer t(ctx, "geno_hist"); launch_geno_hist32(d32, d_tiles, ntiles, d_st, d_hist, st); }
      { Timer t(ctx, "geno_scan"); launch_geno_scan32(d_st, njobs, d_hist, d_out, st); }
      launches += 2;
    }
  }
  std::vector<GenoOut> got((size_t)njobs);
  HIPCHK(copy_d2h(ctx, got.data(), d_out, (size_t)njobs * sizeof(GenoOut)));
  HIPCHK(CTX_SYNC());
  for (size_t i = 0; i < lines.size(); ++i) {
    const GenoOut& b = got[2 * i], & f = got[2 * i + 1];
    rsi_geno_record& r = out[i];
    memset(&r, 0, sizeof(r));
    r.n_body = b.n; r.n_flank = f.n; r.body_min = b.vmin; r.body_max = b.vmax; r.body_sum = b.sum; r.flank_sum = f.sum;
    for (int q = 0; q < 3; ++q) { r.body_q[q] = b.q[q]; r.flank_q[q] = f.q[q]; }
    r.chrom_median = chrom_median;
  }
  G.stats.launches = launches; G.stats.jobs = njobs; G.stats.tiles = ntiles; G.stats.passes = passes;
  G.stats.ms = now_ms() - t0;
  return RSI_OK;
}
extern "C" {

int rsi_hot_geno_calls(rsi_ctx* ctx, int m, int ncalls, const int32_t* start, const int32_t* end, rsi_geno_record* out) {
  if (!ctx || ncalls < 0 || m < 1 || (ncalls > 0 && (!start || !end || !out))) return fail(ctx, RSI_ERR_BAD_ARG, "bad argument");
  if (!ctx->run_m || ctx->ncompact <= 0 || !(ctx->rdc_is_bytes ? ctx->rdc8.p : ctx->rdc.p))
    return fail(ctx, RSI_ERR_BAD_ARG, "geno: the context holds no successful run's compacted depth (none yet, the last one failed, or a debug hook has overwritten it)");
  HIPCHK(hipSetDevice(ctx->device));
  if (!ctx_enter(ctx)) return RSI_ERR_HIP;
  mailbox_reset(ctx);
  const int npairs = (int)(ctx->noncode_pairs.size() / 2);
  std::vector<rsigeno::Ranges> lines((size_t)ncalls);
  for (int i = 0; i < ncalls; ++i)
    lines[(size_t)i] = rsigeno::line_ranges(rsigeno::map_line(start[i], end[i], ctx->n, ctx->noncode_pairs.data(), npairs), m, ctx->ncompact);
  return geno_run(ctx, ctx->rdc_is_bytes ? ctx->rdc8.p : ctx->rdc.p, ctx->rdc_is_bytes ? 1 : 4, ctx->ncompact, lines, 0, ctx->run_rdmedian, out);
}

int rsi_hot_last_geno_stats(const rsi_ctx* ctx, rsi_geno_stats* out) {
  if (!ctx || !out) return RSI_ERR_BAD_ARG;
  *out = ctx->geno.stats;
  return RSI_OK;
}

int rsi_hot_debug_geno(rsi_ctx* ctx, const int32_t* depth, int64_t n, int storage, const int32_t* lo, const int32_t* hi, const int32_t* flo0,
                       const int32_t* fhi0, const int32_t* flo1, const int32_t* fhi1, int njobs, int tile, rsi_geno_record* out) {
  if (njobs < 0 || tile < 0 || (njobs > 0 && (!lo || !hi || !flo0 || !fhi0 || !flo1 || !fhi1 || !out))) return fail(ctx, RSI_ERR_BAD_ARG, "bad argument");
  DepthRef ref;
  int rc;
  if ((rc = debug_depth_upload(ctx, depth, n, storage, &ref)) != RSI_OK) return rc;
  std::vector<rsigeno::Ranges> lines((size_t)njobs);
  for (int i = 0; i < njobs; ++i) {
    rsigeno::Ranges& r = lines[(size_t)i];
    r.body.a = lo[i]; r.body.b = hi[i]; r.left.a = flo0[i]; r.left.b = fhi0[i]; r.right.a = flo1[i]; r.right.b = fhi1[i];
  }
  return geno_run(ctx, ref.p, storage, n, lines, tile, 0.0, out);
}

int rsi_hot_debug_grid_median(rsi_ctx* ctx, const float* x, const int32_t* mask, int64_t nb, int mode, double center, double* out,
                              int32_t* info) {
  int rc;
  if (!x || mode < 0 || mode > 2) return fail(ctx, RSI_ERR_BAD_ARG, "bad argument");
  if ((rc = grid_debug_enter(ctx, nb, out, info)) != RSI_OK) return rc;
  HIPCHK(ctx->tnb.ensure((size_t)nb * 4));
  HIPCHK(hipMemcpyAsync(ctx->tnb.p, x, (size_t)nb * 4, hipMemcpyHostToDevice, ctx->stream));
  ctx->have_nb = false;
  const int32_t* d_mask = nullptr;
  if (mask) {
    HIPCHK(ctx->status1f.ensure((size_t)nb * 4));
    HIPCHK(hipMemcpyAsync(ctx->status1f.p, mask, (size_t)nb * 4, hipMemcpyHostToDevice, ctx->stream));
    d_mask = ctx->status1f.as<int32_t>();
  }
  const float* d_x = ctx->tnb.as<float>();
  if (mode == 1) return grid_debug_mad(ctx, d_x, d_mask, nb, center, false, out, info);
  double med = 0, mad = 0;
  uint64_t c0 = 0, c1 = 0;
  if (mode == 2) {
    info[5] = 2;
    if ((rc = grid_median(ctx, d_x, d_mask, nb, 0, 0.0, &med, &c0)) != RSI_OK) return rc;
    if ((rc = grid_median(ctx, d_x, d_mask, nb, 1, med, &mad, &c1)) != RSI_OK) return rc;
  } else {
    ChainOut* co = nullptr;
    if ((rc = grid_pair_issue(ctx, d_x, d_mask, nb, true, 0.0, false, -1, &co)) != RSI_OK) return rc;
    HIPCHK(CTX_SYNC());
    const GridMedian g0 = co->g[0], g1 = co->g[1];
    grid_debug_record(g0, info);
    grid_debug_record(g1, info + 2);
    info[4] = hist_walk_pack16(nb) ? 1 : 0;
    if ((g0.flags | g1.flags) & kGridTooWide) {
      info[5] = 2;
      if ((rc = grid_median(ctx, d_x, d_mask, nb, 0, 0.0, &med, &c0)) != RSI_OK) return rc;
      if ((rc = grid_median(ctx, d_x, d_mask, nb, 1, med, &mad, &c1)) != RSI_OK) return rc;
    } else {
      if ((rc = grid_result(ctx, g0, Selection{d_x, d_mask, nb, 0, 0.0}, &med, &c0)) != RSI_OK) return rc;
      if (g0.flags & kGridDegenerate) { info[5] = 1; rc = grid_median(ctx, d_x, d_mask, nb, 1, med, &mad, &c1); }
      else rc = grid_result(ctx, g1, Selection{d_x, d_mask, nb, 1, med}, &mad, &c1);
      if (rc != RSI_OK) return rc;
    }
  }
  out[0] = med; out[1] = (double)c0; out[2] = mad; out[3] = (double)c1;
  return RSI_OK;
}

int rsi_hot_debug_nb_keyed(rsi_ctx* ctx, const int64_t* binsum, const int32_t* mask, int64_t nb, int m, int64_t K, double RDmedian, double r,
                           float* T, double* out, int32_t* info) {
  int rc;
  if (!ctx || !binsum || !T || m < 1 || !(r > 0.0) || nb < 3) return fail(ctx, RSI_ERR_BAD_ARG, "bad argument");
  if ((rc = grid_debug_enter(ctx, nb, out, info)) != RSI_OK) return rc;
  info[0] = info[2] = -1; info[4] = 0;
  ctx->ktimes.clear(); ctx->event_next = 0; ctx->phases.clear();
// ... 193 lines not shown
```

### rsicnv_amd/csrc/pipeline_steps.h

```cpp
#pragma once
#include <math.h>
#include <stdio.h>
#include <string.h>
#include <algorithm>
#include <string>
#include <vector>
#include "host_calls.h"
#include "hostmath.h"
#include "kernels.h"

namespace rsih {

inline bool boundary_pairs(const uint64_t* raw, size_t cnt, bool end_exclusive, std::vector<Region>& out) {
  out.clear();
  std::vector<int64_t> s, e;
  for (size_t i = 0; i < cnt; ++i) { const uint64_t v = raw[i]; ((v & 1) ? e : s).push_back((int64_t)(v >> 1)); }
  if (s.size() != e.size()) return false;
  std::sort(s.begin(), s.end());
  std::sort(e.begin(), e.end());
  for (size_t i = 0; i < s.size(); ++i) out.push_back({(int)s[i], (int)(e[i] - (end_exclusive ? 1 : 0))});
  return true;
}

inline float unkey_f32(uint32_t k) {
  const uint32_t b = (k & 0x80000000u) ? (k & 0x7fffffffu) : ~k;
  float f;
  memcpy(&f, &b, 4);
  return f;
}

inline std::vector<Region> noncode_regions(const std::vector<Region>& nruns, int64_t n, int dx) {
  std::vector<Region> noncode;
  for (const Region& r : nruns) {
    Region g{std::max(0, r.start - dx), (int)std::min<int64_t>(n - 1, (int64_t)r.end + dx)};
    if (!noncode.empty() && g.start <= noncode.back().end + 1) noncode.back().end = std::max(noncode.back().end, g.end);
    else noncode.push_back(g);
  }
  return noncode;
}
struct CompactTable { std::vector<int64_t> cbreak, cum; int64_t ncompact = 0; };
inline CompactTable compact_table(const std::vector<Region>& noncode, int64_t n) {
  CompactTable t;
  t.cbreak.resize(noncode.size());
  t.cum.assign(noncode.size() + 1, 0);
  for (size_t k = 0; k < noncode.size(); ++k) {
    t.cbreak[k] = (int64_t)noncode[k].start - t.cum[k];
    t.cum[k + 1] = t.cum[k] + (noncode[k].end - noncode[k].start + 1);
  }
  t.ncompact = n - t.cum.back();
  return t;
}

struct CapMedian { double med; bool beyond; };
inline CapMedian cap_median(const rsik::ValueMedian& vm, int64_t n) {
  CapMedian c;
  c.med = (double)vm.lo;
  if (vm.lo <= vm.hi && (double)vm.hi - (double)vm.lo >= 1.0 && vm.med >= 0) c.med = (double)vm.med;
  c.beyond = (uint64_t)n / 2 > vm.inrange;
  return c;
}
inline int32_t cap_value(double med, double cap) { return (int32_t)(med * cap); }

struct ChromStats { double median = 0, sd = 0; };
inline bool hist_chrom_stats(const uint32_t* hres, size_t res_vals, int64_t ncompact, ChromStats& out) {
  std::vector<uint64_t> hall(res_vals, 0);
  for (size_t v = 0; v < res_vals; ++v) for (int c = 0; c < rsik::kResClasses; ++c) hall[v] += hres[v * rsik::kResClasses + c];
  Quantiles qall;
  if (!hist_quantiles_int(hall.data(), hall.size(), (uint64_t)ncompact, qall)) return false;
  out.median = qall.med;
  {
    unsigned __int128 s1 = 0, s2 = 0;
    for (size_t v = 0; v < res_vals; ++v) { s1 += (unsigned __int128)v * hall[v]; s2 += (unsigned __int128)v * v * hall[v]; }
    const double d1 = (double)s1, d2 = (double)s2;
    const double mean = d1 / double((int)ncompact);
    out.sd = sqrt(d2 / double((int)ncompact) - mean * mean);
  }
  return true;
}
inline bool hist_subsample_mads(const uint32_t* hres, size_t res_vals, double RDmedian, uint64_t sublen, double mads[31]) {
  for (int j = 0; j < 31; ++j) {
    std::vector<uint64_t> hd(res_vals + 1, 0);
    for (size_t v = 0; v < res_vals; ++v) {
      const uint32_t c = hres[v * rsik::kResClasses + j];
      if (!c) continue;
      const int a = (int)fabs((float)(int)v - RDmedian);
      hd[(size_t)a] += c;
    }
    Quantiles qd;
    if (!hist_quantiles_int(hd.data(), hd.size(), sublen, qd)) return false;
    mads[j] = qd.med;
  }
  return true;
}
inline double rank_value_i32(std::vector<int32_t>& v, uint64_t rank) {
  if (v.empty()) return 0.0;
  const auto mm = std::minmax_element(v.begin(), v.end());
  const int32_t lo = *mm.first, hi = *mm.second;
  if ((double)hi - (double)lo < 1.0 || rank == 0) return (double)lo;
  const size_t k = (size_t)std::min<uint64_t>(rank, v.size()) - 1;
  std::nth_element(v.begin(), v.begin() + k, v.end());
  return (double)v[k];
}
inline void array_chrom_stats(const std::vector<int32_t>& rd, ChromStats& out, double mads[31]) {
  const int64_t ncompact = (int64_t)rd.size();
  out.sd = sqrt(variance_pop(rd.data(), (size_t)ncompact));
  const uint64_t sublen = (uint64_t)(ncompact / 31);
  std::vector<int32_t> sub((size_t)sublen);
  std::vector<int32_t> sorted = rd;
  const double RDmed = rank_value_i32(sorted, (uint64_t)ncompact / 2);
  for (int j = 0; j < 31 && sublen > 0; ++j) {
    for (uint64_t k = 0; k < sublen; ++k) sub[(size_t)k] = (int)fabs((float)rd[(size_t)(j + 31 * k)] - RDmed);
    mads[j] = rank_value_i32(sub, sublen / 2);
  }
  out.median = RDmed;
}

struct NbLevels { double med_raw, del_raw, dup_raw; };
inline NbLevels nb_reference_levels(double RDmedian, int m, double r) {
  auto nbf = [&](double sum) {
    const double mm = (double)m;
    return 2.0 * sqrt(r) * log(sqrt((sum + 0.25) / (mm * r - 0.5)) + sqrt(1.0 + (sum + 0.25) / (mm * r - 0.5)));
  };
  return NbLevels{nbf(RDmedian * m), nbf(RDmedian / 2.0 * (double)m), nbf(RDmedian * 1.5 * (double)m)};
}
struct NbScaled { float t0, t2; };
inline NbScaled nb_scaled_levels(double tmin, double nb_med_raw, double nb_del_raw, double RDmedian) {
  const double med_nbt = nb_med_raw - tmin;
  return NbScaled{(float)((nb_del_raw - tmin) / med_nbt * RDmedian), (float)(med_nbt / med_nbt * RDmedian)};
}

constexpr int64_t kNbKeyLimit = 1 << 15;
inline int64_t nb_key_count(int m, int32_t capval) { return (int64_t)m * (int64_t)capval + 1; }
inline bool nb_keyed_applies(bool nb_route, bool capped, int64_t K, int64_t nb, bool long_scan) {
  return nb_route && capped && K >= 1 && K <= kNbKeyLimit && nb >= 8 && !long_scan;
}

struct Lamda { double tsigma, tlamda; };
inline Lamda lamda_from_mad(double absmed, double factor, double target) {
  Lamda l;
  l.tsigma = absmed / 0.6745;
  l.tlamda = factor * l.tsigma;
  l.tlamda = std::max(l.tlamda, target);
  return l;
}
struct ScanSetup { double tsigma, tlamda, target, dev; int cal_max, Lmax_ref, Lmax; bool clipped; };
inline ScanSetup scan_first_pass(bool use_med, double tmedian, double absmed, double factor, int LmaxBase, float t0, float t2,
                                 double threshold, int64_t nb) {
  ScanSetup s;
  if (!use_med) {
    s.target = (t2 - t0) * sqrt(2.5);
    const Lamda l = lamda_from_mad(absmed, factor, s.target);
    s.tsigma = l.tsigma; s.tlamda = l.tlamda;
    const double dnb = fabsf(t2 - t0) + 0.0001;
    const double q = s.tlamda * 2 / dnb;
    s.cal_max = (int)(q * q);
    s.dev = s.tsigma * 3.0;
  } else {
    s.target = tmedian * sqrt(2.0);
    const Lamda l = lamda_from_mad(absmed, factor, s.target);
    s.tsigma = l.tsigma; s.tlamda = l.tlamda;
    if (threshold > 0) s.tlamda = tmedian * threshold;
    const double q = s.tlamda * 4 / (tmedian + 0.001);
    s.cal_max = (int)(q * q);
    s.dev = tmedian * 0.6;
  }
  s.Lmax = LmaxBase;
  if (s.Lmax < s.cal_max) s.Lmax = s.cal_max;
  s.Lmax_ref = s.Lmax;
  s.clipped = s.Lmax > nb;
  if (s.clipped) s.Lmax = (int)nb;
  return s;
}

struct ScanRecord {
  const uint32_t* w;
  int Lmax;
  uint32_t escapes() const { return w[rsik::kScanRecEscapes]; }
  uint32_t inexact() const { return w[rsik::kScanRecInexact]; }
  uint32_t stop_level(int sweep) const { return w[rsik::kScanRecStop + sweep]; }
  uint32_t tiles_listed() const { return w[rsik::kScanRecTiles]; }
  const uint32_t* level_counts(int sweep) const { return w + rsik::kScanRecLevels + (size_t)sweep * rsik::scan_level_stride(Lmax); }
  bool sweeps_stopped(int64_t nb) const {
    for (int k = 0; k < 2; ++k) {
      const uint32_t* cnt = level_counts(k);
      uint64_t cum = 0;
      for (uint32_t L = 0; L <= stop_level(k) && L <= (uint32_t)Lmax; ++L) cum += cnt[L];
      if (!((double)(int)cum / (double)(int)nb > 0.2)) return false;
    }
    return true;
  }
};

inline void level_sums_host(const float* tv, const int* st, int64_t nb, int Lmax, std::vector<float>& wsum, std::vector<int>& wcnt) {
  std::fill(wsum.begin(), wsum.end(), 0.0f);
  std::fill(wcnt.begin(), wcnt.end(), 0);
  float s0 = 0.0f;
  int n0 = 0;
  for (int64_t i = 0; i < nb; ++i) {
    const int sv = st[i];
    if (sv == 0) { s0 += tv[i]; ++n0; }
    else { wsum[(size_t)(sv + Lmax)] += tv[i]; ++wcnt[(size_t)(sv + Lmax)]; }
  }
  wsum[(size_t)Lmax] = s0; wcnt[(size_t)Lmax] = n0;
}
struct LevelChoice {
  bool has_level0 = false, trim = false;
  int lo = 0, hi = 0, leveldel = 0, leveladd = 0;
  float m0 = 0.0f;
  std::vector<std::string> lines;
};
inline LevelChoice choose_levels(const std::vector<float>& wsum, const std::vector<int>& wcnt, int Lmax, double dev) {
  LevelChoice c;
  int lo = 0, hi = 0;
  { int a = 0, b = 2 * Lmax; while (a < b && wcnt[a] == 0) ++a; while (b > a && wcnt[b] == 0) --b; lo = a - Lmax; hi = b - Lmax; }
  const int nl = hi - lo + 1;
  std::vector<float> lsum(wsum.begin() + (lo + Lmax), wsum.begin() + (hi + Lmax + 1));
  std::vector<int> lcnt(wcnt.begin() + (lo + Lmax), wcnt.begin() + (hi + Lmax + 1));
  for (int l = 0; l < nl; ++l) if (lcnt[l] != 0) lsum[l] /= (double)lcnt[l];
  c.lo = lo; c.hi = hi;
  if (!(lo <= 0 && -lo < nl)) return c;
  c.has_level0 = true;
  const float m0 = lsum[-lo];
  int leveldel = lo, leveladd = hi;
  for (int l = 0; l < nl; ++l) if (lsum[l] < m0 - dev) { leveldel = l + lo; break; }
  for (int l = nl - 1; l >= 0; --l) if (lsum[l] > m0 + dev) { leveladd = l + lo; break; }
  char line[128];
  for (int l = 0; l < nl; ++l) if (lcnt[l] != 0) { snprintf(line, sizeof(line), "%d\t%d\t%g", l + lo, lcnt[l], (double)lsum[l]); c.lines.push_back(line); }
  snprintf(line, sizeof(line), "%d\t%g", leveldel, (double)lsum[leveldel - lo]); c.lines.push_back(line);
  snprintf(line, sizeof(line), "%d\t%g", leveladd, (double)lsum[leveladd - lo]); c.lines.push_back(line);
  c.trim = !(leveldel > 0 || leveladd < 0 || leveldel > leveladd);
  if (!c.trim) c.lines.push_back("warning level error, status not filtered");
  c.m0 = m0; c.leveldel = leveldel; c.leveladd = leveladd;
  return c;
}

inline int64_t segment_pairs_per_item(const std::vector<Region>& runs, bool lonely) {
  int64_t pairs_per_item = 1 << 16;
  if (lonely) {
    int64_t total = 0;
    for (const Region& r : runs) { const int64_t len = r.end - r.start + 1; total += len * (len + 1) / 2; }
    const int64_t room = std::max<int64_t>(8, (int64_t)rsik::kItemsInline - 2 * (int64_t)runs.size());
    pairs_per_item = std::min<int64_t>(pairs_per_item, std::max<int64_t>(1 << 13, total / room + 1));
  }
  return pairs_per_item;
}
inline void segment_items(const std::vector<Region>& runs, int64_t pairs_per_item, std::vector<int64_t>& poff, std::vector<rsik::SegItem>& items) {
  poff.assign(runs.size() + 1, 0);
  items.clear();
  for (size_t r = 0; r < runs.size(); ++r) {
    const int len = runs[r].end - runs[r].start + 1;
    poff[r + 1] = poff[r] + len + 1;
    int L = 1;
    while (L <= len) {
      int64_t pairs = 0; int Le = L;
      while (Le <= len && pairs < pairs_per_item) { pairs += len - Le + 1; ++Le; }
      items.push_back({(int32_t)r, (int32_t)len, (int32_t)L, (int32_t)Le});
      L = Le;
    }
  }
}
inline void segments_from_best(const std::vector<Region>& runs, const std::vector<rsik::SegItem>& items, const rsik::BestSeg* best,
                               const IntSpan& status2, double tlamda, std::vector<Candidate>& segs) {
  std::vector<rsik::BestSeg> per_run(runs.size(), rsik::BestSeg{-1.0, 0, 0});
  for (size_t i = 0; i < items.size(); ++i) {
    rsik::BestSeg& b = per_run[(size_t)items[i].run];
    if (best[i].score > b.score) b = best[i];
  }
  for (size_t r = 0; r < runs.size(); ++r) {
    Candidate c;
    const int len = runs[r].end - runs[r].start + 1;
    double sc = per_run[r].score;
    if (sc > 0) { c.start = runs[r].start + per_run[r].start; c.end = c.start + per_run[r].len - 1; }
    else { c.start = runs[r].start; c.end = runs[r].start + len - 1; sc = 0; }
    const Quantiles q = grid_quantiles(status2.at(c.start), (size_t)(c.end - c.start + 1));
    if (q.med > 0) { c.type = kDup; c.score = sc; } else { c.type = kDel; c.score = -sc; }
    if (fabs(c.score) < tlamda * 0.5) continue;
    segs.push_back(c);
  }
}

}
```

Baseline: 281.3 billion.

## Issue speculative edge sharpening early and speed host scan threshold search

```diff
diff --git a/include/rsi_hot.h b/include/rsi_hot.h
--- a/include/rsi_hot.h
+++ b/include/rsi_hot.h
@@ -358,6 +358,9 @@
 int rsi_hot_debug_calls(rsi_ctx* ctx, const int32_t* depth, int64_t n, int storage, double RDmedian, double RDsd, const rsi_params* P,
                         const rsi_call* segs, int nsegs, const int32_t* noncode_start, const int32_t* noncode_end, int nnoncode, int use_tester,
                         rsi_call* blocks, rsi_call* raw, rsi_call* kept, int32_t* counts, int32_t* info);
+int rsi_hot_debug_calls_spec(rsi_ctx* ctx, const int32_t* depth, int64_t n, int storage, double RDmedian, double RDsd, const rsi_params* P,
+                             const rsi_call* segs, int nsegs, const int32_t* noncode_start, const int32_t* noncode_end, int nnoncode, int alter,
+                             rsi_call* blocks, rsi_call* raw, rsi_call* kept, int32_t* counts, int32_t* info, int32_t* spec_info);
 int rsi_hot_debug_nb_transform(rsi_ctx* ctx, const int64_t* binsum, int64_t nb, int m, int64_t ncompact, double RDmedian, double r,
                                float* raw, float* T, int32_t* info);
 int rsi_hot_debug_filterstatus(rsi_ctx* ctx, const float* T, const int32_t* status, int64_t nb, int Lmax, double dev, int32_t* status_out,
diff --git a/rsicnv_amd/api.py b/rsicnv_amd/api.py
--- a/rsicnv_amd/api.py
+++ b/rsicnv_amd/api.py
@@ -57,7 +57,7 @@
            "rsi_hot_run_device", "rsi_hot_load_depth_text", "rsi_hot_run_text", "rsi_hot_load_depth_bam", "rsi_hot_run_bam", "rsi_bam_references", "rsi_result_annotate_bam", "rsi_result_summary", "rsi_summary_format_row", "rsi_summary_format_rows", "rsi_result_pairs", "rsi_result_ncalls", "rsi_result_calls", "rsi_result_stats", "rsi_result_noncode",
            "rsi_result_format_row", "rsi_result_free", "rsi_hot_fetch_i32", "rsi_hot_fetch_f32", "rsi_hot_fetch_i64",
            "rsi_hot_kernel_times", "rsi_hot_phase_times", "rsi_hot_set_timing", "rsi_hot_process_setup", "rsi_pool_create", "rsi_pool_destroy", "rsi_pool_workers", "rsi_pool_hw_queues", "rsi_pool_worker",
-           "rsi_pool_set_timing", "rsi_pool_set_timing_kernel", "rsi_hot_set_timing_kernel", "rsi_pool_set_schedule", "rsi_pool_last_error", "rsi_pool_run", "rsi_pool_run_host", "rsi_pool_submit", "rsi_pool_wait", "rsi_plot_expand", "rsi_plot_write_files", "rsi_result_log_line", "rsi_hot_debug_level_sums", "rsi_hot_debug_scan", "rsi_hot_debug_segments", "rsi_hot_debug_sharpen", "rsi_hot_debug_candidate_tests", "rsi_hot_debug_range_sums", "rsi_hot_debug_block_stage", "rsi_hot_debug_merge", "rsi_hot_debug_calls", "rsi_hot_debug_nb_transform", "rsi_hot_debug_nb_keyed", "rsi_hot_debug_filterstatus", "rsi_hot_debug_grid_median", "rsi_hot_debug_grid_mad_i32", "rsi_synth_generate_host", "rsi_synth_generate_device", "rsi_synth_write_depth_text", "rsi_synth_write_fasta", "rsi_synth_append_genome_text",
+           "rsi_pool_set_timing", "rsi_pool_set_timing_kernel", "rsi_hot_set_timing_kernel", "rsi_pool_set_schedule", "rsi_pool_last_error", "rsi_pool_run", "rsi_pool_run_host", "rsi_pool_submit", "rsi_pool_wait", "rsi_plot_expand", "rsi_plot_write_files", "rsi_result_log_line", "rsi_hot_debug_level_sums", "rsi_hot_debug_scan", "rsi_hot_debug_segments", "rsi_hot_debug_sharpen", "rsi_hot_debug_candidate_tests", "rsi_hot_debug_range_sums", "rsi_hot_debug_block_stage", "rsi_hot_debug_merge", "rsi_hot_debug_calls", "rsi_hot_debug_calls_spec", "rsi_hot_debug_nb_transform", "rsi_hot_debug_nb_keyed", "rsi_hot_debug_filterstatus", "rsi_hot_debug_grid_median", "rsi_hot_debug_grid_mad_i32", "rsi_synth_generate_host", "rsi_synth_generate_device", "rsi_synth_write_depth_text", "rsi_synth_write_fasta", "rsi_synth_append_genome_text",
            "rsi_genome_text_open", "rsi_genome_text_next", "rsi_genome_text_release", "rsi_genome_text_copy_depth",
            "rsi_genome_text_kernel_ms", "rsi_genome_text_close", "rsi_genome_text_last_error", "rsi_hot_run_depth_device",
            "rsi_hot_last_inflate_stats", "rsi_hot_inflate_bgzf", "rsi_genome_text_inflate_stats",
@@ -802,6 +802,26 @@
                                                  info.ctypes.data))
         return outs[0][:counts[0]], outs[1][:counts[1]], outs[2][:counts[2]], dict(zip(LIST_INFO, (int(v) for v in info)))
 
+    def debug_calls_spec(self, depth, storage, segs, noncode, RDmedian, RDsd, alter=-1, **params):
+        d = np.ascontiguousarray(depth, dtype=np.int32)
+        L = np.ascontiguousarray(np.array(segs, dtype=CALL_RECORD).reshape(-1))
+        nc = np.asarray(noncode, dtype=np.int32).reshape(-1, 2)
+        a, b = np.ascontiguousarray(nc[:, 0]), np.ascontiguousarray(nc[:, 1])
+        outs = [np.zeros(max(L.size, 1), dtype=CALL_RECORD) for _ in range(3)]
+        counts = np.zeros(3, dtype=np.int32)
+        info = np.zeros(10, dtype=np.int32)
+        spec = np.zeros(3, dtype=np.int32)
+        P = make_params(**params)
+        self.lib.rsi_hot_debug_calls_spec.argtypes = [C.c_void_p, C.c_void_p, C.c_int64, C.c_int, C.c_double, C.c_double, C.c_void_p, C.c_void_p, C.c_int,
+                                                      C.c_void_p, C.c_void_p, C.c_int, C.c_int, C.c_void_p, C.c_void_p, C.c_void_p, C.c_void_p, C.c_void_p,
+                                                      C.c_void_p]
+        self._check(self.lib.rsi_hot_debug_calls_spec(self.ctx, d.ctypes.data, d.size, int(storage), float(RDmedian), float(RDsd), C.addressof(P),
+                                                      L.ctypes.data, L.size, a.ctypes.data if a.size else None, b.ctypes.data if b.size else None, a.size,
+                                                      int(alter), outs[0].ctypes.data, outs[1].ctypes.data, outs[2].ctypes.data, counts.ctypes.data,
+                                                      info.ctypes.data, spec.ctypes.data))
+        return (outs[0][:counts[0]], outs[1][:counts[1]], outs[2][:counts[2]], dict(zip(LIST_INFO, (int(v) for v in info))),
+                tuple(int(v) for v in spec))
+
     def debug_nb_transform(self, binsum, m, ncompact, RDmedian, r):
         b = np.ascontiguousarray(binsum, dtype=np.int64)
         raw = np.zeros(b.size, dtype=np.float32)
diff --git a/rsicnv_amd/csrc/host_calls.cpp b/rsicnv_amd/csrc/host_calls.cpp
--- a/rsicnv_amd/csrc/host_calls.cpp
+++ b/rsicnv_amd/csrc/host_calls.cpp
@@ -700,16 +700,32 @@
   blocks = segs;
   std::vector<Candidate> L;
   for (Candidate c : segs) {
-    if (c.geno == 0 || c.start == c.end) continue;
-    c.start = c.start * m + m / 2;
-    c.end = c.end * m + m / 2;
-    if (c.start < 0) c.start = 0;
-    if (c.end > np - 1) c.end = np - 1;
-    c.length = c.end - c.start + 1;
+    if (c.geno == 0 || !bins_to_bases(c, m, np)) continue;
     L.push_back(c);
   }
   const double ts0 = tick_ms();
-  if (!(in.tester && in.tester->sharpen(L)))
+  if (in.tester && in.sharpen_spec && !in.sharpen_spec->empty()) {
+    auto key_less = [](const SharpenRecord& a, const SharpenRecord& b) {
+      return a.start != b.start ? a.start < b.start : a.end != b.end ? a.end < b.end : a.type < b.type;
+    };
+    std::vector<SharpenRecord> rec = *in.sharpen_spec;
+    std::sort(rec.begin(), rec.end(), key_less);
+    std::vector<size_t> miss;
+    for (size_t i = 0; i < L.size(); ++i) {
+      const SharpenRecord k{L[i].start, L[i].end, L[i].type, 0, 0};
+      const auto it = std::lower_bound(rec.begin(), rec.end(), k, key_less);
+      if (it != rec.end() && !key_less(k, *it)) { L[i].start = it->new_start; L[i].end = it->new_end; }
+      else miss.push_back(i);
+    }
+    if (in.prof) { in.prof->sharpen_spec_hits += (int)(L.size() - miss.size()); in.prof->sharpen_spec_misses += (int)miss.size(); }
+    if (!miss.empty()) {
+      std::vector<Candidate> M;
+      for (size_t i : miss) M.push_back(L[i]);
+      if (!in.tester->sharpen(M))
+        for (int pass = 0; pass < 2; ++pass) for (Candidate& c : M) sharpen_edges(bases, c);
+      for (size_t k = 0; k < miss.size(); ++k) L[miss[k]] = M[k];
+    }
+  } else if (!(in.tester && in.tester->sharpen(L)))
     for (int pass = 0; pass < 2; ++pass) for (Candidate& c : L) sharpen_edges(bases, c);
   order_by_start(L);
   const double ts1 = tick_ms();
diff --git a/rsicnv_amd/csrc/host_calls.h b/rsicnv_amd/csrc/host_calls.h
--- a/rsicnv_amd/csrc/host_calls.h
+++ b/rsicnv_amd/csrc/host_calls.h
@@ -56,6 +56,7 @@
 struct CallProfile {
   double fetch = 0, gather = 0, winmean = 0, quantiles = 0, variance = 0, sharpen = 0, merge = 0, final_tests = 0, device_ms = 0;
   int tests = 0, spec_hits = 0, single_tests = 0, host_fallbacks = 0, block_batch_hits = 0;
+  int sharpen_spec_hits = 0, sharpen_spec_misses = 0;
   int sum_launches = 0, sum_reused = 0, sum_redone = 0;
 };
 
@@ -67,10 +68,14 @@
   std::vector<std::pair<int, int>> left_chain, right_chain;
 };
 
+struct SharpenRecord { int start, end, type, new_start, new_end; };
+
 class NeighbourTester {
  public:
   virtual ~NeighbourTester() {}
   virtual bool sharpen(std::vector<Candidate>& L) = 0;
+  virtual bool sharpen_issue(const std::vector<Candidate>& L, int max_jobs) { (void)L; (void)max_jobs; return false; }
+  virtual bool sharpen_collect(std::vector<SharpenRecord>& out) { (void)out; return true; }
   virtual bool test(const std::vector<TestPlan>& plans, std::vector<TestStats>& stats, std::vector<int>& left_reach,
                     std::vector<char>& ok) = 0;
   virtual bool range_sums(const std::vector<std::pair<int, int>>& ranges, std::vector<int64_t>& sums) = 0;
@@ -106,9 +111,28 @@
   int64_t ncompact;
   const std::vector<Region>* noncode;
   IntSpan binmedint;
+  const std::vector<SharpenRecord>* sharpen_spec = nullptr;
   int* short_neighbourhoods = nullptr;
   std::vector<int>* block_roads = nullptr;
 };
+
+inline bool bins_to_bases(Candidate& c, int m, int np) {
+  if (c.start == c.end) return false;
+  c.start = c.start * m + m / 2;
+  c.end = c.end * m + m / 2;
+  if (c.start < 0) c.start = 0;
+  if (c.end > np - 1) c.end = np - 1;
+  c.length = c.end - c.start + 1;
+  return true;
+}
+inline std::vector<Candidate> sharpen_spec_jobs(const std::vector<Candidate>& segs, int m, int np) {
+  std::vector<Candidate> J;
+  for (Candidate c : segs) {
+    if (c.start > c.end) std::swap(c.start, c.end);
+    if (bins_to_bases(c, m, np)) J.push_back(c);
+  }
+  return J;
+}
 
 void test_block_segments(const CallerInput& in, IntSpan status, std::vector<Candidate>& segs);
 
diff --git a/rsicnv_amd/csrc/hostmath.h b/rsicnv_amd/csrc/hostmath.h
--- a/rsicnv_amd/csrc/hostmath.h
+++ b/rsicnv_amd/csrc/hostmath.h
@@ -160,4 +160,44 @@
   return hi.d;
 }
 
-}
+union DoubleBits { double d; uint64_t u; };
+template <class Pred>
+double last_true_from(double guess, Pred pred) {
+  if (!pred(0.0)) return -1.0;
+  DoubleBits lo, hi, mid;
+  lo.d = 0.0; hi.d = INFINITY;
+  if (pred(hi.d)) return INFINITY;
+  if (guess >= 0.0 && guess < INFINITY) {
+    DoubleBits g;
+    g.d = guess == 0.0 ? 0.0 : guess;
+    if (pred(g.d)) {
+      lo = g;
+      for (uint64_t step = 1;; step *= 2) {
+        if (step >= hi.u - lo.u) break;
+        mid.u = lo.u + step;
+        if (pred(mid.d)) lo = mid; else { hi = mid; break; }
+      }
+    } else {
+      hi = g;
+      for (uint64_t step = 1;; step *= 2) {
+        if (step >= hi.u - lo.u) break;
+        mid.u = hi.u - step;
+        if (pred(mid.d)) { lo = mid; break; } else hi = mid;
+      }
+    }
+  }
+  while (hi.u - lo.u > 1) {
+    mid.u = lo.u + (hi.u - lo.u) / 2;
+    if (pred(mid.d)) lo = mid; else hi = mid;
+  }
+  return lo.d;
+}
+template <class Pred>
+double first_true_from(double guess, Pred pred) {
+  const double below = last_true_from(guess, [&](double s) { return !pred(s); });
+  if (below < 0.0) return 0.0;
+  if (below == INFINITY) return INFINITY;
+  return nextafter(below, INFINITY);
+}
+
+}
diff --git a/rsicnv_amd/csrc/pipeline.hip b/rsicnv_amd/csrc/pipeline.hip
--- a/rsicnv_amd/csrc/pipeline.hip
+++ b/rsicnv_amd/csrc/pipeline.hip
@@ -172,18 +172,6 @@
   return RSI_OK;
 }
 
-void scan_thresholds(double tmedian, double tlamda, int Lmax, std::vector<double>& del, std::vector<double>& dup) {
-  del.assign((size_t)Lmax + 1 + kScanPad, -INFINITY);
-  dup.assign((size_t)Lmax + 1 + kScanPad, INFINITY);
-  del[0] = -1.0;
-  for (int L = 1; L <= Lmax; ++L) {
-    const double dL = (double)L, sq = sqrt(dL);
-    auto score = [&](double sum) { const float meanf = (float)(sum / dL); return ((double)meanf - tmedian) * sq; };
-    del[L] = rsih::last_true([&](double s) { return !(score(s) > -tlamda); });
-    dup[L] = rsih::first_true([&](double s) { return !(score(s) < tlamda); });
-  }
-}
-
 constexpr uint32_t kEagerBounds = 1024;
 int runs_from_export(rsi_ctx* ctx, const uint32_t* slot, const uint64_t* d_list, std::vector<Region>& runs) {
   const uint32_t cnt = slot[0];
@@ -230,14 +218,20 @@
   std::vector<CandOut>* sink = nullptr;
   int mailbox_lists = 0, copied_lists = 0;
 
-  bool sharpen(std::vector<Candidate>& L) override {
-    if (L.empty()) return true;
+  struct EdgeBatch { EdgeJob* jobs = nullptr; int nj = 0; std::vector<EdgeJob> keys, spill; };
+  std::vector<EdgeBatch> edge_batches;
+  ~DeviceTester() override { if (!edge_batches.empty()) (void)ctx_sync(ctx); }
+
+  bool issue_edges(const std::vector<Candidate>& L, bool mailbox_only) {
     const int nj = (int)L.size();
     EdgeJob* slot = static_cast<EdgeJob*>(mb_alloc(ctx, (size_t)nj * sizeof(EdgeJob)));
-    std::vector<EdgeJob> spill;
-    EdgeJob* jobs = slot;
-    if (!slot) { spill.resize((size_t)nj); jobs = spill.data(); }
-    for (int i = 0; i < nj; ++i) jobs[i] = {L[(size_t)i].start, L[(size_t)i].end, L[(size_t)i].type, 0};
+    if (!slot && mailbox_only) return false;
+    EdgeBatch b;
+    b.nj = nj;
+    b.keys.resize((size_t)nj);
+    if (!slot) b.spill.resize((size_t)nj);
+    EdgeJob* jobs = slot ? slot : b.spill.data();
+    for (int i = 0; i < nj; ++i) jobs[i] = b.keys[(size_t)i] = {L[(size_t)i].start, L[(size_t)i].end, L[(size_t)i].type, 0};
     {
       Phase ph(ctx, "cand.ensure");
       if (nj > ctx->sharpen_ws_jobs) {
@@ -248,7 +242,6 @@
       }
       if (!slot && !ok(ctx->cand_jobs.ensure((size_t)nj * sizeof(EdgeJob)))) return false;
     }
-    GateShared gs(ctx);
     Phase ph(ctx, "cand.sharpen");
     EdgeJob* d_jobs = slot ? slot : ctx->cand_jobs.as<EdgeJob>();
     if (!slot && !ok(copy_h2d(ctx, ctx->cand_jobs.p, jobs, (size_t)nj * sizeof(EdgeJob)))) return false;
@@ -257,9 +250,35 @@
       launch_sharpen_edges(d_rdc, N, d_jobs, nj, ctx->sharpen_ws.p, ctx->sharpen_ws_jobs, ctx->stream);
     }
     if (!slot && !ok(copy_d2h(ctx, jobs, ctx->cand_jobs.p, (size_t)nj * sizeof(EdgeJob)))) return false;
-    if (!wait()) return false;
+    b.jobs = jobs;
+    edge_batches.push_back(std::move(b));
+    return true;
+  }
+  static constexpr int kSharpenSpecJobs = 1024;
+  bool sharpen_issue(const std::vector<Candidate>& L, int max_jobs) override {
+    if (L.empty() || (int)L.size() > std::min(max_jobs, kSharpenSpecJobs) || ctx->gate_shared) return false;
+    for (const Candidate& c : L) if ((int64_t)c.end - c.start >= (1 << 28)) return false;
+    return issue_edges(L, true);
+  }
+  bool sharpen_collect(std::vector<rsih::SharpenRecord>& out) override {
+    if (edge_batches.empty()) return true;
+    Phase ph(ctx, "cand.sharpen");
+    const bool r = wait();
+    if (r)
+      for (const EdgeBatch& b : edge_batches)
+        for (int i = 0; i < b.nj; ++i) out.push_back({b.keys[(size_t)i].start, b.keys[(size_t)i].end, b.keys[(size_t)i].type, b.jobs[i].start, b.jobs[i].end});
+    edge_batches.clear();
+    return r;
+  }
+  bool sharpen(std::vector<Candidate>& L) override {
+    if (L.empty()) return true;
+    GateShared gs(ctx);
+    if (!issue_edges(L, false)) return false;
+    std::vector<rsih::SharpenRecord> rec;
+    if (!sharpen_collect(rec)) return false;
     gs.release();
-    for (int i = 0; i < nj; ++i) { L[(size_t)i].start = jobs[i].start; L[(size_t)i].end = jobs[i].end; }
+    const size_t first = rec.size() - L.size();
+    for (size_t i = 0; i < L.size(); ++i) { L[i].start = rec[first + i].new_start; L[i].end = rec[first + i].new_end; }
     return true;
   }
 
@@ -423,7 +442,9 @@
               std::vector<uint32_t>* spill) {
   uint8_t* small = ctx->small.as<uint8_t>();
   std::vector<double> del, dup;
-  scan_thresholds(tmedian, tlamda, Lmax, del, dup);
+  static const bool thr_bisect = env_on("RSI_HOT_THR_BISECT");
+  if (thr_bisect) rsih::scan_thresholds_bisect(tmedian, tlamda, Lmax, del, dup);
+  else rsih::scan_thresholds(tmedian, tlamda, Lmax, del, dup);
   const size_t nthr = (size_t)Lmax + 1 + kScanPad;
   ScanThr inl;
   const bool use_inl = nthr <= (size_t)kThrInline;
@@ -1203,11 +1224,25 @@
     in.P = P; in.RDmedian = RDmedian; in.RDsd = S.RDsd; in.ncompact = ncompact; in.noncode = &noncode;
     HIPCHK(ctx->h_medint.ensure((size_t)nb * 4));
     struct CopyJoin { rsi_ctx* c; ~CopyJoin() { (void)join_copy(c); } } copy_join{ctx};
-    HIPCHK(hipMemcpyAsync(ctx->h_medint.p, ctx->binmed.p, (size_t)nb * 4, hipMemcpyDeviceToHost, ctx->copy_stream));
-    ctx->copy_pending = true;
-    HIPCHK(hipEventRecord(ctx->copy_ev, ctx->copy_stream));
-    ctx->copy_recorded = true;
+    bool copy_issued = false;
+    auto issue_copy = [&]() -> int {
+      if (copy_issued) return RSI_OK;
+      copy_issued = true;
+      HIPCHK(hipMemcpyAsync(ctx->h_medint.p, ctx->binmed.p, (size_t)nb * 4, hipMemcpyDeviceToHost, ctx->copy_stream));
+      ctx->copy_pending = true;
+      HIPCHK(hipEventRecord(ctx->copy_ev, ctx->copy_stream));
+      ctx->copy_recorded = true;
+      return RSI_OK;
+    };
+    static const bool copy_first = env_on("RSI_HOT_COPY_FIRST");
+    if (copy_first && (rc = issue_copy()) != RSI_OK) return rc;
     in.binmedint = rsih::IntSpan(ctx->h_medint.as<int>(), nb);
+
+    const DepthRef depth_ref = ctx->rdc_is_bytes ? DepthRef{ctx->rdc8.p, 1} : DepthRef{ctx->rdc.p, 4};
+    DeviceTester tester(ctx, depth_ref, ncompact, RDmedian);
+    const bool host_tests = env_int("RSI_HOT_HOST_CANDIDATES", 0) != 0;
+    static const int sharpen_spec_jobs = env_int("RSI_HOT_SHARPEN_SPEC", DeviceTester::kSharpenSpecJobs);
+    bool sharpen_issued = false;
 
     auto do_scan = [&](bool use_med, std::vector<Candidate>& segs) -> int {
       ScanOut so;
@@ -1230,8 +1265,13 @@
         if (!keyed.K && (rc2 = grid_pair_issue(ctx, d_T, nullptr, nb, true, 0.0, nb_planned, 0, &first)) != RSI_OK) return rc2;
         nb_planned = false;
       }
+      if ((rc2 = issue_copy()) != RSI_OK) return rc2;
       rc2 = run_scan(ctx, P, use_med, d_T, nb, RDmedian, factor, LmaxBase, first, med_raw, del_raw, dup_raw, use_med ? nullptr : &keyed, so);
       if (rc2 != RSI_OK) return rc2;
+      if (!host_tests && sharpen_spec_jobs > 0) {
+        if (tester.sharpen_issue(rsih::sharpen_spec_jobs(so.segs, P.m, (int)ncompact), sharpen_spec_jobs)) sharpen_issued = true;
+        if (tester.failed) return RSI_ERR_HIP;
+      }
       S.nb_tmin = rsih::unkey_f32(~first->rawmin_inv);
       ctx->last_scan_med = use_med;
       S.tmedian1 = so.tmedian1; S.tsigma1 = so.tsigma1; S.tlamda1 = so.tlamda1;
@@ -1281,11 +1321,18 @@
     rsih::DepthPager pager(ctx->rdc.as<int32_t>(), ncompact, st, mirror_source, nullptr, 0, ctx->sync_ev);
     rsih::CallProfile prof;
     in.prof = &prof;
-    const DepthRef depth_ref = ctx->rdc_is_bytes ? DepthRef{ctx->rdc8.p, 1} : DepthRef{ctx->rdc.p, 4};
-    DeviceTester tester(ctx, depth_ref, ncompact, RDmedian);
-    const bool host_tests = env_int("RSI_HOT_HOST_CANDIDATES", 0) != 0;
     in.tester = host_tests ? nullptr : &tester;
-    { Phase ph(ctx, "a16-19.calls"); rsih::call_from_segments(in, tested, pager, blocks, raw, kept); }
+    std::vector<rsih::SharpenRecord> sharpen_spec;
+    {
+      Phase ph(ctx, "a16-19.calls");
+      if (sharpen_issued) {
+        const double t0 = now_ms();
+        if (!tester.sharpen_collect(sharpen_spec)) return RSI_ERR_HIP;
+        prof.sharpen += now_ms() - t0;
+        in.sharpen_spec = &sharpen_spec;
+      }
+      rsih::call_from_segments(in, tested, pager, blocks, raw, kept);
+    }
     if (tester.failed) return RSI_ERR_HIP;
     if (short_neighbourhoods) return fail(ctx, RSI_ERR_UNSUPPORTED, "a candidate longer than the neighbourhood left around it (the reference aborts in isitcnv, rsi.cpp:107)");
     if (pager.failed()) return fail(ctx, RSI_ERR_INTERNAL, "no pinned host memory for the candidate stages' depth mirror");
@@ -1294,6 +1341,8 @@
     ctx->phases.push_back({"calls.final", prof.final_tests});
     ctx->phases.push_back({"calls.launches", (double)tester.launches});
     ctx->phases.push_back({"calls.spec_hits", (double)prof.spec_hits});
+    ctx->phases.push_back({"calls.sharpen_spec_hits", (double)prof.sharpen_spec_hits});
+    ctx->phases.push_back({"calls.sharpen_spec_misses", (double)prof.sharpen_spec_misses});
     ctx->phases.push_back({"calls.single_tests", (double)prof.single_tests});
     ctx->phases.push_back({"calls.host_fallbacks", (double)prof.host_fallbacks});
     ctx->phases.push_back({"calls.fetch", pager.fetch_ms()});
@@ -2136,9 +2185,9 @@
   return RSI_OK;
 }
 
-int rsi_hot_debug_calls(rsi_ctx* ctx, const int32_t* depth, int64_t n, int storage, double RDmedian, double RDsd, const rsi_params* P,
-                        const rsi_call* segs, int nsegs, const int32_t* noncode_start, const int32_t* noncode_end, int nnoncode, int use_tester,
-                        rsi_call* blocks, rsi_call* raw, rsi_call* kept, int32_t* counts, int32_t* info) {
+static int debug_calls_impl(rsi_ctx* ctx, const int32_t* depth, int64_t n, int storage, double RDmedian, double RDsd, const rsi_params* P,
+                            const rsi_call* segs, int nsegs, const int32_t* noncode_start, const int32_t* noncode_end, int nnoncode, int use_tester,
+                            rsi_call* blocks, rsi_call* raw, rsi_call* kept, int32_t* counts, int32_t* info, bool spec, int alter, int32_t* spec_info) {
   if (!ctx || !depth || !segs || !blocks || !raw || !kept || !counts || nsegs < 1 || n < 1 || nnoncode < 0 || (nnoncode > 0 && (!noncode_start || !noncode_end)) ||
       !(RDsd == RDsd) || !list_params_ok(P, RDmedian, n))
     return fail(ctx, RSI_ERR_BAD_ARG, "bad argument");
@@ -2170,6 +2219,13 @@
   in.tester = use_tester ? &tester : nullptr;
   rsih::DepthPager pager(depth, n);
   std::vector<Candidate> B, R, K;
+  std::vector<rsih::SharpenRecord> records;
+  if (spec && use_tester) {
+    const bool issued = tester.sharpen_issue(rsih::sharpen_spec_jobs(S, P->m, (int)n), DeviceTester::kSharpenSpecJobs);
+    if (tester.failed || (issued && !tester.sharpen_collect(records))) return RSI_ERR_HIP;
+    if (alter >= 0 && alter < (int)records.size()) records[(size_t)alter].start += 1;
+    in.sharpen_spec = &records;
+  }
   rsih::call_from_segments(in, S, pager, B, R, K);
   if (tester.failed) return RSI_ERR_HIP;
   if (short_neighbourhoods) return fail(ctx, RSI_ERR_UNSUPPORTED, "a candidate longer than the neighbourhood left around it");
@@ -2177,7 +2233,21 @@
   list_out(R, raw, &counts[1]);
   list_out(K, kept, &counts[2]);
   list_info(prof, tester.launches, info);
-  return RSI_OK;
+  if (spec_info) { spec_info[0] = (int32_t)records.size(); spec_info[1] = prof.sharpen_spec_hits; spec_info[2] = prof.sharpen_spec_misses; }
+  return RSI_OK;
+}
+int rsi_hot_debug_calls(rsi_ctx* ctx, const int32_t* depth, int64_t n, int storage, double RDmedian, double RDsd, const rsi_params* P,
+                        const rsi_call* segs, int nsegs, const int32_t* noncode_start, const int32_t* noncode_end, int nnoncode, int use_tester,
+                        rsi_call* blocks, rsi_call* raw, rsi_call* kept, int32_t* counts, int32_t* info) {
+  return debug_calls_impl(ctx, depth, n, storage, RDmedian, RDsd, P, segs, nsegs, noncode_start, noncode_end, nnoncode, use_tester, blocks, raw, kept,
+                          counts, info, false, -1, nullptr);
+}
+int rsi_hot_debug_calls_spec(rsi_ctx* ctx, const int32_t* depth, int64_t n, int storage, double RDmedian, double RDsd, const rsi_params* P,
+                             const rsi_call* segs, int nsegs, const int32_t* noncode_start, const int32_t* noncode_end, int nnoncode, int alter,
+                             rsi_call* blocks, rsi_call* raw, rsi_call* kept, int32_t* counts, int32_t* info, int32_t* spec_info) {
+  if (!spec_info) return fail(ctx, RSI_ERR_BAD_ARG, "bad argument");
+  return debug_calls_impl(ctx, depth, n, storage, RDmedian, RDsd, P, segs, nsegs, noncode_start, noncode_end, nnoncode, 1, blocks, raw, kept, counts,
+                          info, true, alter, spec_info);
 }
 
 }
diff --git a/rsicnv_amd/csrc/pipeline_steps.h b/rsicnv_amd/csrc/pipeline_steps.h
--- a/rsicnv_amd/csrc/pipeline_steps.h
+++ b/rsicnv_amd/csrc/pipeline_steps.h
@@ -170,6 +170,49 @@
   s.clipped = s.Lmax > nb;
   if (s.clipped) s.Lmax = (int)nb;
   return s;
+}
+
+inline void scan_thresholds_bisect(double tmedian, double tlamda, int Lmax, std::vector<double>& del, std::vector<double>& dup,
+                                   uint64_t* evals = nullptr) {
+  del.assign((size_t)Lmax + 1 + rsik::kScanPad, -INFINITY);
+  dup.assign((size_t)Lmax + 1 + rsik::kScanPad, INFINITY);
+  del[0] = -1.0;
+  uint64_t n = 0;
+  for (int L = 1; L <= Lmax; ++L) {
+    const double dL = (double)L, sq = sqrt(dL);
+    auto score = [&](double sum) { ++n; const float meanf = (float)(sum / dL); return ((double)meanf - tmedian) * sq; };
+    del[L] = last_true([&](double s) { return !(score(s) > -tlamda); });
+    dup[L] = first_true([&](double s) { return !(score(s) < tlamda); });
+  }
+  if (evals) *evals += n;
+}
+inline void scan_thresholds(double tmedian, double tlamda, int Lmax, std::vector<double>& del, std::vector<double>& dup,
+                            uint64_t* evals = nullptr) {
+  del.assign((size_t)Lmax + 1 + rsik::kScanPad, -INFINITY);
+  dup.assign((size_t)Lmax + 1 + rsik::kScanPad, INFINITY);
+  del[0] = -1.0;
+  uint64_t n = 0;
+  constexpr int kFloatSteps = 8;
+  for (int L = 1; L <= Lmax; ++L) {
+    const double dL = (double)L, sq = sqrt(dL);
+    auto fscore = [&](float meanf) { return ((double)meanf - tmedian) * sq; };
+    auto score = [&](double sum) { ++n; return fscore((float)(sum / dL)); };
+    {
+      float F = (float)(tmedian - tlamda / sq);
+      for (int k = 0; k < kFloatSteps && fscore(F) > -tlamda; ++k) F = nextafterf(F, -INFINITY);
+      for (int k = 0; k < kFloatSteps && !(fscore(nextafterf(F, INFINITY)) > -tlamda); ++k) F = nextafterf(F, INFINITY);
+      const double guess = dL * (((double)F + (double)nextafterf(F, INFINITY)) * 0.5);
+      del[L] = last_true_from(guess, [&](double s) { return !(score(s) > -tlamda); });
+    }
+    {
+      float F = (float)(tmedian + tlamda / sq);
+      for (int k = 0; k < kFloatSteps && fscore(F) < tlamda; ++k) F = nextafterf(F, INFINITY);
+      for (int k = 0; k < kFloatSteps && !(fscore(nextafterf(F, -INFINITY)) < tlamda); ++k) F = nextafterf(F, -INFINITY);
+      const double guess = dL * (((double)F + (double)nextafterf(F, -INFINITY)) * 0.5);
+      dup[L] = first_true_from(guess, [&](double s) { return !(score(s) < tlamda); });
+    }
+  }
+  if (evals) *evals += n;
 }
 
 struct ScanRecord {
```

Measured after the change: 281.5 billion, median of 2. No clear change (+0.1%).
